# Robinatp/YOLO_Tensorflow

Measured on AMD Instinct MI355X. Metric: images_per_sec, higher is better.
Workload: dtype bf16; 1 GPU; YOLOv3 416x416 batch=32 per GPU, bf16: conv stack + head decode + threshold + TF-NMS; global_batch=32, input=uint8 NHWC resident in HBM, weights=seeded synthetic darknet stream (seed 0), parallelism=dp1

## Files before the change

### include/yolo_hip.h

```cpp
#ifndef YOLO_HIP_H
#define YOLO_HIP_H

#include <stddef.h>
#include <stdint.h>

#ifdef __cplusplus
extern "C" {
#endif

typedef struct yolo_ctx yolo_ctx;

enum yolo_status {
    YOLO_OK = 0,
    YOLO_ERR_INVALID = -1,
    YOLO_ERR_HIP = -2,
    YOLO_ERR_STATE = -3,
    YOLO_ERR_NOMEM = -4,
    YOLO_ERR_IO = -5,
    YOLO_ERR_UNSUPPORTED = -6
};

enum yolo_dtype { YOLO_BF16 = 0, YOLO_FP32 = 1, YOLO_FP8 = 2,
                  YOLO_FP16 = 3,
                  YOLO_FP16X2 = 4 };
// ... 12 lines not shown
    YOLO_NMS_TF_V1 = 4,
    YOLO_NMS_NUMPY_V3 = 3
};
enum yolo_select_mode {
    YOLO_SELECT_GT = 0,
    YOLO_SELECT_GE = 1
};

typedef struct yolo_config {
    uint32_t struct_size;
    const char *cfg_text;
    int32_t max_batch;
    int32_t dtype;
    int32_t semantics;
    int32_t decode;
    int32_t device;
    int32_t keep_layers;
    void *stream;
} yolo_config;

typedef struct yolo_box {
    float x0, y0, x1, y1;
    float score;
    int32_t cls;
} yolo_box;

typedef struct yolo_image_desc {
    uint64_t offset;
    int32_t h, w;
} yolo_image_desc;
enum yolo_fit {
    YOLO_FIT_STRETCH = 0,
    YOLO_FIT_LETTERBOX = 1,
    YOLO_FIT_CV2 = 2,
    YOLO_FIT_CV2_BGR = 3
};
enum yolo_box_units { YOLO_UNITS_NETWORK = 0, YOLO_UNITS_SOURCE_PIXELS = 1 };

yolo_ctx *yolo_create(const yolo_config *cfg, char *err, size_t err_len);
void yolo_destroy(yolo_ctx *ctx);
const char *yolo_last_error(const yolo_ctx *ctx);

int yolo_load_darknet_weights(yolo_ctx *ctx, const char *path, int header_ints);
int yolo_export(yolo_ctx *ctx, const char *path);
yolo_ctx *yolo_create_from_file(const char *path, int max_batch, int device, void *stream, int keep_layers, char *err, size_t err_len);
int yolo_set_weights(yolo_ctx *ctx, const float *flat, size_t n);
size_t yolo_weights_count(const yolo_ctx *ctx);
int yolo_set_act_scales(yolo_ctx *ctx, const float *scales, int n_layers);

int yolo_input_size(const yolo_ctx *ctx, int *height, int *width, int *channels);
int yolo_num_rows(const yolo_ctx *ctx);
int yolo_num_attrs(const yolo_ctx *ctx);
int yolo_num_layers(const yolo_ctx *ctx);
int yolo_head_geometry_hw(const yolo_ctx *ctx, int head, int *kind, int *grid_h, int *grid_w, int *anchors, int *row_offset);
int yolo_head_geometry(const yolo_ctx *ctx, int head, int *kind, int *grid, int *anchors, int *row_offset);
double yolo_conv_flops(const yolo_ctx *ctx);
double yolo_conv_bytes(const yolo_ctx *ctx, int n);

int yolo_forward(yolo_ctx *ctx, const void *images, int n, int fmt, int loc, float scale,
                 float *detections_out, int out_loc);

int yolo_forward_image_u8(yolo_ctx *ctx, const uint8_t *image, int h, int w, int loc,
                          float *detections_out, int out_loc);
int yolo_forward_letterbox_chw(yolo_ctx *ctx, const float *image_chw, int w, int h, int loc,
                               float *detections_out, int out_loc);

int yolo_forward_images_u8(yolo_ctx *ctx, const uint8_t *pixels, size_t bytes, const yolo_image_desc *descs, int n, int fit, int loc,
                           float *detections_out, int out_loc);
int yolo_detect_images_u8(yolo_ctx *ctx, const uint8_t *pixels, size_t bytes, const yolo_image_desc *descs, int n, int fit, int loc,
                          float score_thr, float iou_thr, int max_out, int nms_mode, int select_mode, int units,
                          yolo_box *boxes_out, int32_t *counts_out, int out_loc);
int yolo_detect_images_graph(yolo_ctx *ctx, const uint8_t *pixels, size_t bytes, const yolo_image_desc *descs, int n, int fit,
                             float score_thr, float iou_thr, int max_out, int nms_mode, int select_mode, int units,
                             yolo_box *boxes_out, int32_t *counts_out);
float yolo_fit_unit_value(int fit, int value);

int yolo_darknet_boxes(yolo_ctx *ctx, int w, int h, float thresh, int relative, float *records, int cap, int *count);
int yolo_darknet_boxes_at(yolo_ctx *ctx, int image, int w, int h, float thresh, int relative, float *records, int cap, int *count);
size_t yolo_last_layer_size(const yolo_ctx *ctx);
int yolo_last_layer_output(yolo_ctx *ctx, float *out, size_t out_floats);
int yolo_last_layer_output_batch(yolo_ctx *ctx, int n, float *out, size_t out_floats);

int yolo_head_raw(yolo_ctx *ctx, int head, int n, float *out, size_t out_floats);

int yolo_postprocess(yolo_ctx *ctx, int n, float score_thr, float iou_thr, int max_out,
                     int nms_mode, int select_mode, yolo_box *boxes_out, int32_t *counts_out, int out_loc);

int yolo_postprocess_rows(yolo_ctx *ctx, int n, float score_thr, float iou_thr, int max_out,
                          int nms_mode, int select_mode, yolo_box *boxes_out, int32_t *counts_out, int32_t *rows_out, int out_loc);

int yolo_detect(yolo_ctx *ctx, const void *images, int n, int fmt, int loc, float scale,
                float score_thr, float iou_thr, int max_out, int nms_mode, int select_mode,
                yolo_box *boxes_out, int32_t *counts_out, int out_loc);

int yolo_detect_graph(yolo_ctx *ctx, const void *images, int n, int fmt, float scale, float score_thr, float iou_thr,
                      int max_out, int nms_mode, int select_mode, yolo_box *boxes_out, int32_t *counts_out);

int yolo_synchronize(yolo_ctx *ctx);

int yolo_layer_output(yolo_ctx *ctx, int index, int n, float *out, size_t out_floats, int *dims_out);
int yolo_time_forward(yolo_ctx *ctx, int n, int iters, float *total_ms, float *conv_ms);
int yolo_calibrate(int device, void *stream, int f16, double seconds, float *tflops, float *clock_ghz);
int yolo_calibrate_copy(int device, void *stream, double seconds, float *gbs);
int yolo_time_layers(yolo_ctx *ctx, int n, int iters, float *ms_out);
int yolo_autotune(yolo_ctx *ctx, int n, int iters);
int yolo_get_tile_configs(const yolo_ctx *ctx, int32_t *cfgs);
int yolo_set_tile_configs(yolo_ctx *ctx, const int32_t *cfgs);

int yolo_op_conv2d(const float *x, int n, int h, int w, int cin, const float *w_hwio, const float *bias,
                   int k, int stride, int cout, int act, const float *residual, float *out,
                   int dtype, int tile_cfg, int device);
int yolo_op_conv_num_cfgs(void);
int yolo_op_upsample2x(const float *x, int n, int h, int w, int c, int semantics, float *out, int device);
int yolo_op_reorg(const float *x, int n, int h, int w, int c, int stride, int semantics, float *out, int device);
int yolo_op_maxpool(const float *x, int n, int h, int w, int c, int size, int stride, float *out, int device);
int yolo_op_resize_u8_hw(const uint8_t *img, int h, int w, int out_h, int out_w, float post_scale, float *out, int device);
int yolo_op_resize_u8(const uint8_t *img, int h, int w, int s, float post_scale, float *out, int device);
int yolo_op_resize_cv2(const uint8_t *img, int h, int w, int oh, int ow, int swap_rb, float divisor, float *out, int device);
int yolo_op_detections_boxes(const float *det, int n, int rows, int attrs, float *out, int device);
int yolo_op_decode_hw(const float *raw, int n, int gh, int gw, int na, int classes, const float *anchors_wh,
                      int img_h, int img_w, int decode, int region, float *out, int device);
int yolo_op_decode(const float *raw, int n, int g, int na, int classes, const float *anchors_wh,
                   int img_size, int decode, int region, float *out, int device);
int yolo_op_letterbox(const float *image_chw, int iw, int ih, int w, int h, int embed, float *out_chw, int device);
int yolo_op_nms_detections(const float *boxes_xywh, float *prob, float *objectness, int n, int classes, float thresh,
                           int by_objectness, int device);
int yolo_op_postprocess(const float *det, int n, int rows, int attrs, float score_thr, float iou_thr,
                        int max_out, int nms_mode, int select_mode, yolo_box *boxes_out,
                        int32_t *counts_out, int device);
int yolo_op_postprocess_rows(const float *det, int n, int rows, int attrs, float score_thr, float iou_thr,
                             int max_out, int nms_mode, int select_mode, yolo_box *boxes_out,
                             int32_t *counts_out, int32_t *rows_out, int device);

int yolo_num_classes(const yolo_ctx *ctx);
int yolo_classify(yolo_ctx *ctx, const void *images, int n, int fmt, int loc, float scale, int top_k,
                  int32_t *classes_out, float *probs_out, int out_loc);
int yolo_classify_images_u8(yolo_ctx *ctx, const uint8_t *pixels, size_t bytes, const yolo_image_desc *descs, int n, int fit, int loc,
                            int top_k, int32_t *classes_out, float *probs_out, int out_loc);
int yolo_op_avgpool(const float *x, int n, int h, int w, int c, int dtype, float *out, int device);
enum yolo_activation { YOLO_ACT_LINEAR = 0, YOLO_ACT_LEAKY = 1, YOLO_ACT_RELU = 2, YOLO_ACT_RELIE = 3, YOLO_ACT_LOGISTIC = 4, YOLO_ACT_LOGGY = 5,
                       YOLO_ACT_ELU = 6, YOLO_ACT_RAMP = 7, YOLO_ACT_TANH = 8, YOLO_ACT_PLSE = 9, YOLO_ACT_STAIR = 10, YOLO_ACT_HARDTAN = 11, YOLO_ACT_LHTAN = 12 };
int yolo_activation_code(const char *name);
int yolo_op_activate(const float *x, int n, int h, int w, int c, int act, int dtype, float *out, int device);
int yolo_op_shortcut(const float *x, int n, int h2, int w2, int c2, const float *from, int h1, int w1, int c1, int act, int dtype,
                     float *out, int device);
int yolo_op_softmax(const float *x, int n, int len, int groups, float temperature, int top_k, float *probs_out,
                    int32_t *classes_out, float *topk_probs_out, int device);

enum yolo_hierarchy_mode { YOLO_HIER_CONDITIONAL = 0, YOLO_HIER_ABSOLUTE = 1, YOLO_HIER_LEAVES = 2 };
int yolo_set_hier_thresh(yolo_ctx *ctx, float hier_thresh);
int yolo_set_hierarchy_mode(yolo_ctx *ctx, int mode);
int yolo_darknet_boxes_map(yolo_ctx *ctx, int image, int w, int h, float thresh, int relative, const int32_t *map200, float *records, int cap, int *count);
int yolo_tree_geometry(const yolo_ctx *ctx, int32_t *nodes, int32_t *groups, int32_t *parent, int32_t *child, int32_t *group_offset,
                       int32_t *group_size, int32_t *leaf);
int yolo_tree_read(const char *path, int32_t *nodes, int32_t *groups, int32_t *parent, int32_t *child, int32_t *group_offset, int32_t *group_size,
                   int32_t *leaf, char *err, size_t err_len);
int yolo_plan_check(const char *cfg_text, int dtype, char *err, size_t err_len);
int yolo_plan_table(const char *cfg_text, int dtype, int max_batch, int keep_layers, char *out, size_t out_len, char *err, size_t err_len);
int yolo_op_tree_softmax(const float *x, int n, int len, const char *tree_path, float temperature, int mode, float *out, int device);
int yolo_op_tree_top(const float *x_logits, int n, const char *tree_path, float hier_thresh, int32_t *labels_out, int device);


int yolo_output_map_geometry(yolo_ctx *ctx, int *h, int *w, int *c);
int yolo_output_map(yolo_ctx *ctx, int n, float *out, size_t out_floats);
int yolo_label_map(yolo_ctx *ctx, int n, float thresh, uint8_t *labels_u8);
int yolo_segment_images_u8(yolo_ctx *ctx, const uint8_t *pixels, const yolo_image_desc *descs, int n, int fit, float thresh,
                           uint8_t *labels_u8, const uint64_t *label_offsets);
int yolo_op_deconv2d(const float *x, int n, int h, int w, int cin, const float *w_iohw, const float *bias, int size, int stride, int padding,
                     int cout, int act, int dtype, int out_f32, float *out, int device);
int yolo_op_conv2d_grouped(const float *x, int n, int h, int w, int cin, const float *w_oihw, const float *bias, int size, int stride, int padding,
                           int cout, int groups, int act, int dtype, int out_f32, float *out, int device);
int yolo_op_l2norm(const float *x, int n, int h, int w, int c, int dtype, float *out, int device);
int yolo_op_upsample(const float *x, int n, int h, int w, int c, int stride, float scale, int dtype, float *out, int device);
int yolo_op_label_map(const float *map, int n, int h, int w, int c, float thresh, uint8_t *labels_out, int device);

#ifdef __cplusplus
}
#endif
#endif
```

### yolo_tensorflow_amd/csrc/conv_cfgs.h

```cpp
#pragma once
#include "kernels.h"
#include <type_traits>

struct ConvCfg {
    int id, wp, wc, tp, tc, ns, bk, nl;
    bool halo;
    bool free;
    int bh, bw;
    bool head_tail;
};
#define X(id, wp, wc, tp, tc, ns, bk, nl) {id, wp, wc, tp, tc, ns, bk, nl, false, false, 0, 0, false},
#define HX(id, wp, wc, tp, tc, ns, bk, nl, free, bh, bw, head_tail) {id, wp, wc, tp, tc, ns, bk, nl, true, free, bh, bw, head_tail},
constexpr ConvCfg kCfgs[] = {
    X(0, 2, 2, 4, 4, 2, 64, 0)  X(1, 2, 2, 4, 4, 3, 64, 0)  X(2, 2, 2, 2, 4, 2, 64, 0)  X(3, 2, 2, 2, 4, 3, 64, 0)
    X(4, 4, 1, 4, 2, 2, 64, 0)  X(5, 4, 1, 4, 2, 3, 64, 0)  X(6, 2, 2, 4, 2, 2, 64, 0)  X(7, 2, 2, 4, 2, 3, 64, 0)
    X(8, 4, 1, 4, 4, 2, 64, 0)  X(9, 4, 1, 4, 4, 3, 64, 0)  X(10, 4, 2, 4, 4, 2, 64, 0) X(11, 4, 2, 4, 4, 3, 64, 0)
    X(12, 2, 4, 4, 4, 2, 64, 0) X(13, 2, 4, 4, 4, 3, 64, 0) X(14, 2, 2, 2, 2, 2, 64, 0) X(15, 2, 2, 2, 2, 4, 64, 0)
    X(16, 1, 4, 11, 2, 2, 64, 0) X(17, 1, 4, 11, 4, 2, 64, 0) X(18, 1, 4, 11, 1, 2, 64, 0) X(19, 1, 4, 10, 2, 2, 64, 0)
    X(20, 1, 4, 12, 2, 2, 64, 0) X(21, 1, 4, 9, 2, 2, 64, 0) X(22, 1, 4, 13, 2, 2, 64, 0) X(23, 1, 4, 6, 2, 2, 64, 0)
    X(24, 1, 4, 7, 2, 2, 64, 0)
    X(25, 1, 4, 11, 2, 2, 32, 0) X(26, 2, 2, 4, 2, 2, 32, 0)  X(27, 4, 1, 4, 2, 2, 32, 0)  X(28, 4, 1, 4, 4, 2, 32, 0)
    X(29, 2, 2, 2, 2, 2, 32, 0)  X(30, 2, 2, 2, 4, 2, 32, 0)
    X(31, 1, 8, 11, 2, 2, 64, 4) X(32, 1, 8, 11, 2, 2, 64, 0)
    X(33, 1, 4, 11, 2, 3, 64, 0) X(34, 1, 4, 6, 2, 3, 64, 0)
    X(35, 2, 4, 3, 4, 2, 64, 0)
    HX(36, 1, 8, 11, 2, 2, 64, 0, false, 13, 13, false) HX(37, 1, 8, 11, 2, 2, 64, 4, false, 13, 13, false)
    HX(38, 1, 4, 11, 2, 2, 64, 4, false, 13, 13, false) HX(39, 1, 4, 11, 2, 2, 64, 0, false, 13, 13, false)
    HX(40, 1, 8, 11, 2, 2, 64, 0, true, 13, 13, true)   HX(41, 1, 8, 11, 1, 2, 64, 0, true, 13, 13, false)
    HX(42, 1, 4, 11, 2, 2, 64, 0, true, 13, 13, false)  HX(43, 1, 8, 11, 1, 3, 64, 0, true, 13, 13, false)
    X(44, 1, 8, 6, 2, 2, 64, 0) X(45, 1, 8, 6, 2, 3, 64, 0) X(46, 2, 4, 3, 4, 2, 64, 0) X(47, 2, 4, 2, 4, 2, 64, 0)
    X(48, 2, 4, 3, 2, 2, 64, 0) X(49, 2, 4, 4, 2, 3, 64, 0) X(50, 1, 8, 4, 2, 3, 64, 0) X(51, 2, 4, 2, 2, 3, 64, 0)
    X(52, 2, 4, 3, 2, 3, 64, 0) X(53, 2, 4, 3, 2, 4, 64, 0)
    HX(54, 1, 8, 12, 2, 2, 64, 0, true, 10, 19, true) HX(55, 1, 8, 12, 1, 3, 64, 0, true, 10, 19, false) HX(56, 1, 8, 6, 1, 3, 64, 0, true, 5, 19, false)
    HX(57, 1, 4, 11, 4, 2, 64, 0, true, 13, 13, false) HX(58, 1, 4, 11, 2, 2, 64, 0, true, 13, 13, false)
};
#undef X
#undef HX
constexpr int kNumCfgs = (int)(sizeof(kCfgs) / sizeof(kCfgs[0]));
constexpr bool conv_cfgs_indexed() { for (int i = 0; i < kNumCfgs; ++i) if (kCfgs[i].id != i) return false; return true; }
static_assert(conv_cfgs_indexed(), "a tile configuration's id is its index in kCfgs");

template <int... I> struct CfgList { static constexpr bool has(int cfg) { return ((cfg == I) || ...); } };
template <int... I, class F> hipError_t cfg_dispatch(CfgList<I...>, int cfg, F &&f)
{
    hipError_t e = hipErrorInvalidValue;
    (void)((cfg == I && ((e = f(std::integral_constant<int, I>{})), true)) || ...);
    return e;
}
using Cfgs16 = CfgList<0, 1, 2, 3, 4, 5, 6, 7, 8, 9, 10, 11, 12, 13, 14, 15, 16, 17, 18, 19, 20, 21, 22, 23, 24, 25, 26, 27, 28, 29, 30, 31, 32, 33, 34, 35,
                       44, 45, 46, 47, 48, 49, 50, 51, 52, 53>;
using CfgsHalo16 = CfgList<36, 37, 38, 39, 40, 41, 42, 43, 54, 55, 56>;
using CfgsFp8 = CfgList<0, 2, 4, 6, 8, 12, 14, 16, 17, 19, 20, 23, 31, 32, 33, 34, 45, 48, 49, 51>;
using CfgsHaloFp8 = CfgList<36, 37, 38, 39, 40, 41, 42, 43>;
using CfgsSplit = CfgList<0, 2, 3, 4, 6, 7, 8, 14, 15, 16, 23, 25, 26, 27, 28, 33, 34, 45, 49, 52>;
using CfgsHaloSplit = CfgList<40, 41, 43>;
using CfgsPairK = CfgList<0, 2, 3, 4, 6, 7, 8, 14, 15, 16, 23, 33, 34, 45, 49, 52>;
using CfgsHaloPairK = CfgList<40, 41, 43, 57, 58>;
using CfgsPairKPlain = CfgList<0, 2, 4, 6, 8, 14, 16, 33>;

template <int... I> constexpr bool cfgs_are(CfgList<I...>, bool halo) { return ((I >= 0 && I < kNumCfgs && kCfgs[I].halo == halo) && ...); }
static_assert(cfgs_are(Cfgs16{}, false) && cfgs_are(CfgsFp8{}, false) && cfgs_are(CfgsSplit{}, false) && cfgs_are(CfgsPairK{}, false) && cfgs_are(CfgsPairKPlain{}, false), "tiled lists hold tiled ids");
static_assert(cfgs_are(CfgsHalo16{}, true) && cfgs_are(CfgsHaloFp8{}, true) && cfgs_are(CfgsHaloSplit{}, true) && cfgs_are(CfgsHaloPairK{}, true), "halo lists hold halo ids");

inline bool conv_cfg_instantiated(const ConvArgs &a, int cfg)
{
    if (a.in_dt == DT_FP8) return CfgsFp8::has(cfg) || CfgsHaloFp8::has(cfg);
    if (a.pairk) return a.split ? CfgsPairK::has(cfg) || CfgsHaloPairK::has(cfg) : CfgsPairKPlain::has(cfg);
    if (a.split) return CfgsSplit::has(cfg) || CfgsHaloSplit::has(cfg);
    return Cfgs16::has(cfg) || CfgsHalo16::has(cfg);
}

constexpr bool conv_tail_shape(int wp, int wc, int bc, int nl, int eb) { return wp == 1 && wc == 8 && (eb == 2 ? nl == 0 && (bc == 256 || bc == 128) : bc == 256); }
```

### yolo_tensorflow_amd/csrc/conv_igemm.hip

```cpp
#include "kernels.h"
#include <cstdio>
#include <mutex>
#include <set>
#include <utility>

hipError_t conv_opt_in_lds(const void *kernel, size_t lds_bytes)
{
    static std::mutex mu;
    static std::set<std::pair<int, const void *>> done;
    int dev = 0;
    hipError_t e = hipGetDevice(&dev); if (e != hipSuccess) return e;
    std::lock_guard<std::mutex> g(mu);
    if (done.count({dev, kernel})) return hipSuccess;
    e = hipFuncSetAttribute(kernel, hipFuncAttributeMaxDynamicSharedMemorySize, (int)lds_bytes);
    if (e == hipSuccess) done.insert({dev, kernel});
    return e;
}

#include "conv_igemm_kernel.h"


template <int EB>
static hipError_t launch_conv_diag_t(const ConvArgs &a, hipStream_t s)
{
// ... 94 lines not shown
{
    return (a.in_dt == DT_BF16 || (a.in_dt == DT_F16 && a.out_dt == DT_F16)) && a.ksize == 3 && a.stride == 1 && a.pad == 1 && a.Cin_pad == 8 && a.out_dt != DT_F32 && !a.res && a.Kpad >= 96 &&
           (a.Cout == 16 || a.Cout == 32 || a.Cout == 64);
}

hipError_t launch_conv_c8_direct(const ConvArgs &a, hipStream_t s)
{
    const long M = (long)a.N * a.Ho * a.Wo;
    long waves = (M + 63) / 64;
    long blocks = (waves + 3) / 4; if (blocks > 256 * 8) blocks = 256 * 8;
    dim3 grid((unsigned)blocks), block(256);
    if (a.in_dt == DT_F16) {
        if (a.Cout == 16) hipLaunchKernelGGL((conv_c8_3x3_direct<1, true>), grid, block, 0, s, a);
        else if (a.Cout == 32) hipLaunchKernelGGL((conv_c8_3x3_direct<2, true>), grid, block, 0, s, a);
        else hipLaunchKernelGGL((conv_c8_3x3_direct<4, true>), grid, block, 0, s, a);
    }
    else if (a.Cout == 16) hipLaunchKernelGGL((conv_c8_3x3_direct<1>), grid, block, 0, s, a);
    else if (a.Cout == 32) hipLaunchKernelGGL((conv_c8_3x3_direct<2>), grid, block, 0, s, a);
    else hipLaunchKernelGGL((conv_c8_3x3_direct<4>), grid, block, 0, s, a);
    return hipGetLastError();
}

int conv_num_cfgs() { return kNumCfgs; }
bool conv_cfg_is_halo(int cfg) { return cfg >= 0 && cfg < kNumCfgs && kCfgs[cfg].halo; }
bool conv_cfg_tail_ok(int cfg, int cout, bool fp8, bool head)
{
    if (cfg < 0 || cfg >= kNumCfgs) return false;
    const ConvCfg &c = kCfgs[cfg];
    const int bc = c.wc * c.tc * 16;
    if (head) return !fp8 && c.head_tail && cout == 256;
    return conv_tail_shape(c.wp, c.wc, bc, c.nl, fp8 ? 1 : 2) && bc == cout;
}
const char *conv_cfg_name(int cfg)
{
    struct Names {
        char s[kNumCfgs][32];
        Names()
        {
            for (const ConvCfg &c : kCfgs) {
                const int bp = c.wp * c.tp * 16, bc = c.wc * c.tc * 16;
                if (c.halo && !CfgsHalo16::has(c.id)) snprintf(s[c.id], sizeof s[c.id], "f%dc%d_w%d_pair", bp, bc, c.wp * c.wc);
                else if (c.halo && (c.bh != HALO_B || c.bw != HALO_B)) snprintf(s[c.id], sizeof s[c.id], "f%dx%dc%d_s%d", c.bh, c.bw, bc, c.ns);
                else snprintf(s[c.id], sizeof s[c.id], "%s%dc%d_s%d_k%d%s%d", c.halo ? (c.free ? "f" : "h") : "p", bp, bc, c.ns, c.bk, c.nl ? "_L" : "_w", c.nl ? c.nl : c.wp * c.wc);
            }
        }
    };
    static const Names names;
    if (cfg < 0 || cfg >= kNumCfgs) return cfg == CONV_CFG_DIRECT ? "direct_c8" : "?";
    return names.s[cfg];
}

template <int WP, int WC, int TP, int TC, int NS, int BK, int NL, bool UNI, int EB, bool H16 = false, bool SPLIT = false>
static hipError_t launch_u(const ConvArgs &a, hipStream_t s)
{
    constexpr int BP = WP * TP * 16, BC = WC * TC * 16;
    const long M = (long)a.N * a.Ho * a.Wo;
    const long tiles = ((M + BP - 1) / BP) * ((a.Cout + BC - 1) / BC);
    constexpr size_t lds = conv_lds_bytes<WP, WC, TP, TC, NS, BK, NL>();
    dim3 grid((unsigned)((tiles + 7) / 8 * 8)), block(64 * (WP * WC + NL));
    if (lds > 65536) {
        hipError_t e = conv_opt_in_lds((const void *)conv_igemm<WP, WC, TP, TC, NS, BK, UNI, NL, false, EB, false, false, H16, SPLIT>, lds);
        if (e != hipSuccess) return e;
    }
    hipLaunchKernelGGL((conv_igemm<WP, WC, TP, TC, NS, BK, UNI, NL, false, EB, false, false, H16, SPLIT>), grid, block, lds, s, conv_tile_magic(a, BC, 0));
    return hipGetLastError();
}

template <int WP, int WC, int TP, int TC, int NS, int BK, int NL, int EB, bool H16 = false, bool SPLIT = false>
static hipError_t launch_t(const ConvArgs &a, hipStream_t s)
{
    if (((double)a.N * a.H * a.W * a.in_stride + 2.0 * (a.W + 1) * a.in_stride) * EB >= 2147483648.0) return hipErrorInvalidValue;
    constexpr int BKE = BK * 2 / EB;
    if (a.Kpad % BKE) return hipErrorInvalidValue;
    return (a.Cin_pad % BKE) == 0 ? launch_u<WP, WC, TP, TC, NS, BK, NL, true, EB, H16, SPLIT>(a, s) : launch_u<WP, WC, TP, TC, NS, BK, NL, false, EB, H16, SPLIT>(a, s);
}

template <int ID, int EB, bool H16 = false, bool SPLIT = false>
static hipError_t launch_id(const ConvArgs &a, hipStream_t s)
{
    constexpr ConvCfg c = kCfgs[ID];
    return launch_t<c.wp, c.wc, c.tp, c.tc, c.ns, c.bk, c.nl, EB, H16, SPLIT>(a, s);
}

hipError_t launch_conv_bf16(const ConvArgs &a, int cfg, hipStream_t s)
{
    if (a.in_dt != DT_BF16 && a.in_dt != DT_F16) return hipErrorInvalidValue;
    if (a.in_dt == DT_F16 && a.out_dt != DT_F16 && a.out_dt != DT_F32) return hipErrorInvalidValue;
    if (cfg == CONV_CFG_DIRECT && a.split) return launch_conv_c8_direct_pair(a, s);
    if (a.pairk) return launch_conv_pair(a, cfg, s);
    if (a.split) {
        if (a.in_dt != DT_F16 || (a.out_dt != DT_F16 && a.out_dt != DT_F32) || a.w2 || (a.res && a.out_dt == DT_F32)) return hipErrorInvalidValue;
        if (CfgsHaloSplit::has(cfg)) return launch_conv_halo13(a, cfg, s);
        return cfg_dispatch(CfgsSplit{}, cfg, [&](auto id) { return launch_id<decltype(id)::value, 2, true, true>(a, s); });
    }
    if (cfg == CONV_CFG_DIRECT) return conv_c8_direct_ok(a) ? launch_conv_c8_direct(a, s) : hipErrorInvalidValue;
    if (conv_cfg_is_halo(cfg)) return launch_conv_halo13(a, cfg, s);
    if (a.in_dt == DT_F16) return cfg_dispatch(Cfgs16{}, cfg, [&](auto id) { return launch_id<decltype(id)::value, 2, true>(a, s); });
    return cfg_dispatch(Cfgs16{}, cfg, [&](auto id) { return launch_id<decltype(id)::value, 2>(a, s); });
}

hipError_t launch_conv_fp8(const ConvArgs &a, int cfg, hipStream_t s)
{
    if (a.in_dt != DT_FP8) return hipErrorInvalidValue;
    if (CfgsHaloFp8::has(cfg)) return launch_conv_halo13(a, cfg, s);
    return cfg_dispatch(CfgsFp8{}, cfg, [&](auto id) { return launch_id<decltype(id)::value, 1>(a, s); });
}
```

### yolo_tensorflow_amd/csrc/conv_igemm_kernel.h

```cpp
#pragma once
#include "kernels.h"
#include "conv_cfgs.h"
#include "device_common.h"
#include "halo_perm_tables.h"
#include <type_traits>
#include <utility>

__device__ __forceinline__ uint32_t f32_to_bf16_rn(float f)
{
    __bf16 b = (__bf16)f;
    return (uint32_t)__builtin_bit_cast(uint16_t, b);
}
__device__ __forceinline__ float bf16_bits_to_f32(uint32_t b) { return __builtin_bit_cast(float, b << 16); }
__device__ __forceinline__ void pair_join2(uint32_t H, uint32_t L, float &a, float &b)
{
    asm("v_fma_mix_f32 %0, %1, 1.0, %2 op_sel_hi:[1,0,1]" : "=v"(a) : "v"(H), "v"(L));
    asm("v_fma_mix_f32 %0, %1, 1.0, %2 op_sel:[1,0,1] op_sel_hi:[1,0,1]" : "=v"(b) : "v"(H), "v"(L));
}
__device__ __forceinline__ void pair_split2(float a, float b, uint32_t &H, uint32_t &L)
{
    H = __builtin_bit_cast(uint32_t, __builtin_convertvector(f32x2_t{a, b}, f16x2_t));
    uint32_t l;
    asm("v_fma_mixlo_f16 %0, %1, -1.0, %2 op_sel_hi:[1,0,0]" : "=v"(l) : "v"(H), "v"(a));
    asm("v_fma_mixhi_f16 %0, %1, -1.0, %2 op_sel:[1,0,0] op_sel_hi:[1,0,0]" : "+v"(l) : "v"(H), "v"(b));
    L = l;
}
template <bool HI> __device__ __forceinline__ uint32_t f32x2_to_fp8(float a, float b, uint32_t old)
{
    a = __builtin_amdgcn_fmed3f(a, -FP8_MAX, FP8_MAX); b = __builtin_amdgcn_fmed3f(b, -FP8_MAX, FP8_MAX);
    return (uint32_t)__builtin_amdgcn_cvt_pk_fp8_f32(a, b, (int)old, HI);
}

__device__ __forceinline__ int fast_div(int n, uint32_t mul, uint32_t shift)
{
    return shift == 255 ? n : (int)(__umulhi((uint32_t)n, mul) >> shift);
}

constexpr int PAIR_PD = 4, PAIR_SLEEP = 48;
template <int MAXN> __device__ __forceinline__ void wait_vmcnt_rt(int n)
{
    static_assert(MAXN <= 16, "ladder length");
    switch (n) {
#define W_(k) case k: if (k <= MAXN) { wait_vmcnt<k>(); } break;
        W_(1) W_(2) W_(3) W_(4) W_(5) W_(6) W_(7) W_(8) W_(9) W_(10) W_(11) W_(12) W_(13) W_(14) W_(15) W_(16)
#undef W_
    default: wait_vmcnt<0>(); break;
    }
}

#define OOB_OFFSET 0x80000000u

template <int... I, class F> __device__ __forceinline__ void static_for_impl(std::integer_sequence<int, I...>, F &&f) { (f(std::integral_constant<int, I>{}), ...); }
template <int N, class F> __device__ __forceinline__ void static_for(F &&f) { static_for_impl(std::make_integer_sequence<int, N>{}, f); }

struct HaloPermPk { unsigned w[16][8]; };
template <int N> constexpr HaloPermPk make_halo_perm_pk(const unsigned short (&tab)[N])
{
    HaloPermPk t{};
    for (int l = 0; l < 16; ++l)
        for (int j = 0; j < N / 16; ++j) {
            const unsigned v = tab[j * 16 + l];
            t.w[l][j / 4] |= (v & 0xffu) << (8 * (j % 4));
            t.w[l][4 + j / 4] |= (v >> 8) << (8 * (j % 4));
        }
    return t;
}
__device__ const HaloPermPk kHaloPermPk = make_halo_perm_pk(kHaloPerm13);
__device__ const HaloPermPk kHaloPermPk10x19 = make_halo_perm_pk(kHaloPerm10x19);
__device__ const HaloPermPk kHaloPermPk5x19 = make_halo_perm_pk(kHaloPerm5x19);
constexpr int HALO_B = 13;
constexpr int HALO_APIX = 160;
constexpr int halo_apieces(int bh, int bw) { return ((bh + 2) * (bw + 2) * (HALO_APIX / 16) + 63) / 64; }
constexpr int HALO_APIECES = halo_apieces(HALO_B, HALO_B);
constexpr int HALO_ACT_BYTES = HALO_APIECES * 1024;
constexpr unsigned halo_div_mul(int bw) { return (65536u + bw - 1) / bw; }
constexpr bool halo_div_ok(int bw) { for (unsigned r = 0; r < 256; ++r) if (((r * halo_div_mul(bw)) >> 16) != r / bw) return false; return true; }

template <int WP, int WC, int TP, int TC, int NS, int BK, bool UNI, int NL = 0, bool DIAG = false, int EB = 2, bool HALO = false, bool FREE = false, bool H16 = false, bool SPLIT = false, int BH = HALO_B, int BW = HALO_B, bool HEADT = false, bool PAIRK = false>
__global__ __launch_bounds__(64 * (WP * WC + NL)) void conv_igemm(const ConvArgs a)
{
#if defined(__HIP_DEVICE_COMPILE__)
    constexpr int NC = WP * WC;
    constexpr int NW = NL > 0 ? NL : NC;
    constexpr int NTOT = NC + NL;
    constexpr int BP = WP * TP * 16;
    constexpr int BC = WC * TC * 16;
    static_assert(BK == 64 || BK == 32, "K-step");
    static_assert(BC <= 256, "filters and bias are padded to multiples of 256 output channels (cout_pad): a wider tile would read past them");
    static_assert(EB == 2 || (EB == 1 && BK == 64), "fp8 operands need the 128-B-row form");
    static_assert(!H16 || EB == 2, "fp16 is a 16-bit storage type");
    static_assert(!SPLIT || (H16 && !DIAG), "split pairs are fp16 pairs");
    static_assert(!PAIRK || (H16 && EB == 2 && BK == 64 && UNI && !DIAG && NL == 0), "pair K loop: fp16, 128-byte rows = one 32-channel group hi | lo, uniform taps");
    constexpr int RB = BK * 2;
    constexpr int EPC = 16 / EB;
    constexpr int BKE = RB / EB;
    constexpr int CPRW = RB / 16;
    constexpr int RG = 64 / CPRW;
    constexpr int GP = (BP + RG - 1) / RG, GC = (BC + RG - 1) / RG;
    constexpr int LA = (GP + NW - 1) / NW, LB = (GC + NW - 1) / NW;
    constexpr int L = LA + LB;
    constexpr int BPL = LA * NW * RG, BCL = LB * NW * RG;
    constexpr int STAGE_BYTES = (BPL + BCL) * RB;
    static_assert(!HALO || (WP == 1 && TP == (BH * BW + 15) / 16 && TP <= 16 && BK == 64 && UNI && (NS == 2 || (FREE && NS <= 4))), "halo form: one BH x BW block per workgroup; more than two filter stages in the free-running form only");
    static_assert((BH == 13 && BW == 13) || (BH == 10 && BW == 19) || (BH == 5 && BW == 19), "block shapes with a generated permutation table");
    static_assert(halo_div_ok(BW) && BH * BW <= 256, "row / BW by multiply-high");
    constexpr int HBH = BH, HBW = BW, HPW = BW + 2, HPH = BH + 2, APIX = HALO_APIX, APIECES = halo_apieces(BH, BW), ACT_BYTES = APIECES * 1024;
    constexpr int LAH = HALO ? (APIECES + NW - 1) / NW : 1;
    constexpr int FSTAGE = BCL * RB;
    static_assert(!HALO || LAH <= 9, "a halo tile is fetched during the nine taps of the previous chunk");
    static_assert(!FREE || (HALO && NL == 0 && LB * RG == TC * 16), "free-running form: every wave fetches its own filter rows");

    if constexpr (H16) fp16_saturating_mode();
    extern __shared__ __attribute__((aligned(16))) char smem[];

    unsigned long long t_top = 0;
    if (DIAG) asm volatile("s_memtime %0\n\ts_waitcnt lgkmcnt(0)" : "=s"(t_top)::"memory");
    const int tid = threadIdx.x;
    const int lane = tid & 63;
    u32x4_t perm_rd = {0, 0, 0, 0}, perm_wr = {0, 0, 0, 0};
    if constexpr (HALO) {
        const u32x4_t *pk = (const u32x4_t *)(BH == 10 ? kHaloPermPk10x19.w[lane & 15] : BH == 5 ? kHaloPermPk5x19.w[lane & 15] : kHaloPermPk.w[lane & 15]);
        perm_rd = pk[0]; perm_wr = pk[1];
    }
    asm volatile("" ::"s"(a.in), "s"(a.wt), "s"(a.in_stride), "s"(a.N), "s"(a.H), "s"(a.W), "s"(a.Cout), "s"(a.Kpad), "s"(a.Ho), "s"(a.Wo),
                 "s"(a.tc_mul), "s"(a.tc_shift), "s"(a.bpi_mul), "s"(a.bpi_shift), "s"(a.bpr_mul), "s"(a.bpr_shift));
    const int wave_id = __builtin_amdgcn_readfirstlane(tid >> 6);
    const bool is_loader = NL == 0 || wave_id >= NC;
    const bool is_consumer = wave_id < NC;
    const int wid = NL > 0 ? (wave_id >= NC ? wave_id - NC : 0) : wave_id;
    const int wpi = wave_id % WP, wci = (wave_id / WP) % WC;

    const int M = a.N * a.Ho * a.Wo;
    const int tilesC = (a.Cout + BC - 1) / BC;
    const int hbr = HALO ? (a.H + HBH - 1) / HBH : 0, hbc = HALO ? (a.W + HBW - 1) / HBW : 0;
    const int tilesP = HALO ? a.N * hbr * hbc : (M + BP - 1) / BP;
    const int per_xcd = gridDim.x >> 3;
    const int tile = (blockIdx.x & 7) * per_xcd + (blockIdx.x >> 3);
    if (tile >= tilesP * tilesC) return;
    const int pt = fast_div(tile, a.tc_mul, a.tc_shift);
    const int ct = tile - pt * tilesC;
    int bn = 0, by = 0, bx = 0;
    if constexpr (HALO) {
        const int bpr = hbc, bpi = hbc * hbr;
        bn = fast_div(pt, a.bpi_mul, a.bpi_shift); const int r = pt - bn * bpi; by = fast_div(r, a.bpr_mul, a.bpr_shift); bx = r - by * bpr;
    }

    const int shift = HALO ? 0 : (a.W + 1) * a.in_stride * EB;
    __amdgpu_buffer_rsrc_t rx = buf_rsrc((const char *)a.in - shift);
    __amdgpu_buffer_rsrc_t rw = buf_rsrc(a.wt);

    const int rl = lane / CPRW;
    const int chunk = BK == 64 ? ((lane & 7) ^ (rl & 7)) : ((lane & 3) ^ (3 * ((rl >> 2) & 1)));
    const int KK = a.ksize * a.ksize;
    const int HoWo = a.Ho * a.Wo;
    unsigned woff[LB > 0 ? LB : 1];
#pragma unroll
    for (int i = 0; i < LB; ++i) {
        const int crow = (FREE ? wid * LB + i : wid + i * NW) * RG + rl;
        woff[i] = crow < BC ? (unsigned)((ct * BC + crow) * a.Kpad + chunk * EPC) * (unsigned)EB : OOB_OFFSET;
    }
    if (is_loader && 0 < a.Kpad / BKE) {
// ... 715 lines not shown
                if (is_consumer) {
                    const float slope2 = act_slope(a.act2);
                    f32x4 b2v[T2W];
#pragma unroll
                    for (int t = 0; t < T2W; ++t) b2v[t] = *(const f32x4 *)(a.b2 + (t2g * T2W + t) * 16 + lq * 4);
                    const int hch = (t2g * T2W) * 16 + lq * 4;
                    auto finish = [&](const f32x4 &acc2, int j, int t) {
                        f32x4 v = acc2 + b2v[t];
                        if constexpr (HEAD_TAIL_OK) if (head_tail) {
                            const unsigned r = (unsigned)(j * 16 + l15), y = __umul24(r, halo_div_mul(BW)) >> 16, x = r - __umul24(y, (unsigned)BW);
                            if (y < ylim && x < xlim) {
                                const size_t m = m0 + (size_t)y * a.W + x;
                                const int ch = hch + t * 16;
                                float *o = (float *)a.out2 + m * a.out2_stride + ch;
                                if (a.obj_out) {
#pragma unroll
                                    for (int q = 0; q < 4; ++q) {
                                        const int an = fast_div(ch + q, a.obj_mul, a.obj_shift);
                                        if (ch + q - an * a.obj_attrs == 4 && ch + q < a.C2out) a.obj_out[m * a.obj_na + an] = v[q];
                                    }
                                }
                                if (ch + 3 < a.C2out) *(float4 *)o = float4{v[0], v[1], v[2], v[3]};
                                else
                                    for (int q = 0; q < 4; ++q) if (ch + q < a.C2out) o[q] = v[q];
                            }
                            return;
                        }
                        const f32x4 u = v * slope2;
#pragma unroll
                        for (int q = 0; q < 4; ++q) v[q] = vmax_f32(v[q], u[q]);
                        *(uint2 *)(st2 + (j * 16 + l15) * RS2 + ((t2g * T2W + t) * 16 + lq * 4) * 2) = uint2{pack16x2<H16>(v[0], v[1]), pack16x2<H16>(v[2], v[3])};
                    };
                    const int j0 = head_tail ? 0 : (TP * t2p) / T2P, j1 = head_tail ? TP : (TP * (t2p + 1)) / T2P;
                    {
                        int j = j0;
#pragma unroll 1
                        for (; j + 1 < j1; j += 2) {
                            f32x4 ca[T2W], cb[T2W];
#pragma unroll
                            for (int t = 0; t < T2W; ++t) ca[t] = cb[t] = f32x4{0.f, 0.f, 0.f, 0.f};
#pragma unroll
                            for (int kk = 0; kk < K2S; ++kk) {
                                const bf16x8 xa = *(const bf16x8 *)(smem + (j * 16 + l15) * RS + (kk * 4 + lq) * 16);
                                const bf16x8 xb = *(const bf16x8 *)(smem + ((j + 1) * 16 + l15) * RS + (kk * 4 + lq) * 16);
#pragma unroll
                                for (int t = 0; t < T2W; ++t) {
                                    ca[t] = mma16<H16>(fw2[t][kk], xa, ca[t]);
                                    cb[t] = mma16<H16>(fw2[t][kk], xb, cb[t]);
                                }
                            }
#pragma unroll
                            for (int t = 0; t < T2W; ++t) { finish(ca[t], j, t); finish(cb[t], j + 1, t); }
                        }
                        if (j < j1) {
                            f32x4 cc_[T2W];
#pragma unroll
                            for (int t = 0; t < T2W; ++t) cc_[t] = f32x4{0.f, 0.f, 0.f, 0.f};
#pragma unroll
                            for (int kk = 0; kk < K2S; ++kk) {
                                const bf16x8 x = *(const bf16x8 *)(smem + (j * 16 + l15) * RS + (kk * 4 + lq) * 16);
#pragma unroll
                                for (int t = 0; t < T2W; ++t) cc_[t] = mma16<H16>(fw2[t][kk], x, cc_[t]);
                            }
#pragma unroll
                            for (int t = 0; t < T2W; ++t) finish(cc_[t], j, t);
                        }
                    }
                }
                if (DIAG) te5 = stamp();
                asm volatile("s_waitcnt lgkmcnt(0)" ::: "memory");
                block_barrier();
                if (DIAG) te6 = stamp();
                constexpr int CPR2 = C2 / 8;
                const __amdgpu_buffer_rsrc_t rs_out2 = tile_rsrc((char *)a.out2 + m0 * a.out2_stride * 2);
                if (!head_tail)
#pragma unroll
                for (int it = 0; it < (BP * CPR2 + NT - 1) / NT; ++it) {
                    int row, cc;
                    const unsigned off = piece_off(tid + it * NT, CPR2, 0, (unsigned)a.out2_stride * 2u, row, cc);
                    __builtin_amdgcn_raw_buffer_store_b128(*(const u32x4_t *)(st2 + row * RS2 + cc * 16), rs_out2, off, 0, OUT_STORE_AUX);
                }
            }
        }
    } else if (is_consumer && !HALO) {
#pragma unroll
        for (int i = 0; i < TC; ++i) {
            const int ch = ct * BC + (wci * TC + i) * 16 + lq * 4;
            if (ch >= a.Cout) continue;
            const float4 bv = *(const float4 *)(a.bias + ch);
            float4 sv = float4{1.f, 1.f, 1.f, 1.f};
            if (EB == 1 && a.oscale) sv = *(const float4 *)(a.oscale + ch);
            int oq = -1, oan = 0;
            if (a.obj_out) {
#pragma unroll
                for (int q = 0; q < 4; ++q) {
                    const int an = fast_div(ch + q, a.obj_mul, a.obj_shift);
                    if (ch + q - an * a.obj_attrs == 4 && ch + q < a.Cout) { oq = q; oan = an; }
                }
            }
#pragma unroll
            for (int j = 0; j < TP; ++j) {
                const int m = pt * BP + (wpi * TP + j) * 16 + l15;
                if (m >= M) continue;
                float v[4];
                if (EB == 1) { v[0] = acc[i][j][0] * sv.x + bv.x; v[1] = acc[i][j][1] * sv.y + bv.y; v[2] = acc[i][j][2] * sv.z + bv.z; v[3] = acc[i][j][3] * sv.w + bv.w; }
                else { v[0] = acc[i][j][0] + bv.x; v[1] = acc[i][j][1] + bv.y; v[2] = acc[i][j][2] + bv.z; v[3] = acc[i][j][3] + bv.w; }
                if (a.act != ACT_LINEAR) {
                    const float slope = act_slope(a.act);
#pragma unroll
                    for (int q = 0; q < 4; ++q) v[q] = fmaxf(v[q], slope * v[q]);
                }
                float *o = (float *)a.out + (size_t)m * a.out_stride + ch;
                if (oq >= 0) a.obj_out[(size_t)m * a.obj_na + oan] = oq == 0 ? v[0] : oq == 1 ? v[1] : oq == 2 ? v[2] : v[3];
                if (ch + 3 < a.Cout) *(float4 *)o = float4{v[0], v[1], v[2], v[3]};
                else
                    for (int q = 0; q < 4; ++q) if (ch + q < a.Cout) o[q] = v[q];
            }
        }
    }
    if (DIAG && a.dbg && lane == 0) {
        asm volatile("s_waitcnt vmcnt(0)" ::: "memory");
        const unsigned long long t_end = stamp_loop();
        unsigned long long *d = a.dbg + ((size_t)tile * NTOT + wave_id) * 16;
        const unsigned long long rt1 = __builtin_amdgcn_s_memrealtime();
        d[0] = t_wait; d[1] = t_issue; d[2] = t_mma; d[3] = t_loop_end - t_all0; d[4] = t_end - t_loop_end;
        d[6] = t_all0 - t_top; d[7] = t_first - t_all0; d[8] = te1 - t_loop_end; d[9] = te2 - te1; d[10] = te3 - te2; d[11] = t_end - (te6 ? te6 : te3);
        d[12] = te4 ? te4 - te3 : 0; d[13] = te4 ? te5 - te4 : 0; d[14] = te4 ? te6 - te5 : 0;
        d[15] = (t_loop_end - t_all0) * 100ull / (rt_loop - rt0 ? rt_loop - rt0 : 1);
        d[5] = ((unsigned long long)KT << 40) | ((t_end - t_all0) * 100ull / (rt1 - rt0 ? rt1 - rt0 : 1));
    }
#endif
}

template <int WP, int WC, int TP, int TC, int NS, int BK, int NL = 0, bool HALO = false, int BH = HALO_B, int BW = HALO_B>
constexpr size_t conv_lds_bytes()
{
    constexpr int NW = NL > 0 ? NL : WP * WC, BP = WP * TP * 16, BC = WC * TC * 16;
    constexpr int RG = 64 / (BK * 2 / 16);
    constexpr int LA = ((BP + RG - 1) / RG + NW - 1) / NW, LB = ((BC + RG - 1) / RG + NW - 1) / NW;
    constexpr size_t stage = (size_t)(LA + LB) * NW * RG * (BK * 2);
    constexpr bool tail = conv_tail_shape(WP, WC, BC, 0, 2);
    constexpr size_t lds0 = HALO ? (size_t)2 * halo_apieces(BH, BW) * 1024 + (size_t)NS * LB * NW * RG * (BK * 2) : (size_t)NS * stage, ldso = (size_t)BP * (BC * 2 + 16) + (tail ? (size_t)BP * (BC + 16) : 0);
    return lds0 > ldso ? lds0 : ldso;
}
```

### yolo_tensorflow_amd/csrc/kernels.h

```cpp
#pragma once
#ifndef OUT_STORE_AUX
#define OUT_STORE_AUX 16
#endif
#ifndef HALO_LOAD_AUX
#define HALO_LOAD_AUX 0
#endif
#ifndef RES_LOAD_AUX
#define RES_LOAD_AUX 0
#endif
#include <hip/hip_runtime.h>
#include <stdint.h>
typedef unsigned out_u32x4 __attribute__((ext_vector_type(4)));
__device__ __forceinline__ void out_store16_at(const void *base, unsigned byte_off, unsigned x, unsigned y, unsigned z, unsigned w)
{
#if defined(__HIP_DEVICE_COMPILE__)
    __amdgpu_buffer_rsrc_t r = __builtin_amdgcn_make_buffer_rsrc((void *)base, 0, 0x80000000u, 0x00020000);
    __builtin_amdgcn_raw_buffer_store_b128(out_u32x4{x, y, z, w}, r, byte_off, 0, OUT_STORE_AUX);
#endif
}

typedef uint16_t bf16_t;
struct fp8_t { uint8_t b; };
struct f16_t { uint16_t b; };
enum { DT_BF16 = 0, DT_F32 = 1, DT_FP8 = 2, DT_F16 = 3 };
inline size_t dt_size(int dt) { return dt == DT_F32 ? 4 : dt == DT_FP8 ? 1 : 2; }
#define FP8_MAX 448.0f

struct TView {
    void *ptr = nullptr;
    int n = 0, h = 0, w = 0, c = 0;
    int stride = 0;
    int dt = DT_BF16;
};

enum { ACT_LINEAR = 0, ACT_LEAKY = 1, ACT_RELU = 2, ACT_RELIE = 3, ACT_LOGISTIC = 4, ACT_LOGGY = 5, ACT_ELU = 6, ACT_RAMP = 7, ACT_TANH = 8,
       ACT_PLSE = 9, ACT_STAIR = 10, ACT_HARDTAN = 11, ACT_LHTAN = 12, ACT_COUNT = 13 };
inline bool act_is_slope(int act) { return act == ACT_LINEAR || act == ACT_LEAKY || act == ACT_RELU || act == ACT_RELIE; }
int act_from_name(const char *name);

struct ConvArgs {
    const void *in; int in_stride;
    const void *wt;
    const float *bias;
    void *out; int out_stride; int out_dt;
    const void *res; int res_stride;
    int in_dt;
    int split;
    int pairk;
    const float *oscale;
    float out_inv_scale, res_scale;
    float mid_scale, mid_inv_scale;
    const void *w2; const float *b2; void *out2; int out2_stride, K2pad, act2;
    const void *w2f;
    const float *oscale2; float out2_inv_scale;
    int N, H, W, Cin_pad;
    int Ho, Wo, Cout;
    int ksize, stride, pad;
    int Kpad;
    int kchunk;
    int act;
    const void *zeros;
    uint32_t howo_mul, howo_shift, wo_mul, wo_shift;
    float *obj_out; int obj_attrs, obj_na; uint32_t obj_mul, obj_shift;
    unsigned long long *dbg;
    int dbg_light;
    int C2out;
    int tail_f32;
    uint32_t tc_mul, tc_shift, bpi_mul, bpi_shift, bpr_mul, bpr_shift;
};
inline int conv_kchunk(int cin_pad, int wdt) { const int row = wdt == DT_FP8 ? 128 : 64; return (wdt != DT_F32 && cin_pad % row == 0) ? row : cin_pad; }
inline void conv_magic(uint32_t d, uint32_t &mul, uint32_t &shift)
{
    if (d <= 1) { mul = 0; shift = 255; return; }
    uint32_t l = 0; while ((1u << l) < d) ++l;
    const unsigned k = 31 + l;
    mul = (uint32_t)(((unsigned long long)1 << k) / d + 1);
    shift = k - 32;
}
inline void conv_finalize(ConvArgs &a)
{
    conv_magic((uint32_t)(a.Ho * a.Wo), a.howo_mul, a.howo_shift);
    conv_magic((uint32_t)a.Wo, a.wo_mul, a.wo_shift);
}
inline ConvArgs conv_tile_magic(const ConvArgs &a0, int BC, int bh, int bw = 0)
{
    ConvArgs a = a0;
    if (bw == 0) bw = bh;
    conv_magic((uint32_t)((a.Cout + BC - 1) / BC), a.tc_mul, a.tc_shift);
    if (bh > 0) { const int br = (a.H + bh - 1) / bh, bc = (a.W + bw - 1) / bw; conv_magic((uint32_t)(br * bc), a.bpi_mul, a.bpi_shift); conv_magic((uint32_t)bc, a.bpr_mul, a.bpr_shift); }
    return a;
}

hipError_t conv_opt_in_lds(const void *kernel, size_t lds_bytes);
#define CONV_CFG_DIRECT 1000
bool conv_c8_direct_ok(const ConvArgs &a);
int conv_num_cfgs();
const char *conv_cfg_name(int cfg);
int conv_default_cfg(const ConvArgs &a);
bool conv_cfg_runs(const ConvArgs &a, int cfg);
int conv_resolve_cfg(const ConvArgs &a, int planned);
hipError_t launch_conv_bf16(const ConvArgs &a, int cfg, hipStream_t s);
bool conv_halo13_ok(const ConvArgs &a);
bool conv_halo_cfg_ok(const ConvArgs &a, int cfg);
bool conv_cfg_is_halo(int cfg);
hipError_t launch_conv_halo13(const ConvArgs &a, int cfg, hipStream_t s);
hipError_t launch_conv_halo13_diag(const ConvArgs &a, hipStream_t s, int variant = 0);
bool conv_cfg_tail_ok(int cfg, int cout, bool fp8, bool head = false);
hipError_t launch_conv_pair(const ConvArgs &a, int cfg, hipStream_t s);
struct StemPairArgs {
    const void *in;
    const uint8_t *in_u8; float in_scale, in_mul, in_add;
    const void *w0; const float *b0; int Kpad0, C0, act0;
    const void *w1; const float *b1; int Kpad1, act1;
    void *out; int out_stride;
    int N, H, W, Ho, Wo;
};
bool conv_stem_pair_ok(const StemPairArgs &a);
hipError_t launch_conv_stem_pair(const StemPairArgs &a, hipStream_t s);
bool conv_c8_direct_pair_ok(const ConvArgs &a);
hipError_t launch_conv_c8_direct_pair(const ConvArgs &a, hipStream_t s);
hipError_t launch_conv_fp8(const ConvArgs &a, int cfg, hipStream_t s);
hipError_t launch_conv_diag(const ConvArgs &a, hipStream_t s);
struct StemArgs {
    const void *in; int in_stride;
    const uint8_t *in_u8; float in_scale, in_mul, in_add;
    const void *w0; const float *b0; int Kpad0, C0, act0;
    const void *w1; const float *b1; int Kpad1, C1, act1;
    void *out; int out_stride;
    int dt;
    const void *w2; const float *b2; int Kpad2, C2, act2;
    void *out2; int out2_stride;
    int N, H, W, Ho, Wo;
    const void *zeros;
};
bool conv_stem_ok(const StemArgs &a);
hipError_t launch_conv_stem(const StemArgs &a, hipStream_t s);
struct HaloArgs {
    const void *in; int in_stride;
    const void *w; const float *b; int Kpad, Cin, Cout, act;
    const void *res; int res_stride;
    void *out; int out_stride;
    int N, H, W;
    int dt;
};
bool conv_halo_ok(const HaloArgs &a);
hipError_t launch_conv_halo(const HaloArgs &a, hipStream_t s);
bool conv_s2_ok(const HaloArgs &a);
hipError_t launch_conv_s2(const HaloArgs &a, hipStream_t s);
struct C3S2Args {
    const void *in; int in_stride;
    const void *w3; const float *b3; int Kpad3, act3;
    const void *res; int res_stride;
    const void *w5; const float *b5; int Kpad5, act5;
    void *out; int out_stride;
    int N, H, W;
    int dt;
};
bool conv_c3s2_ok(const C3S2Args &a);
hipError_t launch_conv_c3s2(const C3S2Args &a, hipStream_t s);
struct BlockArgs {
    const void *x; int x_stride;
    const void *w1; const float *b1; int Kpad1, act1;
    const void *w2; const float *b2; int Kpad2, act2;
    void *out; int out_stride;
    int N, H, W, C, Cmid;
    int dt;
};
bool conv_resblock_ok(const BlockArgs &a);
hipError_t launch_conv_resblock(const BlockArgs &a, hipStream_t s);
hipError_t launch_conv_f32(const ConvArgs &a, hipStream_t s);

#define DECONV_MAX_SIZE 7
#define DECONV_MAX_STRIDE 4
#define DECONV_CO_TILE 32
struct DeconvArgs {
    const void *in; int in_stride;
    const void *wt;
    const float *bias;
    void *out; int out_stride; int out_dt, in_dt;
    int N, H, W, Cin_pad, Ho, Wo, Cout;
    int Cstore;
    int size, stride, pad, act;
    int cout_pad;
    int woff[DECONV_MAX_STRIDE * DECONV_MAX_STRIDE], kp[DECONV_MAX_STRIDE * DECONV_MAX_STRIDE];
// ... 205 lines not shown
```

### yolo_tensorflow_amd/csrc/post_ops.hip

```cpp
#include "kernels.h"
#include "wave_ops.h"
#include <math.h>

struct BoxOut { float x0, y0, x1, y1, score; int cls; };

__device__ __forceinline__ float sigmoidf_(float x) { return 1.0f / (1.0f + expf(-x)); }
__device__ __forceinline__ float sigmoid_fast(float x)
{
    const float e = __builtin_amdgcn_exp2f(-x * 1.44269504088896340736f);
    return __builtin_amdgcn_rcpf(1.0f + e);
}

__device__ __forceinline__ float yolo_box_attr(int k, float x, int cx, int cy, const float *anchor, float GW, float GH, float SX, float SY, int mode)
{
    const float t = k < 2 ? sigmoidf_(x) + (float)(k == 0 ? cx : cy) : expf(x) * anchor[k - 2];
    const float G = (k & 1) ? GH : GW, S = (k & 1) ? SY : SX;
    return mode == 0 ? t / G : t * S;
}

__global__ __launch_bounds__(256) void k_decode_yolo(const DecodeArgs a, float *scores, int *labels)
{
    const int attrs = 5 + a.classes;
    const int lane = threadIdx.x & 63;
    const long wave = ((long)blockIdx.x * blockDim.x + threadIdx.x) >> 6;
    const long nwaves = ((long)gridDim.x * blockDim.x) >> 6;
    const int gg = a.gh * a.gw;
    const long total = (long)a.n * gg * a.na;
    const float GW = (float)a.gw, GH = (float)a.gh, SX = (float)(a.img_w / a.gw), SY = (float)(a.img_h / a.gh);
    constexpr int U = 4;
    const bool two = attrs > 64;
    for (long b0 = wave * U; b0 < total; b0 += nwaves * U) {
        float v0[U], v1[U];
        const float *src[U]; float *dst[U]; size_t rowi[U]; int an_[U], cell_[U];
        const unsigned ub = (unsigned)__builtin_amdgcn_readfirstlane((int)b0);
        unsigned t0 = ub / (unsigned)a.na; int an = (int)(ub - t0 * a.na);
        int b = (int)(t0 / (unsigned)gg); int cell = (int)(t0 - (unsigned)b * gg);
#pragma unroll
        for (int u = 0; u < U; ++u) {
            if (u > 0 && b0 + u < total) { if (++an == a.na) { an = 0; if (++cell == gg) { cell = 0; ++b; } } }
            an_[u] = an; cell_[u] = cell;
            src[u] = a.raw + ((size_t)b * gg + cell) * a.raw_stride + an * attrs;
            rowi[u] = (size_t)b * a.rows_total + a.row_off + (size_t)cell * a.na + an;
            dst[u] = a.det + rowi[u] * attrs;
            v0[u] = lane < attrs ? src[u][lane] : 0.f;
            v1[u] = (two && lane + 64 < attrs) ? src[u][lane + 64] : 0.f;
        }
#pragma unroll
        for (int u = 0; u < U; ++u) {
            if (b0 + u >= total) break;
            const int an = an_[u], cell = cell_[u];
            const float r0 = lane < 4 ? yolo_box_attr(lane, v0[u], cell % a.gw, cell / a.gw, a.anchors + 2 * an, GW, GH, SX, SY, a.mode) : sigmoid_fast(v0[u]);
            const float r1 = sigmoid_fast(v1[u]);
            if (lane < attrs) dst[u][lane] = r0;
            if (two && lane + 64 < attrs) dst[u][lane + 64] = r1;
            const float obj = __shfl(r0, 4);
            float best = -INFINITY; int bi = 0x7fffffff;
            if (lane >= 5 && lane < attrs) { best = obj * r0; bi = lane - 5; }
            if (two && lane + 64 < attrs) first_max(best, bi, obj * r1, lane + 59);
            wave_argmax(best, bi);
            if (lane == 0 && scores) { scores[rowi[u]] = best; labels[rowi[u]] = bi; }
        }
    }
}

template <int CTRL, int ROWS = 0xF, typename T>
__device__ __forceinline__ T dpp(T v)
{
    const int i = __builtin_bit_cast(int, v);
    return __builtin_bit_cast(T, __builtin_amdgcn_update_dpp(i, i, CTRL, ROWS, 0xF, false));
}
template <typename T, typename Op>
__device__ __forceinline__ T row_reduce_dpp(T v, Op op)
{
    v = op(v, dpp<0xB1>(v));
    v = op(v, dpp<0x4E>(v));
    v = op(v, dpp<0x124>(v));
    v = op(v, dpp<0x128>(v));
    return v;
}
__device__ __forceinline__ float row_max_dpp(float v) { return row_reduce_dpp(v, [](float x, float y) { return fmaxf(x, y); }); }
__device__ __forceinline__ int row_min_dpp(int v) { return row_reduce_dpp(v, [](int x, int y) { return min(x, y); }); }
__device__ __forceinline__ float wave_max_dpp(float v)
{
    v = row_max_dpp(v);
    v = fmaxf(v, dpp<0x142, 0xA>(v));
    v = fmaxf(v, dpp<0x143, 0xC>(v));
    return __builtin_bit_cast(float, __builtin_amdgcn_readlane(__builtin_bit_cast(int, v), 63));
}

__device__ __forceinline__ int block_rank(bool flag, int *wcnt, int &total)
{
    const int lane = threadIdx.x & 63, wv = threadIdx.x >> 6;
    const unsigned long long m = __ballot(flag);
    if (lane == 0) wcnt[wv] = __popcll(m);
// ... 36 lines not shown
    }
    for (long p = wave; p < total; p += nwaves) {
        const unsigned up = (unsigned)__builtin_amdgcn_readfirstlane((int)p);
        const int b = (int)(up / (unsigned)gg), cell = (int)(up - (unsigned)b * gg);
        const int cy = cell / a.gw, cx = cell - cy * a.gw;
        const size_t row0 = (size_t)b * a.rows_total + a.row_off + (size_t)cell * a.na;
        float *dst = a.det ? a.det + row0 * attrs : nullptr;
        float *dst4 = a.box4 ? a.box4 + row0 * 4 : nullptr;
        float x[R], v[R];
#pragma unroll
        for (int r = 0; r < R; ++r) x[r] = xn[r];
        if (p + nwaves < total) {
            const float *src = a.raw + (size_t)(p + nwaves) * a.raw_stride;
#pragma unroll
            for (int r = 0; r < R; ++r) xn[r] = ok_[r] ? src[lane + 64 * r] : 0.f;
        }
        float xs = 0.f; int ks = 4, ans = 0;
        if (merged) {
#pragma unroll
            for (int r = 0; r < R; ++r) if (spec_[r]) { xs = x[r]; ks = k_[r]; ans = an_[r]; }
            const float vs = ks < 4 ? yolo_box_attr(ks, xs, cx, cy, a.anchors + 2 * ans, GW, GH, SX, SY, a.mode) : 0.f;
#pragma unroll
            for (int r = 0; r < R; ++r) {
                v[r] = spec_[r] ? vs : sigmoid_fast(x[r]);
                if (dst) { if (ok_[r]) dst[lane + 64 * r] = v[r]; }
                else if (spec_[r]) dst4[an_[r] * 4 + k_[r]] = v[r];
            }
        } else {
#pragma unroll
            for (int r = 0; r < R; ++r) {
                v[r] = k_[r] < 4 ? yolo_box_attr(k_[r], x[r], cx, cy, a.anchors + 2 * an_[r], GW, GH, SX, SY, a.mode) : sigmoid_fast(x[r]);
                if (dst) { if (ok_[r]) dst[lane + 64 * r] = v[r]; }
                else if (spec_[r]) dst4[an_[r] * 4 + k_[r]] = v[r];
            }
        }
        if (!scores) continue;
        for (int an = 0; an < a.na; ++an) {
            const int oc = an * attrs + 4, ol = oc & 63, orr = oc >> 6;
            float ov = v[0];
#pragma unroll
            for (int r = 1; r < R; ++r) ov = orr == r ? v[r] : ov;
            const float obj = __shfl(ov, ol);
            if (obj < a.reject_below) {
                if (lane == 0) { scores[row0 + an] = obj; labels[row0 + an] = 0; }
                continue;
            }
            float sc[R]; float best = -INFINITY;
#pragma unroll
            for (int r = 0; r < R; ++r) {
                sc[r] = (ok_[r] && an_[r] == an && k_[r] >= 5) ? obj * v[r] : -INFINITY;
                best = fmaxf(best, sc[r]);
            }
            best = wave_max_dpp(best);
            int label = 0x7fffffff;
#pragma unroll
            for (int r = R - 1; r >= 0; --r) {
                const unsigned long long m = __ballot(sc[r] == best);
                if (m) label = (int)__builtin_ctzll(m) + 64 * r - an * attrs - 5;
            }
            if (lane == 0) { scores[row0 + an] = best; labels[row0 + an] = label; }
        }
    }
}

__global__ __launch_bounds__(1024) void k_decode_yolo_lean_p1(const LeanArgs a, float *scores, int *labels)
{
    __shared__ int wcnt[16]; __shared__ unsigned s_base;
    const int attrs = 5 + a.classes;
    for (long base = (long)blockIdx.x * 1024; base < a.total; base += (long)gridDim.x * 1024) {
        const long box = base + threadIdx.x;
        const bool valid = box < a.total;
        int hd = 0;
#pragma unroll
        for (int k = 1; k < 4; ++k) if (k < a.nheads && box >= a.h[k].box_begin) hd = k;
        const float *raw = a.h[0].raw, *objp = a.h[0].obj; int raw_stride = a.h[0].raw_stride, gg = a.h[0].gh * a.h[0].gw, na = a.h[0].na, row_off = a.h[0].row_off; long bb = a.h[0].box_begin;
#pragma unroll
        for (int k = 1; k < 4; ++k) if (hd == k) { raw = a.h[k].raw; objp = a.h[k].obj; raw_stride = a.h[k].raw_stride; gg = a.h[k].gh * a.h[k].gw; na = a.h[k].na; row_off = a.h[k].row_off; bb = a.h[k].box_begin; }
        const unsigned ubox = valid ? (unsigned)(box - bb) : 0u;
        const unsigned cidx = ubox / (unsigned)na; const int an = (int)(ubox - cidx * (unsigned)na);
        const unsigned b = cidx / (unsigned)gg; const int cell = (int)(cidx - b * (unsigned)gg);
        const unsigned row = b * (unsigned)a.rows_total + (unsigned)row_off + (unsigned)cell * (unsigned)na + (unsigned)an;
        const unsigned eoff = cidx * (unsigned)raw_stride + (unsigned)(an * attrs);
        const float obj = sigmoid_fast(objp ? objp[ubox] : raw[eoff + 4]);
        const bool pass = valid && !(obj < a.reject_below);
        if (valid && !pass) { scores[row] = obj; labels[row] = 0; }
        int tot;
        const int rank = block_rank(pass, wcnt, tot);
        if (threadIdx.x == 0 && tot) s_base = atomicAdd(a.list_count, (unsigned)tot);
        __syncthreads();
        const unsigned slot = s_base + (unsigned)rank;
        if (pass && slot < a.list_cap) a.list[slot] = uint4{eoff, row, (unsigned)cell | ((unsigned)an << 24) | ((unsigned)hd << 28), __float_as_uint(obj)};
    }
}
__global__ __launch_bounds__(256) void k_decode_yolo_lean_p2(const LeanArgs a, float *scores, int *labels)
{
    const int attrs = 5 + a.classes;
    const int l15 = threadIdx.x & 15;
    const unsigned rowid = (blockIdx.x * blockDim.x + threadIdx.x) >> 4, nrows = (gridDim.x * blockDim.x) >> 4;
    unsigned count = __hip_atomic_load(a.list_count, __ATOMIC_RELAXED, __HIP_MEMORY_SCOPE_AGENT);
    if (count > a.list_cap) count = a.list_cap;
    for (unsigned base = 0; base < count; base += nrows) {
        const unsigned idx = base + rowid;
        const bool act = idx < count;
        const uint4 d = act ? a.list[idx] : uint4{0, 0, 0, 0};
        const unsigned r_eoff = d.x, r_row = d.y; const int r_cell = (int)(d.z & 0xffffffu), r_an = (int)((d.z >> 24) & 15u), r_hd = (int)(d.z >> 28);
        const float r_obj = __uint_as_float(d.w);
        const float *r_raw = a.h[0].raw; int r_gw = a.h[0].gw, r_gh = a.h[0].gh; float r_sx = a.h[0].sx, r_sy = a.h[0].sy;
#pragma unroll
        for (int k = 1; k < 4; ++k) if (r_hd == k) { r_raw = a.h[k].raw; r_gw = a.h[k].gw; r_gh = a.h[k].gh; r_sx = a.h[k].sx; r_sy = a.h[k].sy; }
        const float *src = r_raw + r_eoff;
        float vv[8];
#pragma unroll
        for (int t = 0; t < 8; ++t) { const int k = l15 + 16 * t; vv[t] = (act && k < attrs) ? src[k] : 0.f; }
        const float g_raw = vv[0];
        float best = -INFINITY; int label = 0x7fffffff;
#pragma unroll
        for (int t = 0; t < 8; ++t) {
            const int k = l15 + 16 * t;
            if (act && k >= 5 && k < attrs) first_max(best, label, r_obj * sigmoid_fast(vv[t]), k - 5);
        }
        const float rbest = row_max_dpp(best);
        const int rlabel = row_min_dpp(best == rbest ? label : 0x7fffffff);
        if (act && l15 < 4) {
            a.box4[(size_t)r_row * 4 + l15] = yolo_box_attr(l15, g_raw, r_cell % r_gw, r_cell / r_gw, a.h[r_hd].anchors + 2 * r_an, (float)r_gw, (float)r_gh, r_sx, r_sy, a.mode);
            if (l15 == 0) { scores[r_row] = rbest; labels[r_row] = rlabel; }
        }
    }
}
hipError_t launch_decode_lean(const LeanArgs &a, float *scores, int *labels, hipStream_t s)
{
    if (a.nheads < 1 || a.nheads > 4 || !a.box4 || !scores || !labels || 5 + a.classes > 128 || !a.list || !a.list_count) return hipErrorInvalidValue;
    size_t blocks = ((size_t)a.total + 1023) / 1024; if (blocks > 256 * 2) blocks = 256 * 2;
    hipLaunchKernelGGL(k_decode_yolo_lean_p1, dim3((unsigned)blocks), dim3(1024), 0, s, a, scores, labels);
    hipLaunchKernelGGL(k_decode_yolo_lean_p2, dim3(1024), dim3(256), 0, s, a, scores, labels);
    return hipGetLastError();
}

__global__ void k_decode_region(const DecodeArgs a)
{
    const int attrs = 5 + a.classes;
    size_t box = (size_t)blockIdx.x * blockDim.x + threadIdx.x;
    const int gg = a.gh * a.gw;
    const size_t total = (size_t)a.n * gg * a.na;
    if (box >= total) return;
    int an = (int)(box % a.na); size_t t = box / a.na;
    int cell = (int)(t % gg); int b = (int)(t / gg);
    const float *p = a.raw + ((size_t)b * gg + cell) * a.raw_stride + an * attrs;
    float *o = a.det + ((size_t)b * a.rows_total + a.row_off + (size_t)cell * a.na + an) * attrs;
#pragma unroll
    for (int k = 0; k < 5; ++k) o[k] = region_box_attr(k, p, cell, a.gw, a.gh, a.anchors + 2 * an);
    float mx = -INFINITY;
    for (int k = 0; k < a.classes; ++k) mx = fmaxf(mx, p[5 + k]);
    float sum = 0.f;
    for (int k = 0; k < a.classes; ++k) sum += expf(p[5 + k] - mx);
    for (int k = 0; k < a.classes; ++k) o[5 + k] = expf(p[5 + k] - mx) / sum;
}

__global__ void k_decode_v1(const float *raw, int raw_stride, int n, int S, int B, int C, int sqr, float *det, int rows_total, int row_off,
                            float *scores, int *labels)
{
    const int i = blockIdx.x * blockDim.x + threadIdx.x;
    const int per = S * S * B;
    if (i >= n * per) return;
    const int img = i / per, r = i - img * per, cell = r / B, b = r - cell * B;
    const float *p = raw + (size_t)img * raw_stride;
    const float *cls = p + cell * C, *box = p + S * S * (C + B) + (cell * B + b) * 4;
    const float conf = p[S * S * C + cell * B + b];
// ... 674 lines not shown
```

### yolo_tensorflow_amd/csrc/yolo_api.cpp

```cpp
#include "yolo_ctx.h"

namespace yolo_impl {

int need_map(yolo_ctx *c, const char *what)
{
    if (c->map_layer < 0) return fail(c, YOLO_ERR_INVALID, "%s: the network is not a map network (a %s; [net] yolo_output=map declares one)", what, c->cls_layer >= 0 ? "classifier" : "detector");
    return YOLO_OK;
}

int map_to_f32(yolo_ctx *c, int n)
{
    const Layer &M = c->layers[c->map_layer];
    const size_t cap = 2 * (size_t)c->max_batch * M.H * M.W * M.C;
    if (c->map_f32_cap < cap) { HIPCK(c, hipMalloc((void **)&c->d_map_f32, cap * 4)); c->map_f32_cap = cap; }
    TView v = M.out; v.n = n;
    HIPCK(c, launch_to_f32(v, c->d_map_f32, c->stream));
    return YOLO_OK;
}

int map_f32_view(yolo_ctx *c, int n, const float **map, int *stride)
{
    const Layer &M = c->layers[c->map_layer];
    if (M.out.dt == DT_F32) { *map = (const float *)M.out.ptr; *stride = M.out.stride; return YOLO_OK; }
    if (int r = map_to_f32(c, n)) return r;
// ... 87 lines not shown
    if (int r = yolo_head_geometry_hw(c, head, kind, &gh, &gw, anchors, row_offset)) return r;
    if (gh != gw) return fail(const_cast<yolo_ctx *>(c), YOLO_ERR_UNSUPPORTED, "yolo_head_geometry: head %d has a %d x %d grid; use yolo_head_geometry_hw", head, gh, gw);
    if (grid) *grid = gh;
    return YOLO_OK;
}
double yolo_conv_flops(const yolo_ctx *c) { return c ? c->conv_flops : 0; }
double yolo_conv_bytes(const yolo_ctx *c, int n)
{
    if (!c) return 0;
    double b = 0;
    for (int i = 0; i < (int)c->layers.size(); ++i) if (c->layers[i].type == L_CONV) {
        const Layer &L = c->layers[i];
        const TView in = view_of(c, L.in[0]); const double ie = (double)dt_size(L.in_dt), oe = (double)dt_size(L.out.dt);
        if (!input_never_loaded(L, i)) b += (double)n * in.h * in.w * L.cin * ie;
        if (!never_stored(L, i)) b += (double)n * L.H * L.W * L.filters * oe;
        b += (double)L.filters * L.cin * L.size * L.size * ie;
    }
    return b;
}

int yolo_darknet_boxes(yolo_ctx *c, int w, int h, float thresh, int relative, float *records, int cap, int *count)
{
    return yolo_darknet_boxes_at(c, 0, w, h, thresh, relative, records, cap, count);
}

int yolo_darknet_boxes_at(yolo_ctx *c, int image, int w, int h, float thresh, int relative, float *records, int cap, int *count)
{
    return yolo_darknet_boxes_map(c, image, w, h, thresh, relative, nullptr, records, cap, count);
}

int yolo_darknet_boxes_map(yolo_ctx *c, int image, int w, int h, float thresh, int relative, const int32_t *map200, float *records, int cap, int *count)
{
    if (!c || !count) return YOLO_ERR_INVALID;
    if (map200) {
        if (c->tree_head < 0) return fail(c, YOLO_ERR_INVALID, "yolo_darknet_boxes_map: the network has no [region] head with a tree");
        if (c->attrs - 5 < 200) return fail(c, YOLO_ERR_INVALID, "yolo_darknet_boxes_map: a map has 200 entries and the head only %d classes", c->attrs - 5);
        for (int j = 0; j < 200; ++j) if (map200[j] < 0 || map200[j] >= c->attrs - 5) return fail(c, YOLO_ERR_INVALID, "yolo_darknet_boxes_map: map[%d] = %d is not a class", j, (int)map200[j]);
    }
    if (int r = need_detector(c, "yolo_darknet_boxes")) return r;
    if (c->last_n < 1 || !c->det_valid) return fail(c, YOLO_ERR_STATE, "yolo_darknet_boxes needs a yolo_forward* pass first");
    if (image < 0 || image >= c->last_n) return fail(c, YOLO_ERR_INVALID, "image %d outside the last forward's batch of %d", image, c->last_n);
    if (w < 1 || h < 1 || cap < 0 || (cap > 0 && !records)) return fail(c, YOLO_ERR_INVALID, "bad image size / capacity");
    HIPCK(c, hipSetDevice(c->device));
    if (!c->d_dn_rec) {
        HIPCK(c, hipMalloc((void **)&c->d_dn_rec, (size_t)c->rows * c->attrs * 4));
        HIPCK(c, hipMalloc((void **)&c->d_dn_src, (size_t)c->rows * 4));
        HIPCK(c, hipMalloc((void **)&c->d_dn_count, 4));
    }
    DnBoxesArgs a; memset(&a, 0, sizeof a);
    a.det = c->d_det + (size_t)image * c->rows * c->attrs; a.attrs = c->attrs;
    for (size_t li = 0; li < c->layers.size(); ++li) {
        const Layer &L = c->layers[li];
        if (L.type != L_YOLO && L.type != L_REGION && L.type != L_DETECT) continue;
        if (a.nheads == 8) return fail(c, YOLO_ERR_UNSUPPORTED, "more than 8 heads");
        if (L.type == L_DETECT) {
            if (a.nheads) return fail(c, YOLO_ERR_UNSUPPORTED, "a [detection] head next to other heads");
            a.raw = (const float *)c->layers[li - 1].out.ptr + (size_t)image * c->layers[li - 1].out.stride; a.side = L.side; a.classes = L.classes; a.sqr = L.sqr;
            a.kind[0] = 2; a.cells[0] = L.side * L.side; a.na[0] = L.na; a.off[0] = L.row_off; a.nheads = 1;
            continue;
        }
        if (a.raw) return fail(c, YOLO_ERR_UNSUPPORTED, "a [detection] head next to other heads");
        a.kind[a.nheads] = L.type == L_REGION; a.cells[a.nheads] = L.H * L.W; a.na[a.nheads] = L.na; a.off[a.nheads] = L.row_off; ++a.nheads;
    }
    a.thresh = thresh; a.w = w; a.h = h; a.netw = c->in_w; a.neth = c->in_h; a.relative = relative;
    a.cap = cap < c->rows ? cap : c->rows;
    a.rec = a.cap > 0 ? c->d_dn_rec : nullptr; a.src = c->d_dn_src; a.count = c->d_dn_count;
    HIPCK(c, launch_darknet_boxes(a, c->stream));
    if (c->tree_head >= 0 && a.rec) {
        if (map200) {
            if (!c->d_map200) HIPCK(c, hipMalloc((void **)&c->d_map200, 200 * 4));
            HIPCK(c, hipMemcpyAsync(c->d_map200, map200, 200 * 4, hipMemcpyHostToDevice, c->stream));
        }
        HIPCK(c, launch_darknet_tree_probs(a.det, c->attrs, c->trees[c->layers[c->tree_head].tree].dev, thresh, c->hier_thresh, map200 ? c->d_map200 : nullptr,
                                           a.rec, a.src, a.count, a.cap, c->stream));
    }
    int n = 0;
    HIPCK(c, hipMemcpyAsync(&n, c->d_dn_count, 4, hipMemcpyDeviceToHost, c->stream)); HIPCK(c, hipStreamSynchronize(c->stream));
    *count = n;
    const int got = n < a.cap ? n : a.cap;
    if (got > 0) { HIPCK(c, hipMemcpyAsync(records, c->d_dn_rec, (size_t)got * c->attrs * 4, hipMemcpyDeviceToHost, c->stream)); HIPCK(c, hipStreamSynchronize(c->stream)); }
    return YOLO_OK;
}

size_t yolo_last_layer_size(const yolo_ctx *c)
{
    if (!c) return 0;
    if (c->cls_layer >= 0) return (size_t)c->layers[c->cls_layer].C;
    if (c->map_layer >= 0) { const Layer &M = c->layers[c->map_layer]; return (size_t)M.H * M.W * M.C; }
    for (int i = (int)c->layers.size() - 1; i >= 0; --i) {
        const Layer &L = c->layers[i];
        if (L.type == L_DETECT) return (size_t)L.side * L.side * (L.classes + 5 * L.na);
        if (L.type == L_YOLO || L.type == L_REGION) return (size_t)L.H * L.W * L.na * (5 + L.classes);
    }
    return 0;
}

int yolo_last_layer_output_batch(yolo_ctx *c, int n, float *out, size_t out_floats)
{
    if (!c || !out) return YOLO_ERR_INVALID;
    if (c->last_n < 1) return fail(c, YOLO_ERR_STATE, "yolo_last_layer_output before a forward pass");
    if (n < 1 || n > c->last_n) return fail(c, YOLO_ERR_INVALID, "yolo_last_layer_output of %d images but the last forward ran %d", n, c->last_n);
    if (c->cls_layer >= 0) {
        const Layer &S = c->layers[c->cls_layer];
        if (out_floats < (size_t)n * S.C) return fail(c, YOLO_ERR_INVALID, "output buffer too small (%zu < %zu floats)", out_floats, (size_t)n * S.C);
        HIPCK(c, hipSetDevice(c->device));
        return copy_out(c, out, S.out.ptr, (size_t)n * S.C * 4, YOLO_HOST);
    }
    if (c->map_layer >= 0) {
        const Layer &M = c->layers[c->map_layer];
        const size_t per = (size_t)M.H * M.W * M.C;
        if (out_floats < per * n) return fail(c, YOLO_ERR_INVALID, "output buffer too small (%zu < %zu floats)", out_floats, per * n);
        HIPCK(c, hipSetDevice(c->device));
        if (int r = map_to_f32(c, n)) return r;
        HIPCK(c, launch_nhwc_to_chw(c->d_map_f32, c->d_map_f32 + (size_t)c->max_batch * per, n, M.H * M.W, M.C, c->stream));
        return copy_out(c, out, c->d_map_f32 + (size_t)c->max_batch * per, per * n * 4, YOLO_HOST);
    }
    const int li = output_layer(c);
    if (li < 1 || (c->layers[li].type != L_YOLO && c->layers[li].type != L_REGION && c->layers[li].type != L_DETECT))
        return fail(c, YOLO_ERR_UNSUPPORTED, "the last layer is not a detection head");
    const Layer &L = c->layers[li]; const Layer &P = c->layers[li - 1];
    const size_t per = yolo_last_layer_size(c), need = per * (size_t)n;
    if (out_floats < need) return fail(c, YOLO_ERR_INVALID, "output buffer too small (%zu < %zu floats)", out_floats, need);
    HIPCK(c, hipSetDevice(c->device));
    if (L.type == L_DETECT) {
        HIPCK(c, hipMemcpy2DAsync(out, per * 4, P.out.ptr, (size_t)P.out.stride * 4, per * 4, (size_t)n, hipMemcpyDeviceToHost, c->stream)); HIPCK(c, hipStreamSynchronize(c->stream));
        return YOLO_OK;
    }
    if (!c->d_dn_last || c->dn_last_cap < need) {
        if (c->d_dn_last) { HIPCK(c, hipStreamSynchronize(c->stream)); HIPCK(c, hipFree(c->d_dn_last)); c->d_dn_last = nullptr; c->dn_last_cap = 0; }
        HIPCK(c, hipMalloc((void **)&c->d_dn_last, need * 4)); c->dn_last_cap = need;
    }
    const size_t cells = (size_t)L.H * L.W;
    for (int b = 0; b < n; ++b)
        if (L.tree >= 0) HIPCK(c, launch_head_darknet_layout_tree((const float *)P.out.ptr + (size_t)b * cells * P.out.stride, P.out.stride, (int)cells, L.na, L.classes, c->trees[L.tree].dev, c->d_dn_last + (size_t)b * per, c->stream));
        else HIPCK(c, launch_head_darknet_layout((const float *)P.out.ptr + (size_t)b * cells * P.out.stride, P.out.stride, (int)cells, L.na, L.classes, L.type == L_REGION, c->d_dn_last + (size_t)b * per, c->stream));
    HIPCK(c, hipMemcpyAsync(out, c->d_dn_last, need * 4, hipMemcpyDeviceToHost, c->stream)); HIPCK(c, hipStreamSynchronize(c->stream));
    return YOLO_OK;
}

int yolo_last_layer_output(yolo_ctx *c, float *out, size_t out_floats) { return yolo_last_layer_output_batch(c, 1, out, out_floats); }

int yolo_head_raw(yolo_ctx *c, int head, int n, float *out, size_t out_floats)
{
    if (!c || !out || head < 0) return YOLO_ERR_INVALID;
    if (int r = need_detector(c, "yolo_head_raw")) return r;
    if (c->last_n < 1 || n < 1 || n > c->last_n) return fail(c, YOLO_ERR_STATE, "yolo_head_raw of %d images but the last forward ran %d", n, c->last_n);
    int k = 0;
    for (size_t li = 1; li < c->layers.size(); ++li) {
        const Layer &L = c->layers[li];
        if (L.type != L_YOLO && L.type != L_REGION && L.type != L_DETECT) continue;
        if (k++ != head) continue;
        const Layer &P = c->layers[li - 1];
        const size_t px = (size_t)n * P.H * P.W, need = px * P.C;
        if (out_floats < need) return fail(c, YOLO_ERR_INVALID, "output buffer too small (%zu < %zu floats)", out_floats, need);
        if (P.out.dt != DT_F32 || !P.out.ptr) return fail(c, YOLO_ERR_STATE, "internal: head conv output is not fp32");
        HIPCK(c, hipSetDevice(c->device));
        HIPCK(c, hipMemcpy2DAsync(out, (size_t)P.C * 4, P.out.ptr, (size_t)P.out.stride * 4, (size_t)P.C * 4, px, hipMemcpyDeviceToHost, c->stream));
        HIPCK(c, hipStreamSynchronize(c->stream));
        return YOLO_OK;
    }
    return fail(c, YOLO_ERR_INVALID, "no detection head %d", head);
}

int yolo_output_map_geometry(yolo_ctx *c, int *h, int *w, int *ch)
{
    if (!c) return YOLO_ERR_INVALID;
    if (int r = need_map(c, "yolo_output_map_geometry")) return r;
    const Layer &M = c->layers[c->map_layer];
    if (h) *h = M.H; if (w) *w = M.W; if (ch) *ch = M.C;
    return YOLO_OK;
}

int yolo_output_map(yolo_ctx *c, int n, float *out, size_t out_floats)
{
    if (!c || !out) return YOLO_ERR_INVALID;
    if (int r = need_map(c, "yolo_output_map")) return r;
    if (c->last_n < 1 || n < 1 || n > c->last_n) return fail(c, YOLO_ERR_STATE, "yolo_output_map of %d images but the last forward ran %d", n, c->last_n);
    const Layer &M = c->layers[c->map_layer];
    const size_t need = (size_t)n * M.H * M.W * M.C;
    if (out_floats < need) return fail(c, YOLO_ERR_INVALID, "output buffer too small (%zu < %zu floats)", out_floats, need);
    HIPCK(c, hipSetDevice(c->device));
    if (int r = map_to_f32(c, n)) return r;
    return copy_out(c, out, c->d_map_f32, need * 4, YOLO_HOST);
}

int yolo_label_map(yolo_ctx *c, int n, float thresh, uint8_t *labels_u8)
{
    if (!c || !labels_u8) return YOLO_ERR_INVALID;
    if (int r = need_map(c, "yolo_label_map")) return r;
    if (c->last_n < 1 || n < 1 || n > c->last_n) return fail(c, YOLO_ERR_STATE, "yolo_label_map of %d images but the last forward ran %d", n, c->last_n);
    const Layer &M = c->layers[c->map_layer];
    if (M.C > 255) return fail(c, YOLO_ERR_UNSUPPORTED, "yolo_label_map: a map of %d channels (uint8 labels hold at most 255 classes; 255 itself means `below thresh`)", M.C);
    HIPCK(c, hipSetDevice(c->device));
    const size_t npix = (size_t)n * M.H * M.W;
    const float *map = nullptr; int map_stride = 0;
    if (int r = map_f32_view(c, n, &map, &map_stride)) return r;
    if (int r = map_labels_room(c, npix)) return r;
    HIPCK(c, launch_label_map(map, map_stride, npix, M.C, thresh, c->d_map_labels, c->stream));
    return copy_out(c, labels_u8, c->d_map_labels, npix, YOLO_HOST);
}

int yolo_synchronize(yolo_ctx *c) { if (!c) return YOLO_ERR_INVALID; HIPCK(c, hipStreamSynchronize(c->stream)); return YOLO_OK; }

int yolo_layer_output(yolo_ctx *c, int index, int n, float *out, size_t out_floats, int *dims_out)
{
    if (!c) return YOLO_ERR_INVALID;
    if (index < 0 || index >= (int)c->layers.size() || n < 1 || n > c->last_n) return fail(c, YOLO_ERR_INVALID, "bad layer index / n");
    const Layer &L = c->layers[index];
    if (!c->keep_layers) {
        bool kept = L.type == L_CONV && L.storage >= 0 && L.residual_from < -1 && !never_stored(L, index);
        if (kept) for (const Storage &o : c->storages) if (&o != &c->storages[L.storage] && o.phys == c->storages[L.storage].phys && o.def > c->storages[L.storage].def) kept = false;
        if (!kept) return fail(c, YOLO_ERR_STATE, "yolo_layer_output needs keep_layers=1 (without it: only a conv layer's own tensor whose buffer no later layer reuses)");
    }
    if (dims_out) { dims_out[0] = L.H; dims_out[1] = L.W; dims_out[2] = L.C; }
    size_t need = (size_t)n * L.H * L.W * L.C;
    if (!out) return YOLO_OK;
    if (out_floats < need) return fail(c, YOLO_ERR_INVALID, "output buffer too small");
    HIPCK(c, hipSetDevice(c->device));
    float *tmp = nullptr; HIPCK(c, hipMalloc((void **)&tmp, need * 4));
    TView v = L.out; v.n = n;
    float vs = 1.f;
    if (v.dt == DT_FP8) {
        vs = c->eff_scale[index];
        if (vs != vs) { hipFree(tmp); return fail(c, YOLO_ERR_UNSUPPORTED, "layer %d concatenates tensors with different fp8 scales; read its sources", index); }
    }
    hipError_t e = hipSuccess;
    float *wide = nullptr;
    if (L.pair && v.dt == DT_F16) {
        const int cp = roundup(L.C, 32);
        e = hipMalloc((void **)&wide, (size_t)n * L.H * L.W * cp * 4);
        if (e == hipSuccess) e = launch_split_to_f32(v.ptr, v.stride, cp, wide, cp, (size_t)n * L.H * L.W, c->stream);
        v.ptr = wide; v.stride = cp; v.dt = DT_F32;
    }
    if (e == hipSuccess) e = launch_to_f32(v, tmp, c->stream, vs);
    if (e == hipSuccess) e = hipMemcpyAsync(out, tmp, need * 4, hipMemcpyDeviceToHost, c->stream);
    if (e == hipSuccess) e = hipStreamSynchronize(c->stream);
    hipFree(tmp); if (wide) hipFree(wide);
    if (e != hipSuccess) return fail(c, YOLO_ERR_HIP, "layer_output: %s", hipGetErrorString(e));
    return YOLO_OK;
}

}
```

### yolo_tensorflow_amd/csrc/yolo_ctx.h

```cpp
#pragma once
#include "../../include/yolo_hip.h"
#include "kernels.h"

#include <algorithm>
#include <cmath>
#include <cstdarg>
#include <cstdio>
#include <cstdlib>
#include <cstring>
#include <map>
#include <string>
#include <vector>

namespace yolo_impl {

enum LType { L_CONV, L_SHORTCUT, L_ROUTE, L_UPSAMPLE, L_MAXPOOL, L_REORG, L_YOLO, L_REGION, L_DETECT, L_LOCAL, L_AVGPOOL, L_SOFTMAX,
             L_DECONV, L_ACTIVATE, L_L2NORM,
             L_GCONV };
enum ConvKernel { K_TILED, K_HALO, K_S2 };
enum FuseKind { F_NONE, F_STEM, F_PSTEM, F_RESBLOCK, F_C3S2 };

struct Section { std::string type; std::map<std::string, std::string> kv; };

struct Layer {
    LType type;
    int H = 0, W = 0, C = 0;
    std::vector<int> in;
    int filters = 0, size = 0, stride = 1, pad = 0, bn = 0, act = ACT_LINEAR;
    int post_act = ACT_LINEAR;
    bool general = false;
    int cin = 0, cin_pad = 0, kpad = 0, cout_pad = 0;
    void *d_w = nullptr; float *d_b = nullptr; float *d_sc = nullptr;
    void *d_wf = nullptr;
    int in_dt = DT_BF16;
    int store_dt = DT_BF16;
    bool pair = false;
    int tile_cfg = -1;
    int residual_from = -2;
    bool head = false;
    float *d_obj = nullptr;
    int kernel = K_TILED;
    int fused = F_NONE, launcher = -1;
    int fuse_n = 0; bool fuse_ok = false;
    bool fc = false; int fc_h = 0, fc_w = 0, fc_c = 0;
    bool s2d7 = false;
    int side = 0, sqr = 0;
    int tail_layer = -1, fused_into = -1; bool tail_on = false;
    bool noop = false;
    std::vector<int> copy_inputs;
    std::vector<int> copy_offsets;
    int psize = 0, pstride = 0, ppad = 0;
    float up_scale = 1.f;
    bool inplace = false;
    int na = 0, classes = 0, row_off = 0;
    std::vector<float> anchors;
    int groups = 1; float temperature = 1.f; bool pool_fused = false; bool cost = false;
    int tree = -1;
    int storage = -1; int ch_off = 0;
    TView out;
};

struct Tree {
    std::string path, text;
    int n = 0, groups = 0, levels = 0;
    std::vector<int> parent, child, goff, gsize, leaf, order, lvl;
    int *d_all = nullptr; TreeDev dev{};
};

struct Storage { int def = 1 << 30, last = -1; size_t bytes = 0; int phys = -1; int stride = 0; int dt = DT_BF16; bool persistent = false; };


}
using namespace yolo_impl;

struct yolo_ctx {
    std::string err, cfg_text;
    int device = 0;
    hipStream_t stream = nullptr; bool own_stream = false;
    int max_batch = 1, dtype = YOLO_BF16, semantics = YOLO_SEM_TF, decode = YOLO_DECODE_RATIO, keep_layers = 0;
    int in_h = 0, in_w = 0, in_c = 0;
    std::vector<Layer> layers;
    std::vector<Storage> storages;
    std::vector<void *> phys; std::vector<size_t> phys_bytes;
    TView input;
    void *d_zeros = nullptr;
    void *d_stage = nullptr; size_t stage_bytes = 0;
    TView s2d;
    const uint8_t *stem_u8 = nullptr; float stem_scale = 1.f; int stem_u8_n = 0;
    float in_mul = 1.f, in_add = 0.f;
    float *d_det = nullptr; int rows = 0, attrs = 0;
    int cls_layer = -1, cls_topk = 0, cls_mode = 0; int *d_cls_idx = nullptr; float *d_cls_prob = nullptr;
    int map_layer = -1; float *d_map_f32 = nullptr; size_t map_f32_cap = 0; uint8_t *d_map_labels = nullptr; size_t map_labels_cap = 0; unsigned long long *d_label_off = nullptr;
    bool lean_cnt_dirty = false;
    void *d_lean_list = nullptr; unsigned *d_lean_cnt = nullptr;
    float *d_box4 = nullptr; bool lean = false, det_valid = false, lean_ok = false; float lean_thr = 0.f; int lean_heads = 0;
    float *d_scores = nullptr; int *d_labels = nullptr; int *d_cand = nullptr; unsigned long long *d_keys = nullptr;
    float4 *d_sbox = nullptr; int *d_slabel = nullptr; float *d_sscore = nullptr; int rows_pow2 = 0;
    void *d_boxes = nullptr; int *d_counts = nullptr; int boxes_cap = 0;
    int *d_srow = nullptr, *d_rows = nullptr;
    float *d_dn_rec = nullptr; int *d_dn_src = nullptr; int *d_dn_count = nullptr; float *d_dn_last = nullptr; size_t dn_last_cap = 0;
    struct GKey { const void *img; int n, fmt; float scale, st, it; int mo, nm, sm; void *bo, *co; } gkey{};
    hipGraphExec_t gexec = nullptr; int gstate = 0;
    ImgDesc *d_descs = nullptr; void *d_pix = nullptr; size_t pix_cap = 0;
    int geom_fit = -1, geom_n = 0;
    struct GKeyImages { const void *pix; size_t bytes; int n, fit, units; float st, it; int mo, nm, sm; void *bo, *co; } gkey_img;
    hipGraphExec_t gexec_img = nullptr; int gstate_img = 0;
    std::vector<Tree> trees; int tree_head = -1; float hier_thresh = 0.5f, lean_hier = 0.f; int hierarchy_mode = 0; bool tree_full = false;
    int *d_map200 = nullptr;
    bool weights_loaded = false;
    int scores_mode = -1;
    size_t weights_count = 0;
    double conv_flops = 0;
    int last_n = 0;
    std::vector<float> user_scale, eff_scale;
    bool split() const { return dtype == YOLO_FP16X2; }
    bool in_pair = false;
    bool pair_of(int idx) const { return idx < 0 ? in_pair : layers[idx].pair; }
    float *d_f32a = nullptr, *d_f32b = nullptr; size_t f32_cap = 0;
    int act_dt() const { return dtype == YOLO_FP32 ? DT_F32 : dtype == YOLO_FP8 ? DT_FP8 : (dtype == YOLO_FP16 || dtype == YOLO_FP16X2) ? DT_F16 : DT_BF16; }
    bool half_like() const { return dtype == YOLO_BF16 || dtype == YOLO_FP16; }
    int gran() const { return dtype == YOLO_FP8 ? 16 : 8; }
    size_t esize() const { return dt_size(act_dt()); }
};

namespace yolo_impl {

int fail(yolo_ctx *c, int code, const char *fmt, ...);
#define HIPCK(c, expr)                                                                       \
    do { hipError_t e_ = (expr);                                                             \
        if (e_ != hipSuccess) return fail(c, YOLO_ERR_HIP, "%s: %s", #expr, hipGetErrorString(e_)); } while (0)

inline int roundup(int x, int m) { return (x + m - 1) / m * m; }
inline int pair_width(int C) { return 2 * roundup(C, 32); }
inline int gran_of(int dt) { return dt == DT_FP8 ? 16 : 8; }
inline void drop_graph(yolo_ctx *c)
{
    if (c->gexec) { hipGraphExecDestroy(c->gexec); c->gexec = nullptr; } if (c->gstate > 0) c->gstate = 0;
    if (c->gexec_img) { hipGraphExecDestroy(c->gexec_img); c->gexec_img = nullptr; } if (c->gstate_img > 0) c->gstate_img = 0;
}

inline bool fused_may_fall_back(const Layer &L) { return L.fused == F_RESBLOCK || L.fused == F_C3S2; }
inline bool never_stored(const Layer &L, int i) { return L.fused != F_NONE && i < L.launcher; }
inline bool input_never_loaded(const Layer &L, int i) { return L.fused != F_NONE && L.fused != F_PSTEM && i >= L.launcher; }
inline bool fixed_kernel(const Layer &L) { return L.kernel != K_TILED || L.fused != F_NONE; }
inline bool window_check_skipped(const Layer &L, int i) { return L.fused != F_NONE && (!fused_may_fall_back(L) || (L.fused == F_RESBLOCK && i < L.launcher)); }
inline bool rides_as_tail(const yolo_ctx *c, const Layer &L) { return L.fused_into >= 0 && c->layers[L.fused_into].tail_on; }
inline bool issues_launch(const yolo_ctx *c, int i) { const Layer &L = c->layers[i]; return (L.fused == F_NONE || L.launcher == i) && !rides_as_tail(c, L); }

uint16_t f2bf(float f);
uint16_t f2h(float f);
uint8_t f2e4m3(float f);
void pack_conv(const Layer &L, const float *bn_or_bias, const float *w_oihw, int wdt, const float *in_scale,
               std::vector<uint8_t> &wbuf, std::vector<float> &bias, std::vector<float> &osc, int semantics = YOLO_SEM_TF, int split = 0);
void pack_deconv(const Layer &L, const float *bn_or_bias, const float *w_iohw, int wdt, std::vector<uint8_t> &wbuf, std::vector<float> &bias, int semantics = YOLO_SEM_TF);
void pack_gconv(const Layer &L, const float *bn_or_bias, const float *w_oihw, int wdt, std::vector<uint8_t> &wbuf, std::vector<float> &bias, int semantics = YOLO_SEM_TF);
float h2f(uint16_t h);
void resolve_scales(yolo_ctx *c);
void channel_scales(const yolo_ctx *c, int idx, std::vector<float> &out);
int tail_fragments(yolo_ctx *c);
int parse_tree(const std::string &text, Tree &t, std::string &err);
int load_tree(const std::string &path, Tree &t, std::string &err);
std::vector<int> pack_tree(const Tree &t, size_t at[7]);
TreeDev tree_dev(const Tree &t, const int *base, const size_t at[7]);
int upload_tree(yolo_ctx *c, Tree &t);
void free_tree(Tree &t);
int score_tree_rows(yolo_ctx *c, int n);
extern thread_local const std::vector<std::pair<std::string, std::string>> *g_tree_texts;
bool parse_cfg(const char *text, std::vector<Section> &out, std::string &err);
int build_plan(yolo_ctx *c, const std::vector<Section> &secs);
int allocate(yolo_ctx *c);
TView view_of(const yolo_ctx *c, int idx);
ConvArgs conv_args(const yolo_ctx *c, const Layer &L, int n);
DeconvArgs deconv_geometry(int size, int stride, int pad, int h, int w, int cin_pad, int filters, int act, int in_dt);
GConvArgs gconv_geometry(int size, int stride, int pad, int h, int w, int cin, int filters, int groups, int act, int in_dt);
int run_layer(yolo_ctx *c, int i, int n);
int stage_in(yolo_ctx *c, const void *images, int n, int fmt, int loc, float scale);
int run_network(yolo_ctx *c, int n, bool lean = false);
int copy_out(yolo_ctx *c, void *dst, const void *src, size_t bytes, int loc);
int output_layer(const yolo_ctx *c);
int need_detector(yolo_ctx *c, const char *what);
int post_args_ok(yolo_ctx *c, int max_out, int nms_mode, int select_mode);
struct PostGeom { int fit, pixels; };
int post(yolo_ctx *c, const float *det, int n, int rows, int attrs, float score_thr, float iou_thr, int max_out,
         int nms_mode, int select_mode, int img_h, int img_w, int scores_ready, yolo_box *boxes_out, int32_t *counts_out, int out_loc, int32_t *rows_out = nullptr,
         const PostGeom *geom = nullptr);
int need_map(yolo_ctx *c, const char *what);
int map_to_f32(yolo_ctx *c, int n);
int map_f32_view(yolo_ctx *c, int n, const float **map, int *stride);
int map_labels_room(yolo_ctx *c, size_t bytes);
extern thread_local std::string g_op_err;
TView make_view(void *p, int n, int h, int w, int c, int stride, int dt);

}
```

### yolo_tensorflow_amd/csrc/yolo_run.cpp

```cpp
#include "yolo_ctx.h"

namespace yolo_impl {

int fail(yolo_ctx *c, int code, const char *fmt, ...)
{
    char buf[512];
    va_list ap; va_start(ap, fmt); vsnprintf(buf, sizeof buf, fmt, ap); va_end(ap);
    if (c) c->err = buf;
    return code;
}

ConvArgs conv_args(const yolo_ctx *c, const Layer &L, int n)
{
    ConvArgs a; memset(&a, 0, sizeof a);
    TView in = view_of(c, L.in[0]);
    a.in = in.ptr; a.in_stride = in.stride; a.wt = L.d_w; a.bias = L.d_b;
    a.out = L.out.ptr; a.out_stride = L.out.stride; a.out_dt = L.out.dt; a.in_dt = L.in_dt; a.oscale = L.d_sc;
    if (L.pair || (c->split() && L.out.dt == DT_F32)) a.split = 1;
    a.pairk = L.in[0] >= 0 && c->pair_of(L.in[0]) ? 1 : 0;
    a.out_inv_scale = 1.f; a.res_scale = 1.f; a.mid_scale = 1.f; a.mid_inv_scale = 1.f;
    const int li = (int)(&L - c->layers.data());
    if (L.residual_from >= -1) { TView r = view_of(c, L.residual_from); a.res = r.ptr; a.res_stride = r.stride; }
    if (L.tail_on && L.tail_layer >= 0 && c->layers[L.tail_layer].in_dt == L.in_dt && (L.in_dt == DT_FP8 || c->layers[L.tail_layer].d_wf)) {
        const Layer &T = c->layers[L.tail_layer];
// ... 51 lines not shown
{
    const TView in = view_of(c, L.in[0]);
    GConvArgs a = gconv_geometry(L.size, L.stride, L.pad, in.h, in.w, L.cin, L.filters, L.groups, L.act, L.in_dt);
    a.in = in.ptr; a.in_stride = in.stride; a.wt = L.d_w; a.bias = L.d_b; a.out = L.out.ptr; a.out_stride = L.out.stride; a.out_dt = L.out.dt; a.N = n;
    a.Cstore = std::min(L.out.stride, roundup(L.filters, L.out.dt == DT_F32 && L.head ? 4 : 8));
    return a;
}

static int via_f32(yolo_ctx *c, const Layer &L, int n, int kind)
{
    hipStream_t s = c->stream;
    const TView in = view_of(c, L.in[0]);
    const int cpi = roundup(in.c, 32), cpo = roundup(L.C, 32);
    const size_t pin = (size_t)n * in.h * in.w, pout = (size_t)n * L.H * L.W;
    if (pin * cpi > c->f32_cap || pout * cpo > c->f32_cap) return fail(c, YOLO_ERR_STATE, "internal: fp32 staging too small");
    HIPCK(c, launch_split_to_f32(in.ptr, in.stride, cpi, c->d_f32a, cpi, pin, s));
    TView a; a.ptr = c->d_f32a; a.n = n; a.h = in.h; a.w = in.w; a.c = cpi; a.stride = cpi; a.dt = DT_F32;
    TView b; b.ptr = c->d_f32b; b.n = n; b.h = L.H; b.w = L.W; b.c = cpo; b.stride = cpo; b.dt = DT_F32;
    if (kind == 0) HIPCK(c, launch_upsample2x(a, b, c->semantics == YOLO_SEM_TF, s));
    else if (kind == 1) HIPCK(c, launch_maxpool(a, b, L.psize, L.pstride, L.ppad, s));
    else {
        a.c = in.c; b.c = L.C;
        if (in.c % 32 || L.C % 32) return fail(c, YOLO_ERR_UNSUPPORTED, "reorg of a pair tensor of %d channels (whole 32-channel groups only)", in.c);
        HIPCK(c, launch_reorg(a, b, L.pstride, c->semantics == YOLO_SEM_DARKNET, s));
    }
    HIPCK(c, launch_split_from_f32(c->d_f32b, cpo, L.out.ptr, L.out.stride, cpo, pout, s));
    return YOLO_OK;
}

static StemPairArgs stem_pair_args(const yolo_ctx *c, int l, int n)
{
    const Layer &A = c->layers[0], &L = c->layers[l]; StemPairArgs t; memset(&t, 0, sizeof t);
    t.in = c->input.ptr; t.w0 = A.d_w; t.b0 = A.d_b; t.Kpad0 = A.kpad; t.C0 = A.filters; t.act0 = A.act;
    t.in_u8 = c->stem_u8; t.in_scale = c->stem_scale; t.in_mul = c->in_mul; t.in_add = c->in_add;
    t.w1 = L.d_w; t.b1 = L.d_b; t.Kpad1 = L.kpad; t.act1 = L.act;
    t.out = L.out.ptr; t.out_stride = L.out.stride; t.N = n; t.H = A.H; t.W = A.W; t.Ho = L.H; t.Wo = L.W;
    return t;
}
static StemArgs stem_args(const yolo_ctx *c, int l, int n)
{
    const Layer &A = c->layers[0], &L = c->layers[l]; StemArgs t; memset(&t, 0, sizeof t);
    t.in = c->input.ptr; t.in_stride = c->input.stride;
    t.in_u8 = c->stem_u8; t.in_scale = c->stem_scale; t.in_mul = c->in_mul; t.in_add = c->in_add;
    t.w0 = A.d_w; t.b0 = A.d_b; t.Kpad0 = A.kpad; t.C0 = A.filters; t.act0 = A.act;
    t.w1 = L.d_w; t.b1 = L.d_b; t.Kpad1 = L.kpad; t.C1 = L.filters; t.act1 = L.act;
    if (l + 1 < (int)c->layers.size() && c->layers[l + 1].fused == L.fused) { const Layer &T = c->layers[l + 1];
        t.w2 = T.d_w; t.b2 = T.d_b; t.Kpad2 = T.kpad; t.C2 = T.filters; t.act2 = T.act; t.out2 = T.out.ptr; t.out2_stride = T.out.stride;
    }
    t.out = L.out.ptr; t.out_stride = L.out.stride; t.N = n; t.H = A.H; t.W = A.W; t.Ho = L.H; t.Wo = L.W; t.zeros = c->d_zeros; t.dt = L.in_dt;
    return t;
}
static BlockArgs block_args(const yolo_ctx *c, int l, int n)
{
    const Layer &A = c->layers[l - 1], &B = c->layers[l]; const TView x = view_of(c, A.in[0]); BlockArgs b; memset(&b, 0, sizeof b);
    b.x = x.ptr; b.x_stride = x.stride; b.w1 = A.d_w; b.b1 = A.d_b; b.Kpad1 = A.kpad; b.act1 = A.act;
    b.w2 = B.d_w; b.b2 = B.d_b; b.Kpad2 = B.kpad; b.act2 = B.act; b.out = B.out.ptr; b.out_stride = B.out.stride;
    b.N = n; b.H = B.H; b.W = B.W; b.C = B.filters; b.Cmid = A.filters; b.dt = B.in_dt;
    return b;
}
static C3S2Args c3s2_args(const yolo_ctx *c, int l, int n)
{
    const Layer &A = c->layers[l - 2], &B = c->layers[l]; const TView x = view_of(c, A.in[0]), r = view_of(c, A.residual_from); C3S2Args t; memset(&t, 0, sizeof t);
    t.in = x.ptr; t.in_stride = x.stride; t.w3 = A.d_w; t.b3 = A.d_b; t.Kpad3 = A.kpad; t.act3 = A.act; t.res = r.ptr; t.res_stride = r.stride;
    t.w5 = B.d_w; t.b5 = B.d_b; t.Kpad5 = B.kpad; t.act5 = B.act; t.out = B.out.ptr; t.out_stride = B.out.stride;
    t.N = n; t.H = A.H; t.W = A.W; t.dt = B.in_dt;
    return t;
}
static HaloArgs halo_args(const ConvArgs &a, const Layer &L, int n)
{
    HaloArgs h; memset(&h, 0, sizeof h);
    h.in = a.in; h.in_stride = a.in_stride; h.w = a.wt; h.b = a.bias; h.Kpad = a.Kpad; h.Cin = L.cin; h.Cout = L.filters; h.act = L.act;
    h.res = a.res; h.res_stride = a.res_stride; h.out = a.out; h.out_stride = a.out_stride; h.N = n; h.H = a.H; h.W = a.W; h.dt = L.in_dt;
    return h;
}

static bool fused_launch_applies(yolo_ctx *c, const Layer &L, int n)
{
    if (!fused_may_fall_back(L)) return L.fused != F_NONE;
    Layer &G = c->layers[L.launcher]; const int l = L.launcher;
    if (G.fuse_n != n) { G.fuse_ok = L.fused == F_RESBLOCK ? conv_resblock_ok(block_args(c, l, n)) : conv_c3s2_ok(c3s2_args(c, l, n)); G.fuse_n = n; }
    return G.fuse_ok;
}

static int run_conv(yolo_ctx *c, int i, int n)
{
    Layer &L = c->layers[i];
    hipStream_t s = c->stream;
    auto nview = [&](TView v) { v.n = n; return v; };
    if (fused_launch_applies(c, L, n)) {
        if (i == L.launcher) switch (L.fused) {
        case F_STEM: { StemArgs t = stem_args(c, i, n); HIPCK(c, launch_conv_stem(t, s)); break; }
        case F_PSTEM: { StemPairArgs t = stem_pair_args(c, i, n); if (c->input.stride != 24 || !conv_stem_pair_ok(t)) return fail(c, YOLO_ERR_STATE, "layer %d: the fused split-fp16 stem does not apply to this plan", i);
            HIPCK(c, launch_conv_stem_pair(t, s)); break; }
        case F_RESBLOCK: { BlockArgs b = block_args(c, i, n); HIPCK(c, launch_conv_resblock(b, s)); break; }
        case F_C3S2: { C3S2Args t = c3s2_args(c, i, n); HIPCK(c, launch_conv_c3s2(t, s)); break; }
        }
        return YOLO_OK;
    }
    if (rides_as_tail(c, L)) return YOLO_OK;
    ConvArgs a = conv_args(c, L, n);
    if (L.tail_on && !a.w2) return fail(c, YOLO_ERR_STATE, "layer %d: the plan folds the 1x1 conv %d into this layer, but its filters are not available in the producer's operand type", i, L.tail_layer);
    if (L.s2d7) HIPCK(c, launch_reorg(nview(c->input), nview(c->s2d), 2, 0, s));
    if (L.kernel != K_TILED) {
        HaloArgs h = halo_args(a, L, n);
        if (L.kernel == K_HALO && conv_halo_ok(h)) { HIPCK(c, launch_conv_halo(h, s)); return YOLO_OK; }
        if (L.kernel == K_S2 && conv_s2_ok(h)) { HIPCK(c, launch_conv_s2(h, s)); return YOLO_OK; }
    }
    if (c->dtype == YOLO_FP32) { HIPCK(c, launch_conv_f32(a, s)); return YOLO_OK; }
    const int cfg = conv_resolve_cfg(a, L.tile_cfg);
    if (a.w2 && !a.split && !a.pairk && !conv_cfg_tail_ok(cfg, a.Cout, a.in_dt == DT_FP8, a.tail_f32 != 0)) return fail(c, YOLO_ERR_STATE, "layer %d: tile config %d cannot run the fused 1x1 tail", i, cfg);
    HIPCK(c, a.in_dt == DT_FP8 ? launch_conv_fp8(a, cfg, s) : launch_conv_bf16(a, cfg, s));
    return YOLO_OK;
}

static int run_decode(yolo_ctx *c, int i, int n)
{
    const Layer &L = c->layers[i];
    hipStream_t s = c->stream;
    if (L.tree < 0 && c->lean && c->lean_thr > 0.f && c->lean_heads >= 1 && c->lean_heads <= 4) {
        bool later_head = false;
        for (size_t k = i + 1; k < c->layers.size(); ++k) later_head |= c->layers[k].type == L_YOLO;
        if (later_head) return YOLO_OK;
        LeanArgs la; memset(&la, 0, sizeof la);
        long begin = 0;
        for (size_t k = 0; k < c->layers.size(); ++k) {
            const Layer &Y = c->layers[k];
            if (Y.type != L_YOLO) continue;
            const Layer &P = c->layers[k - 1];
            LeanHead &h = la.h[la.nheads++];
            h.raw = (const float *)P.out.ptr; h.obj = P.d_obj; h.raw_stride = P.out.stride; h.gh = Y.H; h.gw = Y.W; h.na = Y.na; h.row_off = Y.row_off; h.box_begin = begin;
            const int stride[2] = {c->in_w / Y.W, c->in_h / Y.H};
            h.sx = (float)stride[0]; h.sy = (float)stride[1];
            for (int q = 0; q < 2 * Y.na; ++q) h.anchors[q] = (float)(1.0 * (double)Y.anchors[q] / (double)stride[q & 1]);
            begin += (long)n * Y.H * Y.W * Y.na;
        }
        la.total = begin; la.n = n; la.classes = L.classes; la.mode = c->decode; la.rows_total = c->rows;
        la.box4 = c->d_box4; la.reject_below = c->lean_thr; la.list = (uint4 *)c->d_lean_list; la.list_count = c->d_lean_cnt; la.list_cap = (unsigned)((size_t)c->max_batch * c->rows);
        if (c->lean_cnt_dirty) HIPCK(c, hipMemsetAsync(c->d_lean_cnt, 0, 4, s));
        c->lean_cnt_dirty = true;
        HIPCK(c, launch_decode_lean(la, c->d_scores, c->d_labels, s));
        return YOLO_OK;
    }
    const Layer &P = c->layers[i - 1];
    DecodeArgs d; memset(&d, 0, sizeof d);
    d.raw = (const float *)P.out.ptr; d.raw_stride = P.out.stride; d.n = n; d.gh = L.H; d.gw = L.W; d.na = L.na; d.classes = L.classes;
    d.img_h = c->in_h; d.img_w = c->in_w; d.mode = c->decode; d.region = L.type == L_REGION;
    const int stride[2] = {c->in_w / L.W, c->in_h / L.H};
    for (int k = 0; k < 2 * L.na; ++k) d.anchors[k] = L.type == L_YOLO ? (float)(1.0 * (double)L.anchors[k] / (double)stride[k & 1]) : L.anchors[k];
    d.det = c->lean ? nullptr : c->d_det; d.box4 = c->lean ? c->d_box4 : nullptr; d.rows_total = c->rows; d.row_off = L.row_off;
    d.reject_below = c->lean ? c->lean_thr : -INFINITY;
    if (L.tree < 0) HIPCK(c, launch_decode(d, c->d_scores, c->d_labels, s));
    else if (c->lean) { HIPCK(c, launch_decode_region_tree_lean(d, c->trees[L.tree].dev, c->hier_thresh, c->d_scores, c->d_labels, s)); c->lean_hier = c->hier_thresh; }
    else HIPCK(c, launch_decode_region_tree(d, c->trees[L.tree].dev, s));
    return YOLO_OK;
}

int run_layer(yolo_ctx *c, int i, int n)
{
    Layer &L = c->layers[i];
    hipStream_t s = c->stream;
    auto nview = [&](TView v) { v.n = n; return v; };
    switch (L.type) {
    case L_CONV:
        if (int r = run_conv(c, i, n)) return r;
        if (L.post_act != ACT_LINEAR) HIPCK(c, launch_activate(nview(L.out), L.pair, L.post_act, s));
        break;
    case L_SHORTCUT:
        if (L.general) {
            HIPCK(c, launch_shortcut(nview(view_of(c, L.in[0])), nview(view_of(c, L.in[1])), nview(L.out), L.pair, L.act, s));
        } else if (!L.noop && L.pair) {
            HIPCK(c, launch_add_split(view_of(c, L.in[0]).ptr, view_of(c, L.in[0]).stride, view_of(c, L.in[1]).ptr, view_of(c, L.in[1]).stride, L.out.ptr, L.out.stride, roundup(L.C, 32), (size_t)n * L.H * L.W, s));
        } else if (!L.noop) {
            float sa = 1.f, sb = 1.f, so = 1.f;
            if (c->dtype == YOLO_FP8) { sa = c->eff_scale[L.in[0]]; sb = c->eff_scale[L.in[1]]; so = 1.f / c->eff_scale[i]; }
            HIPCK(c, launch_add(nview(view_of(c, L.in[0])), nview(view_of(c, L.in[1])), nview(L.out), s, sa, sb, so));
        }
        break;
    case L_ROUTE:
        for (size_t k = 0; k < L.copy_inputs.size(); ++k) {
            TView src = nview(view_of(c, L.copy_inputs[k])); TView dst = nview(L.out);
            dst.ptr = (char *)dst.ptr + (size_t)L.copy_offsets[k] * dt_size(dst.dt); dst.c = src.c;
            if (src.c % 8) return fail(c, YOLO_ERR_UNSUPPORTED, "route copy of %d channels", src.c);
            if (L.pair) {
                if (src.c % 32 || L.copy_offsets[k] % 32) return fail(c, YOLO_ERR_UNSUPPORTED, "route copy of a pair tensor: %d channels at offset %d (whole 32-channel groups only)", src.c, L.copy_offsets[k]);
                TView dv = nview(L.out);
                dv.ptr = (char *)L.out.ptr + (size_t)2 * L.copy_offsets[k] * 2; dv.c = 2 * src.c; src.c = 2 * src.c;
                HIPCK(c, launch_copy(src, dv, s));
                continue;
            }
            HIPCK(c, launch_copy(src, dst, s));
        }
        break;
    case L_LOCAL:
        HIPCK(c, launch_local(nview(view_of(c, L.in[0])), nview(L.out), L.d_w, L.d_b, L.size, L.stride, L.pad, L.act, s));
// ... 215 lines not shown
    if (e == hipSuccess && c->in_pair) e = launch_split_from_f32(c->d_f32a, 8, c->input.ptr, 24, 8, (size_t)c->in_h * c->in_w, c->stream, PAIR_B3);
    int r = e == hipSuccess ? run_network(c, 1) : fail(c, YOLO_ERR_HIP, "resize: %s", hipGetErrorString(e));
    if (tmp) { hipStreamSynchronize(c->stream); hipFree(tmp); }
    if (r) return r;
    if (det_out) return copy_out(c, det_out, c->d_det, (size_t)c->rows * c->attrs * 4, out_loc);
    return YOLO_OK;
}

int yolo_forward_letterbox_chw(yolo_ctx *c, const float *image_chw, int w, int h, int loc, float *det_out, int out_loc)
{
    if (!c) return YOLO_ERR_INVALID;
    if (!c->weights_loaded) return fail(c, YOLO_ERR_STATE, "yolo_forward_letterbox_chw before weights were loaded");
    if (!image_chw || h < 1 || w < 1) return fail(c, YOLO_ERR_INVALID, "bad image");
    HIPCK(c, hipSetDevice(c->device));
    const float *src = image_chw; void *tmp = nullptr;
    if (loc == YOLO_HOST) {
        HIPCK(c, hipMalloc(&tmp, (size_t)h * w * 3 * 4));
        HIPCK(c, hipMemcpyAsync(tmp, image_chw, (size_t)h * w * 3 * 4, hipMemcpyHostToDevice, c->stream)); src = (const float *)tmp;
    }
    c->stem_u8 = nullptr;
    hipError_t e = c->in_pair ? launch_letterbox_chw(src, w, h, c->in_h, c->in_w, c->d_f32a, DT_F32, 8, c->stream) : launch_letterbox_chw(src, w, h, c->in_h, c->in_w, c->input.ptr, c->input.dt, 8, c->stream);
    if (e == hipSuccess && c->in_pair) e = launch_split_from_f32(c->d_f32a, 8, c->input.ptr, 24, 8, (size_t)c->in_h * c->in_w, c->stream, PAIR_B3);
    int r = e == hipSuccess ? run_network(c, 1) : fail(c, YOLO_ERR_HIP, "letterbox: %s", hipGetErrorString(e));
    if (tmp) { hipStreamSynchronize(c->stream); hipFree(tmp); }
    if (r) return r;
    if (det_out) return copy_out(c, det_out, c->d_det, (size_t)c->rows * c->attrs * 4, out_loc);
    return YOLO_OK;
}

static int postprocess_impl(yolo_ctx *c, int n, float score_thr, float iou_thr, int max_out, int nms_mode, int select_mode,
                            yolo_box *boxes_out, int32_t *counts_out, int32_t *rows_out, int out_loc, const PostGeom *geom)
{
    if (int r = need_detector(c, "yolo_postprocess")) return r;
    if (n < 1 || n > c->last_n) return fail(c, YOLO_ERR_STATE, "postprocess of %d images but the last forward ran %d", n, c->last_n);
    HIPCK(c, hipSetDevice(c->device));
    if (c->tree_head >= 0) {
        if (nms_mode == YOLO_NMS_NUMPY_V3) return fail(c, YOLO_ERR_UNSUPPORTED, "YOLO_NMS_NUMPY_V3 over a softmax-tree head");
        if (!c->det_valid && (score_thr < c->lean_thr || c->hier_thresh != c->lean_hier))
            return fail(c, YOLO_ERR_STATE, "the last forward ran through yolo_detect* with score threshold %g and hier_thresh %g; other values need yolo_forward", c->lean_thr, c->lean_hier);
        if (c->det_valid) if (int r = score_tree_rows(c, n)) return r;
        c->scores_mode = 2;
        return post(c, c->d_det, n, c->rows, c->attrs, score_thr, iou_thr, max_out, nms_mode, select_mode,
                    nms_mode == YOLO_NMS_PER_CLASS ? c->in_h : 0, nms_mode == YOLO_NMS_PER_CLASS ? c->in_w : 0, 1, boxes_out, counts_out, out_loc, rows_out, geom);
    }
    const int want = nms_mode == YOLO_NMS_NUMPY_V3 ? 1 : 0;
    if (!c->det_valid && score_thr < c->lean_thr)
        return fail(c, YOLO_ERR_STATE, "the last forward ran through yolo_detect* with score threshold %g and pruned the scores below it; a lower threshold needs yolo_forward", c->lean_thr);
    if (!c->det_valid && want != c->scores_mode)
        return fail(c, YOLO_ERR_STATE, "the last forward ran through yolo_detect* without materialising the decoded tensor; this NMS flavour needs it (call yolo_forward)");
    const int ready = c->scores_mode == want;
    c->scores_mode = want;
    return post(c, c->d_det, n, c->rows, c->attrs, score_thr, iou_thr, max_out, nms_mode, select_mode,
                nms_mode == YOLO_NMS_PER_CLASS ? c->in_h : 0, nms_mode == YOLO_NMS_PER_CLASS ? c->in_w : 0, ready, boxes_out, counts_out, out_loc, rows_out, geom);
}

int yolo_postprocess_rows(yolo_ctx *c, int n, float score_thr, float iou_thr, int max_out, int nms_mode, int select_mode,
                          yolo_box *boxes_out, int32_t *counts_out, int32_t *rows_out, int out_loc)
{
    if (!c) return YOLO_ERR_INVALID;
    return postprocess_impl(c, n, score_thr, iou_thr, max_out, nms_mode, select_mode, boxes_out, counts_out, rows_out, out_loc, nullptr);
}

int yolo_postprocess(yolo_ctx *c, int n, float score_thr, float iou_thr, int max_out, int nms_mode, int select_mode,
                     yolo_box *boxes_out, int32_t *counts_out, int out_loc)
{
    return yolo_postprocess_rows(c, n, score_thr, iou_thr, max_out, nms_mode, select_mode, boxes_out, counts_out, nullptr, out_loc);
}

int yolo_detect(yolo_ctx *c, const void *images, int n, int fmt, int loc, float scale, float score_thr, float iou_thr,
                int max_out, int nms_mode, int select_mode, yolo_box *boxes_out, int32_t *counts_out, int out_loc)
{
    if (!c) return YOLO_ERR_INVALID;
    if (int r = post_args_ok(c, max_out, nms_mode, select_mode)) return r;
    int r = forward_impl(c, images, n, fmt, loc, scale, nullptr, YOLO_DEVICE, nms_mode != YOLO_NMS_NUMPY_V3, score_thr); if (r) return r;
    return yolo_postprocess(c, n, score_thr, iou_thr, max_out, nms_mode, select_mode, boxes_out, counts_out, out_loc);
}

int yolo_detect_graph(yolo_ctx *c, const void *images, int n, int fmt, float scale, float score_thr, float iou_thr, int max_out,
                      int nms_mode, int select_mode, yolo_box *boxes_out, int32_t *counts_out)
{
    if (!c) return YOLO_ERR_INVALID;
    if (!images || !boxes_out || !counts_out) return fail(c, YOLO_ERR_INVALID, "yolo_detect_graph needs device pointers for images, boxes_out and counts_out");
    yolo_ctx::GKey k{images, n, fmt, scale, score_thr, iou_thr, max_out, nms_mode, select_mode, (void *)boxes_out, (void *)counts_out};
    if (memcmp(&k, &c->gkey, sizeof k) != 0) {
        if (c->gexec) { hipGraphExecDestroy(c->gexec); c->gexec = nullptr; }
        c->gkey = k; if (c->gstate >= 0) c->gstate = 0;
    }
    if (int r = post_args_ok(c, max_out, nms_mode, select_mode)) return r;
    auto eager = [&]() -> int {
        int r = forward_impl(c, images, n, fmt, YOLO_DEVICE, scale, nullptr, YOLO_DEVICE, nms_mode != YOLO_NMS_NUMPY_V3, score_thr); if (r) return r;
        return yolo_postprocess(c, n, score_thr, iou_thr, max_out, nms_mode, select_mode, boxes_out, counts_out, YOLO_DEVICE);
    };
    if (c->gstate <= 0) { int r = eager(); if (r == YOLO_OK && c->gstate == 0) c->gstate = 1; return r; }
    HIPCK(c, hipSetDevice(c->device));
    if (c->gstate == 1) {
        hipGraph_t g = nullptr;
        if (hipStreamBeginCapture(c->stream, hipStreamCaptureModeThreadLocal) != hipSuccess) { (void)hipGetLastError(); c->gstate = -1; return eager(); }
        int r = eager();
        hipError_t e = hipStreamEndCapture(c->stream, &g);
        if (r != YOLO_OK || e != hipSuccess || !g) { (void)hipGetLastError(); if (g) hipGraphDestroy(g); c->gstate = -1; return r ? r : eager(); }
        e = hipGraphInstantiate(&c->gexec, g, nullptr, nullptr, 0);
        hipGraphDestroy(g);
        if (e != hipSuccess) { (void)hipGetLastError(); c->gexec = nullptr; c->gstate = -1; return eager(); }
        c->gstate = 2;
    }
    if (c->lean_cnt_dirty) { HIPCK(c, hipMemsetAsync(c->d_lean_cnt, 0, 4, c->stream)); c->lean_cnt_dirty = false; }
    HIPCK(c, hipGraphLaunch(c->gexec, c->stream));
    c->lean = nms_mode != YOLO_NMS_NUMPY_V3 && c->lean_ok; c->det_valid = !c->lean; c->lean_thr = score_thr;
    c->last_n = n; c->scores_mode = nms_mode == YOLO_NMS_NUMPY_V3 ? 1 : 0;
    return YOLO_OK;
}

static_assert(sizeof(ImgDesc) == sizeof(yolo_image_desc) && sizeof(yolo_image_desc) == 16, "yolo_image_desc is the device table's row");

static int images_check(yolo_ctx *c, const void *pixels, size_t bytes, const yolo_image_desc *descs, int n, int fit)
{
    if (!c->weights_loaded) return fail(c, YOLO_ERR_STATE, "forward of images before weights were loaded");
    if (n < 1 || n > c->max_batch) return fail(c, YOLO_ERR_INVALID, "batch %d outside 1..%d", n, c->max_batch);
    if (!pixels || !descs) return fail(c, YOLO_ERR_INVALID, "pixels / descs == NULL");
    if (fit < YOLO_FIT_STRETCH || fit > YOLO_FIT_CV2_BGR) return fail(c, YOLO_ERR_INVALID, "bad fit %d", fit);
    if (bytes < 3 || bytes > 0xffffffffull) return fail(c, YOLO_ERR_INVALID, "packed buffer of %zu bytes (3 .. 2^32 - 1)", bytes);
    for (int i = 0; i < n; ++i) {
        const yolo_image_desc &d = descs[i];
        if (d.h < 1 || d.w < 1) return fail(c, YOLO_ERR_INVALID, "image %d: %d x %d", i, (int)d.h, (int)d.w);
        const uint64_t need = (uint64_t)d.h * (uint64_t)d.w * 3u;
        if (d.offset > bytes || need > bytes - d.offset)
            return fail(c, YOLO_ERR_INVALID, "image %d: %d x %d x 3 bytes at offset %llu end past the %zu-byte buffer", i, (int)d.h, (int)d.w, (unsigned long long)d.offset, bytes);
        if (fit == YOLO_FIT_LETTERBOX) {
            int nw, nh; letterbox_dims(c->in_w, c->in_h, d.w, d.h, &nw, &nh);
            if (nw < 1 || nh < 1) return fail(c, YOLO_ERR_INVALID, "image %d: %d x %d letterboxes to less than one pixel", i, (int)d.h, (int)d.w);
        }
    }
    return YOLO_OK;
}

static int detect_images_check(yolo_ctx *c, int fit, int max_out, int nms_mode, int select_mode, int units)
{
    if (int r = post_args_ok(c, max_out, nms_mode, select_mode)) return r;
    if (units != YOLO_UNITS_NETWORK && units != YOLO_UNITS_SOURCE_PIXELS) return fail(c, YOLO_ERR_INVALID, "bad units %d", units);
    if (fit == YOLO_FIT_LETTERBOX)
        for (auto &L : c->layers) if (L.type == L_DETECT) return fail(c, YOLO_ERR_UNSUPPORTED, "letterbox box mapping of a [detection] head (darknet v1 does not letterbox)");
    return YOLO_OK;
}

static int images_step(yolo_ctx *c, const uint8_t *pixels, size_t bytes, const yolo_image_desc *descs, int n, int fit, bool upload, bool lean, float score_thr)
{
    c->lean_thr = score_thr;
    if (upload) HIPCK(c, hipMemcpyAsync(c->d_descs, descs, (size_t)n * sizeof(ImgDesc), hipMemcpyHostToDevice, c->stream));
    c->stem_u8 = nullptr;
    if (c->in_pair) {
        HIPCK(c, launch_fit_images(pixels, bytes, c->d_descs, n, fit, c->in_h, c->in_w, c->d_f32a, DT_F32, 8, c->in_mul, c->in_add, c->stream));
        HIPCK(c, launch_split_from_f32(c->d_f32a, 8, c->input.ptr, 24, 8, (size_t)n * c->in_h * c->in_w, c->stream, PAIR_B3));
    } else HIPCK(c, launch_fit_images(pixels, bytes, c->d_descs, n, fit, c->in_h, c->in_w, c->input.ptr, c->input.dt, 8, c->in_mul, c->in_add, c->stream));
    if (int r = run_network(c, n, lean)) return r;
    c->geom_fit = fit; c->geom_n = n;
    return YOLO_OK;
}

static int forward_images_impl(yolo_ctx *c, const uint8_t *pixels, size_t bytes, const yolo_image_desc *descs, int n, int fit, int loc,
                               float *det_out, int out_loc, bool lean, float score_thr)
{
    if (int r = images_check(c, pixels, bytes, descs, n, fit)) return r;
    HIPCK(c, hipSetDevice(c->device));
    const uint8_t *src = pixels;
    if (loc == YOLO_HOST) {
        if (bytes > c->pix_cap) {
            HIPCK(c, hipStreamSynchronize(c->stream));
            if (c->d_pix) HIPCK(c, hipFree(c->d_pix));
            c->d_pix = nullptr; c->pix_cap = 0;
            HIPCK(c, hipMalloc(&c->d_pix, bytes)); c->pix_cap = bytes;
        }
        HIPCK(c, hipMemcpyAsync(c->d_pix, pixels, bytes, hipMemcpyHostToDevice, c->stream));
        src = (const uint8_t *)c->d_pix;
    }
    if (int r = images_step(c, src, bytes, descs, n, fit, true, lean && !det_out, score_thr)) return r;
    if (det_out) return copy_out(c, det_out, c->d_det, (size_t)n * c->rows * c->attrs * 4, out_loc);
    return YOLO_OK;
}

int yolo_forward_images_u8(yolo_ctx *c, const uint8_t *pixels, size_t bytes, const yolo_image_desc *descs, int n, int fit, int loc,
                           float *det_out, int out_loc)
{
    if (!c) return YOLO_ERR_INVALID;
    return forward_images_impl(c, pixels, bytes, descs, n, fit, loc, det_out, out_loc, false, 0.f);
}

int yolo_detect_images_u8(yolo_ctx *c, const uint8_t *pixels, size_t bytes, const yolo_image_desc *descs, int n, int fit, int loc,
                          float score_thr, float iou_thr, int max_out, int nms_mode, int select_mode, int units,
                          yolo_box *boxes_out, int32_t *counts_out, int out_loc)
{
    if (!c) return YOLO_ERR_INVALID;
    if (int r = detect_images_check(c, fit, max_out, nms_mode, select_mode, units)) return r;
    if (int r = forward_images_impl(c, pixels, bytes, descs, n, fit, loc, nullptr, YOLO_DEVICE, nms_mode != YOLO_NMS_NUMPY_V3, score_thr)) return r;
    const PostGeom g{fit, units == YOLO_UNITS_SOURCE_PIXELS};
    return postprocess_impl(c, n, score_thr, iou_thr, max_out, nms_mode, select_mode, boxes_out, counts_out, nullptr, out_loc, &g);
}

int yolo_detect_images_graph(yolo_ctx *c, const uint8_t *pixels, size_t bytes, const yolo_image_desc *descs, int n, int fit,
                             float score_thr, float iou_thr, int max_out, int nms_mode, int select_mode, int units,
                             yolo_box *boxes_out, int32_t *counts_out)
{
    if (!c) return YOLO_ERR_INVALID;
    if (!pixels || !boxes_out || !counts_out) return fail(c, YOLO_ERR_INVALID, "yolo_detect_images_graph needs device pointers for pixels, boxes_out and counts_out");
    if (int r = detect_images_check(c, fit, max_out, nms_mode, select_mode, units)) return r;
    if (int r = images_check(c, pixels, bytes, descs, n, fit)) return r;
    yolo_ctx::GKeyImages k; memset(&k, 0, sizeof k);
    k.pix = pixels; k.bytes = bytes; k.n = n; k.fit = fit; k.units = units; k.st = score_thr; k.it = iou_thr; k.mo = max_out; k.nm = nms_mode; k.sm = select_mode;
    k.bo = (void *)boxes_out; k.co = (void *)counts_out;
    if (memcmp(&k, &c->gkey_img, sizeof k) != 0) {
        if (c->gexec_img) { hipGraphExecDestroy(c->gexec_img); c->gexec_img = nullptr; }
        c->gkey_img = k; if (c->gstate_img >= 0) c->gstate_img = 0;
    }
    HIPCK(c, hipSetDevice(c->device));
    HIPCK(c, hipMemcpyAsync(c->d_descs, descs, (size_t)n * sizeof(ImgDesc), hipMemcpyHostToDevice, c->stream));
    const PostGeom g{fit, units == YOLO_UNITS_SOURCE_PIXELS};
    const bool lean = nms_mode != YOLO_NMS_NUMPY_V3;
    auto eager = [&]() -> int {
        if (int r = images_step(c, pixels, bytes, descs, n, fit, false, lean, score_thr)) return r;
        return postprocess_impl(c, n, score_thr, iou_thr, max_out, nms_mode, select_mode, boxes_out, counts_out, nullptr, YOLO_DEVICE, &g);
    };
    if (c->gstate_img <= 0) { int r = eager(); if (r == YOLO_OK && c->gstate_img == 0) c->gstate_img = 1; return r; }
    if (c->gstate_img == 1) {
        hipGraph_t gr = nullptr;
        if (hipStreamBeginCapture(c->stream, hipStreamCaptureModeThreadLocal) != hipSuccess) { (void)hipGetLastError(); c->gstate_img = -1; return eager(); }
        int r = eager();
        hipError_t e = hipStreamEndCapture(c->stream, &gr);
        if (r != YOLO_OK || e != hipSuccess || !gr) { (void)hipGetLastError(); if (gr) hipGraphDestroy(gr); c->gstate_img = -1; return r ? r : eager(); }
        e = hipGraphInstantiate(&c->gexec_img, gr, nullptr, nullptr, 0);
        hipGraphDestroy(gr);
        if (e != hipSuccess) { (void)hipGetLastError(); c->gexec_img = nullptr; c->gstate_img = -1; return eager(); }
        c->gstate_img = 2;
    }
    if (c->lean_cnt_dirty) { HIPCK(c, hipMemsetAsync(c->d_lean_cnt, 0, 4, c->stream)); c->lean_cnt_dirty = false; }
    HIPCK(c, hipGraphLaunch(c->gexec_img, c->stream));
    c->lean = lean && c->lean_ok; c->det_valid = !c->lean; c->lean_thr = score_thr;
    c->last_n = n; c->scores_mode = nms_mode == YOLO_NMS_NUMPY_V3 ? 1 : 0; c->stem_u8 = nullptr; c->geom_fit = fit; c->geom_n = n;
    return YOLO_OK;
}

static int classify_check(yolo_ctx *c, int top_k, const int32_t *classes_out, const float *probs_out)
{
    if (c->map_layer >= 0) return fail(c, YOLO_ERR_INVALID, "yolo_classify: the network is a map network ([net] yolo_output=map); use yolo_output_map / yolo_label_map");
    if (c->cls_layer < 0) return fail(c, YOLO_ERR_INVALID, "yolo_classify: the network is a detector (its output layer is not a [softmax])");
    const Layer &L = c->layers[c->cls_layer];
    if (top_k < 0 || top_k > CLS_TOPK_MAX || top_k > L.C) return fail(c, YOLO_ERR_INVALID, "top_k %d outside 0..%d", top_k, L.C < CLS_TOPK_MAX ? L.C : CLS_TOPK_MAX);
    if (top_k > 0 && L.groups != 1) return fail(c, YOLO_ERR_INVALID, "top_k needs a [softmax] with groups=1 (this one has groups=%d)", L.groups);
    if (!probs_out || (top_k > 0 && !classes_out)) return fail(c, YOLO_ERR_INVALID, "classes_out / probs_out == NULL");
    return YOLO_OK;
}

static int classify_out(yolo_ctx *c, int n, int top_k, int32_t *classes_out, float *probs_out, int out_loc)
{
    const Layer &L = c->layers[c->cls_layer];
    if (top_k == 0) return copy_out(c, probs_out, L.out.ptr, (size_t)n * L.C * 4, out_loc);
    if (int r = copy_out(c, classes_out, c->d_cls_idx, (size_t)n * top_k * 4, out_loc)) return r;
    return copy_out(c, probs_out, c->d_cls_prob, (size_t)n * top_k * 4, out_loc);
}

int yolo_classify(yolo_ctx *c, const void *images, int n, int fmt, int loc, float scale, int top_k, int32_t *classes_out, float *probs_out, int out_loc)
{
    if (!c) return YOLO_ERR_INVALID;
    if (int r = classify_check(c, top_k, classes_out, probs_out)) return r;
    c->cls_topk = top_k; c->cls_mode = c->hierarchy_mode;
    const int r = forward_impl(c, images, n, fmt, loc, scale, nullptr, YOLO_DEVICE, false);
    c->cls_topk = 0; c->cls_mode = 0;
    if (r) return r;
    return classify_out(c, n, top_k, classes_out, probs_out, out_loc);
}

int yolo_classify_images_u8(yolo_ctx *c, const uint8_t *pixels, size_t bytes, const yolo_image_desc *descs, int n, int fit, int loc, int top_k,
                            int32_t *classes_out, float *probs_out, int out_loc)
{
    if (!c) return YOLO_ERR_INVALID;
    if (int r = classify_check(c, top_k, classes_out, probs_out)) return r;
    c->cls_topk = top_k; c->cls_mode = c->hierarchy_mode;
    const int r = forward_images_impl(c, pixels, bytes, descs, n, fit, loc, nullptr, YOLO_DEVICE, false, 0.f);
    c->cls_topk = 0; c->cls_mode = 0;
    if (r) return r;
    return classify_out(c, n, top_k, classes_out, probs_out, out_loc);
}

int yolo_segment_images_u8(yolo_ctx *c, const uint8_t *pixels, const yolo_image_desc *descs, int n, int fit, float thresh, uint8_t *labels_u8,
                           const uint64_t *label_offsets)
{
    if (!c) return YOLO_ERR_INVALID;
    if (int r = need_map(c, "yolo_segment_images_u8")) return r;
    if (!labels_u8) return fail(c, YOLO_ERR_INVALID, "labels_u8 == NULL");
    const Layer &M = c->layers[c->map_layer];
    if (M.C > 255) return fail(c, YOLO_ERR_UNSUPPORTED, "yolo_segment_images_u8: a map of %d channels (uint8 labels hold at most 255 classes)", M.C);
    if (!descs || n < 1 || n > c->max_batch) return fail(c, YOLO_ERR_INVALID, "batch %d outside 1..%d", n, c->max_batch);
    size_t bytes = 0, total = 0;
    std::vector<unsigned long long> off(n);
    for (int i = 0; i < n; ++i) {
        if (descs[i].h < 1 || descs[i].w < 1) return fail(c, YOLO_ERR_INVALID, "image %d: %d x %d", i, (int)descs[i].h, (int)descs[i].w);
        const size_t px = (size_t)descs[i].h * (size_t)descs[i].w;
        bytes = std::max(bytes, (size_t)descs[i].offset + px * 3);
        off[i] = label_offsets ? label_offsets[i] : total;
        total = std::max(total, (size_t)off[i] + px);
    }
    if (int r = forward_images_impl(c, pixels, bytes, descs, n, fit, YOLO_HOST, nullptr, YOLO_DEVICE, false, 0.f)) return r;
    if (!c->d_label_off) HIPCK(c, hipMalloc((void **)&c->d_label_off, (size_t)c->max_batch * 8));
    HIPCK(c, hipMemcpyAsync(c->d_label_off, off.data(), (size_t)n * 8, hipMemcpyHostToDevice, c->stream));
    const float *map = nullptr; int map_stride = 0;
    if (int r = map_f32_view(c, n, &map, &map_stride)) return r;
    if (int r = map_labels_room(c, total)) return r;
    if (label_offsets) HIPCK(c, hipMemsetAsync(c->d_map_labels, 0, total, c->stream));
    HIPCK(c, launch_segment_labels(map, map_stride, M.H, M.W, M.C, thresh, c->d_descs, c->d_label_off, n, fit, c->in_h, c->in_w, c->d_map_labels, c->stream));
    return copy_out(c, labels_u8, c->d_map_labels, total, YOLO_HOST);
}

float yolo_fit_unit_value(int fit, int value)
{
    if (fit < YOLO_FIT_STRETCH || fit > YOLO_FIT_CV2_BGR || value < 0 || value > 255) return NAN;
    return fit_unit_value(fit, (unsigned)value);
}

namespace { struct EventSet {
    std::vector<hipEvent_t> e; bool ok = true;
    explicit EventSet(int n) { e.reserve(n); for (int i = 0; i < n; ++i) { hipEvent_t x; if (hipEventCreate(&x) != hipSuccess) { ok = false; break; } e.push_back(x); } }
    ~EventSet() { for (auto x : e) hipEventDestroy(x); }
    EventSet(const EventSet &) = delete; EventSet &operator=(const EventSet &) = delete;
}; }

int yolo_time_forward(yolo_ctx *c, int n, int iters, float *total_ms, float *conv_ms)
{
    if (!c) return YOLO_ERR_INVALID;
    if (!c->weights_loaded) return fail(c, YOLO_ERR_STATE, "weights not loaded");
    if (n < 1 || n > c->max_batch || iters < 1) return fail(c, YOLO_ERR_INVALID, "bad n/iters");
    HIPCK(c, hipSetDevice(c->device));
    EventSet evs(2); if (!evs.ok) return fail(c, YOLO_ERR_HIP, "hipEventCreate failed");
    hipEvent_t e0 = evs.e[0], e1 = evs.e[1];
    c->lean = false;
    if (c->stem_u8 && n > c->stem_u8_n) c->stem_u8 = nullptr;
    if (total_ms) {
        HIPCK(c, hipEventRecord(e0, c->stream));
        for (int it = 0; it < iters; ++it) { int r = run_network(c, n); if (r) return r; }
        HIPCK(c, hipEventRecord(e1, c->stream)); HIPCK(c, hipEventSynchronize(e1));
        float ms = 0; HIPCK(c, hipEventElapsedTime(&ms, e0, e1)); *total_ms = ms / iters;
    }
    if (conv_ms) {
        float all_ms = 0, rest_ms = 0;
        for (int pass = 0; pass < 2; ++pass) {
            HIPCK(c, hipEventRecord(e0, c->stream));
            for (int it = 0; it < iters; ++it) { int r = run_layers(c, n, pass == 1); if (r) return r; }
            HIPCK(c, hipEventRecord(e1, c->stream)); HIPCK(c, hipEventSynchronize(e1));
            float ms = 0; HIPCK(c, hipEventElapsedTime(&ms, e0, e1)); (pass == 0 ? all_ms : rest_ms) = ms / iters;
        }
        *conv_ms = all_ms - rest_ms;
        c->last_n = n; c->scores_mode = 0; c->det_valid = true;
    }
    return YOLO_OK;
}

int yolo_time_layers(yolo_ctx *c, int n, int iters, float *ms_out)
{
    if (!c || !ms_out) return YOLO_ERR_INVALID;
    if (!c->weights_loaded) return fail(c, YOLO_ERR_STATE, "weights not loaded");
    if (n < 1 || n > c->max_batch || iters < 1) return fail(c, YOLO_ERR_INVALID, "bad n/iters");
    HIPCK(c, hipSetDevice(c->device));
    const int NL = (int)c->layers.size();
    c->lean = false; c->det_valid = true;
    if (c->stem_u8 && n > c->stem_u8_n) c->stem_u8 = nullptr;
    EventSet evs(NL + 1); if (!evs.ok) return fail(c, YOLO_ERR_HIP, "hipEventCreate failed");
    std::vector<hipEvent_t> &ev = evs.e;
    std::vector<double> acc(NL, 0.0);
    for (int it = 0; it < iters; ++it) {
        HIPCK(c, hipEventRecord(ev[0], c->stream));
        for (int i = 0; i < NL; ++i) { int r = run_layer(c, i, n); if (r) return r; HIPCK(c, hipEventRecord(ev[i + 1], c->stream)); }
        HIPCK(c, hipStreamSynchronize(c->stream));
        for (int i = 0; i < NL; ++i) { float ms = 0; HIPCK(c, hipEventElapsedTime(&ms, ev[i], ev[i + 1])); acc[i] += ms; }
    }
    for (int i = 0; i < NL; ++i) ms_out[i] = (float)(acc[i] / iters);
    c->last_n = n;
    return YOLO_OK;
}

}
```

### yolo_tensorflow_amd/hip.py

```python
import ctypes as C
import os
import numpy as np

_HERE = os.path.dirname(os.path.abspath(__file__))
LIB_OVERRIDE = os.environ.get("YOLO_HIP_LIB") or None
LIB_PATH = LIB_OVERRIDE or os.path.join(_HERE, "libyolo_hip.so")

BF16, FP32, FP8, FP16, FP16X2 = 0, 1, 2, 3, 4
SEM_TF, SEM_DARKNET = 0, 1
DECODE_RATIO, DECODE_PIXEL = 0, 1
HOST, DEVICE = 0, 1
IMG_U8, IMG_F32, IMG_F32_CHW = 0, 1, 2
NMS_TF, NMS_PER_CLASS, NMS_DARKNET, NMS_NUMPY_V3, NMS_TF_V1 = 0, 1, 2, 3, 4
SELECT_GT, SELECT_GE = 0, 1
FIT_STRETCH, FIT_LETTERBOX, FIT_CV2, FIT_CV2_BGR = 0, 1, 2, 3
UNITS_NETWORK, UNITS_SOURCE_PIXELS = 0, 1

BOX_DTYPE = np.dtype([("x0", "<f4"), ("y0", "<f4"), ("x1", "<f4"), ("y1", "<f4"), ("score", "<f4"), ("cls", "<i4")])
DESC_DTYPE = np.dtype([("offset", "<u8"), ("h", "<i4"), ("w", "<i4")])


class ImageDesc(C.Structure):
    _fields_ = [("offset", C.c_uint64), ("h", C.c_int32), ("w", C.c_int32)]

EXPORTS = [
    "yolo_create", "yolo_destroy", "yolo_last_error", "yolo_load_darknet_weights", "yolo_set_weights",
    "yolo_weights_count", "yolo_set_act_scales", "yolo_export", "yolo_create_from_file", "yolo_input_size", "yolo_num_rows", "yolo_num_attrs", "yolo_num_layers", "yolo_head_geometry", "yolo_head_geometry_hw", "yolo_op_decode_hw", "yolo_op_resize_u8_hw",
    "yolo_conv_flops", "yolo_conv_bytes", "yolo_forward", "yolo_forward_image_u8", "yolo_postprocess",
    "yolo_detect", "yolo_detect_graph", "yolo_synchronize", "yolo_layer_output", "yolo_time_forward", "yolo_time_layers",
    "yolo_autotune", "yolo_get_tile_configs", "yolo_set_tile_configs", "yolo_op_conv2d", "yolo_op_conv_num_cfgs", "yolo_op_upsample2x", "yolo_op_reorg",
    "yolo_darknet_boxes", "yolo_last_layer_size", "yolo_last_layer_output", "yolo_op_letterbox",
    "yolo_op_maxpool", "yolo_op_resize_u8", "yolo_op_detections_boxes", "yolo_op_nms_detections", "yolo_forward_letterbox_chw", "yolo_op_decode", "yolo_op_postprocess",
    "yolo_postprocess_rows", "yolo_op_postprocess_rows", "yolo_last_layer_output_batch", "yolo_head_raw", "yolo_calibrate", "yolo_calibrate_copy", "yolo_op_resize_cv2",
    "yolo_forward_images_u8", "yolo_detect_images_u8", "yolo_detect_images_graph", "yolo_fit_unit_value", "yolo_darknet_boxes_at",
    "yolo_num_classes", "yolo_classify", "yolo_classify_images_u8", "yolo_op_avgpool", "yolo_op_softmax",
    "yolo_set_hier_thresh", "yolo_set_hierarchy_mode", "yolo_darknet_boxes_map", "yolo_tree_geometry", "yolo_tree_read", "yolo_plan_check", "yolo_plan_table",
    "yolo_op_tree_softmax", "yolo_op_tree_top", "yolo_activation_code", "yolo_op_activate", "yolo_op_shortcut",
    "yolo_output_map_geometry", "yolo_output_map", "yolo_label_map", "yolo_segment_images_u8", "yolo_op_deconv2d", "yolo_op_l2norm", "yolo_op_upsample", "yolo_op_label_map",
    "yolo_op_conv2d_grouped",
]
HIER_CONDITIONAL, HIER_ABSOLUTE, HIER_LEAVES = 0, 1, 2
_HIER_MODES = {None: HIER_CONDITIONAL, "conditional": HIER_CONDITIONAL, "absolute": HIER_ABSOLUTE, "leaves": HIER_LEAVES}
DIST_EXPORTS = ["yolo_shard_bounds", "yolo_dist_flat_words", "yolo_dist_split_records", "yolo_dist_unique_id", "yolo_dist_create",
                "yolo_dist_detect", "yolo_dist_detect_async", "yolo_dist_destroy"]


class YoloError(RuntimeError):
    pass


class _Config(C.Structure):
    _fields_ = [("struct_size", C.c_uint32), ("cfg_text", C.c_char_p), ("max_batch", C.c_int32),
                ("dtype", C.c_int32), ("semantics", C.c_int32), ("decode", C.c_int32), ("device", C.c_int32),
                ("keep_layers", C.c_int32), ("stream", C.c_void_p)]


_lib = None


def load_library():
    global _lib
    if _lib is not None:
        return _lib
    if not os.path.exists(LIB_PATH):
        raise YoloError("%s is missing -- build it with `python -c 'import __graft_entry__ as g; g.build()'` "
                        "(or `make -C yolo_tensorflow_amd/csrc`); there is no CPU fallback" % LIB_PATH)
    l = C.CDLL(LIB_PATH)
    P, I, F, D = C.c_void_p, C.c_int, C.c_float, C.c_double
    FP = C.POINTER(C.c_float)
    l.yolo_create.argtypes = [C.POINTER(_Config), C.c_char_p, C.c_size_t]; l.yolo_create.restype = P
    l.yolo_destroy.argtypes = [P]; l.yolo_destroy.restype = None
    l.yolo_last_error.argtypes = [P]; l.yolo_last_error.restype = C.c_char_p
    l.yolo_load_darknet_weights.argtypes = [P, C.c_char_p, I]
    l.yolo_set_weights.argtypes = [P, FP, C.c_size_t]
    l.yolo_weights_count.argtypes = [P]; l.yolo_weights_count.restype = C.c_size_t
    l.yolo_set_act_scales.argtypes = [P, P, I]
    l.yolo_head_geometry.argtypes = [P, I, P, P, P, P]
    l.yolo_head_geometry_hw.argtypes = [P, I, P, P, P, P, P]
    l.yolo_export.argtypes = [P, C.c_char_p]
    l.yolo_create_from_file.argtypes = [C.c_char_p, I, I, P, I, C.c_char_p, C.c_size_t]; l.yolo_create_from_file.restype = P
    l.yolo_input_size.argtypes = [P, C.POINTER(I), C.POINTER(I), C.POINTER(I)]
    for n in ("yolo_num_rows", "yolo_num_attrs", "yolo_num_layers", "yolo_synchronize", "yolo_num_classes"):
        getattr(l, n).argtypes = [P]
    l.yolo_conv_flops.argtypes = [P]; l.yolo_conv_flops.restype = D
    l.yolo_conv_bytes.argtypes = [P, I]; l.yolo_conv_bytes.restype = D
    l.yolo_forward.argtypes = [P, P, I, I, I, F, P, I]
    l.yolo_forward_image_u8.argtypes = [P, P, I, I, I, P, I]
    l.yolo_postprocess.argtypes = [P, I, F, F, I, I, I, P, P, I]
    l.yolo_detect.argtypes = [P, P, I, I, I, F, F, F, I, I, I, P, P, I]
    l.yolo_detect_graph.argtypes = [P, P, I, I, F, F, F, I, I, I, P, P]
    l.yolo_layer_output.argtypes = [P, I, I, P, C.c_size_t, C.POINTER(I)]
    l.yolo_time_forward.argtypes = [P, I, I, FP, FP]
    l.yolo_time_layers.argtypes = [P, I, I, FP]
    l.yolo_autotune.argtypes = [P, I, I]
    l.yolo_get_tile_configs.argtypes = [P, P]
    l.yolo_set_tile_configs.argtypes = [P, P]
    l.yolo_op_conv2d.argtypes = [P, I, I, I, I, P, P, I, I, I, I, P, P, I, I, I]
    l.yolo_op_conv_num_cfgs.argtypes = []
    l.yolo_op_upsample2x.argtypes = [P, I, I, I, I, I, P, I]
    l.yolo_op_reorg.argtypes = [P, I, I, I, I, I, I, P, I]
    l.yolo_op_maxpool.argtypes = [P, I, I, I, I, I, I, P, I]
    l.yolo_op_resize_u8.argtypes = [P, I, I, I, F, P, I]
    l.yolo_op_resize_u8_hw.argtypes = [P, I, I, I, I, F, P, I]
    l.yolo_op_detections_boxes.argtypes = [P, I, I, I, P, I]
    l.yolo_op_nms_detections.argtypes = [P, P, P, I, I, F, I, I]
    l.yolo_forward_letterbox_chw.argtypes = [P, P, I, I, I, P, I]
    l.yolo_op_decode.argtypes = [P, I, I, I, I, P, I, I, I, P, I]
    l.yolo_op_decode_hw.argtypes = [P, I, I, I, I, I, P, I, I, I, I, P, I]
    l.yolo_darknet_boxes.argtypes = [P, I, I, F, I, P, I, P]
    l.yolo_last_layer_size.argtypes = [P]; l.yolo_last_layer_size.restype = C.c_size_t
    l.yolo_last_layer_output.argtypes = [P, P, C.c_size_t]
    l.yolo_op_letterbox.argtypes = [P, I, I, I, I, I, P, I]
    l.yolo_op_postprocess.argtypes = [P, I, I, I, F, F, I, I, I, P, P, I]
    l.yolo_op_postprocess_rows.argtypes = [P, I, I, I, F, F, I, I, I, P, P, P, I]
    l.yolo_postprocess_rows.argtypes = [P, I, F, F, I, I, I, P, P, P, I]
    l.yolo_last_layer_output_batch.argtypes = [P, I, P, C.c_size_t]
    l.yolo_head_raw.argtypes = [P, I, I, P, C.c_size_t]
    l.yolo_calibrate.argtypes = [I, P, I, C.c_double, FP, FP]
    l.yolo_calibrate_copy.argtypes = [I, P, C.c_double, FP]
    l.yolo_op_resize_cv2.argtypes = [P, I, I, I, I, I, F, P, I]
    SZ = C.c_size_t
    l.yolo_forward_images_u8.argtypes = [P, P, SZ, P, I, I, I, P, I]
    l.yolo_detect_images_u8.argtypes = [P, P, SZ, P, I, I, I, F, F, I, I, I, I, P, P, I]
    l.yolo_detect_images_graph.argtypes = [P, P, SZ, P, I, I, F, F, I, I, I, I, P, P]
    l.yolo_fit_unit_value.argtypes = [I, I]; l.yolo_fit_unit_value.restype = F
    l.yolo_darknet_boxes_at.argtypes = [P, I, I, I, F, I, P, I, P]
    l.yolo_classify.argtypes = [P, P, I, I, I, F, I, P, P, I]
    l.yolo_classify_images_u8.argtypes = [P, P, SZ, P, I, I, I, I, P, P, I]
    l.yolo_op_avgpool.argtypes = [P, I, I, I, I, I, P, I]
    l.yolo_op_softmax.argtypes = [P, I, I, I, F, I, P, P, P, I]
    l.yolo_set_hier_thresh.argtypes = [P, F]
    l.yolo_set_hierarchy_mode.argtypes = [P, I]
    l.yolo_darknet_boxes_map.argtypes = [P, I, I, I, F, I, P, P, I, P]
    l.yolo_tree_geometry.argtypes = [P, P, P, P, P, P, P, P]
    l.yolo_tree_read.argtypes = [C.c_char_p, P, P, P, P, P, P, P, C.c_char_p, SZ]
    l.yolo_plan_check.argtypes = [C.c_char_p, I, C.c_char_p, SZ]
    l.yolo_plan_table.argtypes = [C.c_char_p, I, I, I, C.c_char_p, SZ, C.c_char_p, SZ]
    l.yolo_op_tree_softmax.argtypes = [P, I, I, C.c_char_p, F, I, P, I]
    l.yolo_op_tree_top.argtypes = [P, I, C.c_char_p, F, P, I]
    l.yolo_activation_code.argtypes = [C.c_char_p]
    l.yolo_op_activate.argtypes = [P, I, I, I, I, I, I, P, I]
    l.yolo_op_shortcut.argtypes = [P, I, I, I, I, P, I, I, I, I, I, P, I]
    l.yolo_output_map_geometry.argtypes = [P, C.POINTER(I), C.POINTER(I), C.POINTER(I)]
    l.yolo_output_map.argtypes = [P, I, P, SZ]
    l.yolo_label_map.argtypes = [P, I, F, P]
    l.yolo_segment_images_u8.argtypes = [P, P, P, I, I, F, P, P]
    l.yolo_op_deconv2d.argtypes = [P, I, I, I, I, P, P, I, I, I, I, I, I, I, P, I]
    l.yolo_op_conv2d_grouped.argtypes = [P, I, I, I, I, P, P, I, I, I, I, I, I, I, I, P, I]
    l.yolo_op_l2norm.argtypes = [P, I, I, I, I, I, P, I]
    l.yolo_op_upsample.argtypes = [P, I, I, I, I, I, F, I, P, I]
    l.yolo_op_label_map.argtypes = [P, I, I, I, I, F, P, I]
    l.yolo_shard_bounds.argtypes = [I, I, I, C.POINTER(I), C.POINTER(I)]
    l.yolo_dist_flat_words.argtypes = [I, I]; l.yolo_dist_flat_words.restype = C.c_size_t
    l.yolo_dist_split_records.argtypes = [P, I, I, I, P, P]
    l.yolo_dist_unique_id.argtypes = [P]
    l.yolo_dist_create.argtypes = [P, I, I, P, P, I, I, C.c_char_p, C.c_size_t]; l.yolo_dist_create.restype = P
    l.yolo_dist_detect.argtypes = [P, P, I, F, F, F, I, I, P, P]
    l.yolo_dist_detect_async.argtypes = [P, P, I, F, F, F, I, I, C.POINTER(P)]
    l.yolo_dist_destroy.argtypes = [P]; l.yolo_dist_destroy.restype = None
    _lib = l
    return l


def _ptr(a):
    if a is None:
        return None, HOST
    if isinstance(a, int):
        return C.c_void_p(a), DEVICE
    if isinstance(a, np.ndarray):
        if not a.flags["C_CONTIGUOUS"]:
            raise YoloError("array must be C-contiguous")
        return C.c_void_p(a.ctypes.data), HOST
    if hasattr(a, "data_ptr"):
        if not a.is_contiguous():
            raise YoloError("tensor must be contiguous")
        return C.c_void_p(a.data_ptr()), (DEVICE if a.is_cuda else HOST)
    raise YoloError("unsupported buffer type %r" % type(a))


def _op_check(rc, what):
    if rc != 0:
        msg = load_library().yolo_last_error(None)
        raise YoloError("%s failed (%d): %s" % (what, rc, msg.decode() if msg else ""))


_warned_legacy = False
HIP_STREAM_LEGACY = 1


def pack_images(images):
    arrs = []
    for i, im in enumerate(images):
        a = np.ascontiguousarray(im)
        if a.dtype != np.uint8 or a.ndim != 3 or a.shape[2] != 3 or a.shape[0] < 1 or a.shape[1] < 1:
            raise YoloError("image %d: need a uint8 [h, w, 3] array, got %s %s" % (i, a.dtype, a.shape))
        arrs.append(a)
    if not arrs:
        raise YoloError("pack_images: no images")
    descs = np.zeros(len(arrs), dtype=DESC_DTYPE)
    off = 0
# ... 88 lines not shown
        for t in tensors:
            if hasattr(t, "is_cuda") and t.is_cuda:
                import torch
                torch.cuda.current_stream(t.device).synchronize()
                return

    def close(self):
        if getattr(self, "ctx", None):
            self.lib.yolo_destroy(self.ctx)
            self.ctx = None

    def __del__(self):
        try:
            self.close()
        except Exception:
            pass

    def weights_count(self):
        return self.lib.yolo_weights_count(self.ctx)

    def set_act_scales(self, scales):
        sc = np.ascontiguousarray(scales, dtype=np.float32)
        self._check(self.lib.yolo_set_act_scales(self.ctx, sc.ctypes.data, sc.size), "yolo_set_act_scales")

    def load_weights(self, path, header_ints=0):
        self._check(self.lib.yolo_load_darknet_weights(self.ctx, os.fsencode(path), header_ints), "yolo_load_darknet_weights")

    def set_weights(self, flat):
        flat = np.ascontiguousarray(flat, dtype=np.float32)
        self._check(self.lib.yolo_set_weights(self.ctx, flat.ctypes.data_as(C.POINTER(C.c_float)), flat.size), "yolo_set_weights")

    def forward(self, images, scale=1.0 / 255.0, want_detections=True, n=None, fmt=None, out=None):
        p, loc = _ptr(images)
        self._last_image = images if loc == DEVICE else None
        self._order_after_producer(images, out)
        if n is None:
            n = int(images.shape[0])
        if fmt is None:
            fmt = IMG_U8 if str(images.dtype).endswith("uint8") else IMG_F32
        det = None
        dp, dloc = None, HOST
        if out is not None:
            dp, dloc = _ptr(out)
        elif want_detections:
            det = np.empty((n, self.rows, self.attrs), dtype=np.float32)
            dp, dloc = _ptr(det)
        self._check(self.lib.yolo_forward(self.ctx, p, n, fmt, loc, scale, dp, dloc), "yolo_forward")
        return det

    def forward_image(self, image_u8):
        image_u8 = np.ascontiguousarray(image_u8, dtype=np.uint8)
        det = np.empty((1, self.rows, self.attrs), dtype=np.float32)
        self._check(self.lib.yolo_forward_image_u8(self.ctx, image_u8.ctypes.data, image_u8.shape[0], image_u8.shape[1],
                                                   HOST, det.ctypes.data, HOST), "yolo_forward_image_u8")
        return det

    def postprocess(self, n, score_thr=0.5, iou_thr=0.5, max_out=20, nms_mode=NMS_TF, select_mode=SELECT_GT,
                    boxes_out=None, counts_out=None, rows_out=None, return_rows=False):
        if boxes_out is not None:
            bp, bloc = _ptr(boxes_out); cp, _ = _ptr(counts_out); rp, _ = _ptr(rows_out)
            self._order_after_producer(boxes_out, counts_out, rows_out)
            self._check(self.lib.yolo_postprocess_rows(self.ctx, n, score_thr, iou_thr, max_out, nms_mode, select_mode, bp, cp, rp, bloc), "yolo_postprocess")
            return None
        boxes = np.zeros((n, max_out), dtype=BOX_DTYPE); counts = np.zeros(n, dtype=np.int32)
        rows = np.full((n, max_out), -1, dtype=np.int32) if return_rows else None
        self._check(self.lib.yolo_postprocess_rows(self.ctx, n, score_thr, iou_thr, max_out, nms_mode, select_mode,
                                                   boxes.ctypes.data, counts.ctypes.data, rows.ctypes.data if return_rows else None, HOST), "yolo_postprocess")
        recs = [boxes[i, :counts[i]].copy() for i in range(n)]
        if return_rows:
            return recs, [rows[i, :counts[i]].copy() for i in range(n)]
        return recs

    def head_geometry(self, head):
        kind, gh, gw, na, off = C.c_int(), C.c_int(), C.c_int(), C.c_int(), C.c_int()
        self._check(self.lib.yolo_head_geometry_hw(self.ctx, head, C.byref(kind), C.byref(gh), C.byref(gw), C.byref(na), C.byref(off)), "yolo_head_geometry_hw")
        return {"kind": kind.value, "grid_h": gh.value, "grid_w": gw.value, "anchors": na.value, "row_offset": off.value}

    def head_raw(self, head, n):
        g = self.head_geometry(head)
        out = np.empty((n, g["grid_h"], g["grid_w"], g["anchors"] * self.attrs), dtype=np.float32)
        self._check(self.lib.yolo_head_raw(self.ctx, head, n, out.ctypes.data, out.size), "yolo_head_raw")
        return out

    def last_layer_output(self, n=1):
        self.lib.yolo_last_layer_size.restype = C.c_size_t
        per = self.lib.yolo_last_layer_size(self.ctx)
        out = np.empty((n, per), dtype=np.float32)
        self._check(self.lib.yolo_last_layer_output_batch(self.ctx, n, out.ctypes.data, out.size), "yolo_last_layer_output_batch")
        return out

    def set_hier_thresh(self, hier_thresh):
        self._check(self.lib.yolo_set_hier_thresh(self.ctx, float(hier_thresh)), "yolo_set_hier_thresh")

    def set_hierarchy_mode(self, mode):
        self._check(self.lib.yolo_set_hierarchy_mode(self.ctx, _HIER_MODES[mode] if mode in _HIER_MODES else int(mode)), "yolo_set_hierarchy_mode")

    def tree_geometry(self):
        n, g = C.c_int32(0), C.c_int32(0)
        self._check(self.lib.yolo_tree_geometry(self.ctx, C.byref(n), C.byref(g), None, None, None, None, None), "yolo_tree_geometry")
        if n.value == 0:
            return None
        a = {k: np.zeros(n.value if k in ("parent", "child", "leaf") else g.value, dtype=np.int32) for k in ("parent", "child", "group_offset", "group_size", "leaf")}
        self._check(self.lib.yolo_tree_geometry(self.ctx, None, None, a["parent"].ctypes.data, a["child"].ctypes.data, a["group_offset"].ctypes.data,
                                                a["group_size"].ctypes.data, a["leaf"].ctypes.data), "yolo_tree_geometry")
        a.update(n=n.value, groups=g.value)
        return a

    def detect(self, images, scale=1.0 / 255.0, hier_thresh=None, **kw):
        if hier_thresh is not None:
            self.set_hier_thresh(hier_thresh)
        self.forward(images, scale=scale, want_detections=False)
        return self.postprocess(int(images.shape[0]), **kw)

    def detect_fused(self, images, scale=1.0 / 255.0, hier_thresh=None, **kw):
        if hier_thresh is not None:
            self.set_hier_thresh(hier_thresh)
        p, loc = _ptr(images)
        self._last_image = images if loc == DEVICE else None
        self._order_after_producer(images)
        n = int(images.shape[0])
        fmt = IMG_U8 if str(images.dtype).endswith("uint8") else IMG_F32
        a = dict(score_thr=0.5, iou_thr=0.5, max_out=20, nms_mode=NMS_TF, select_mode=SELECT_GT); a.update(kw)
        boxes = np.zeros((n, a["max_out"]), dtype=BOX_DTYPE); counts = np.zeros(n, dtype=np.int32)
        self._check(self.lib.yolo_detect(self.ctx, p, n, fmt, loc, scale, a["score_thr"], a["iou_thr"], a["max_out"], a["nms_mode"], a["select_mode"],
                                         boxes.ctypes.data, counts.ctypes.data, HOST), "yolo_detect")
        return [boxes[i, :counts[i]].copy() for i in range(n)]

    def detect_graph(self, images, boxes_out, counts_out, scale=1.0 / 255.0, score_thr=0.5, iou_thr=0.5, max_out=20,
                     nms_mode=NMS_TF, select_mode=SELECT_GT, hier_thresh=None):
        if hier_thresh is not None:
            self.set_hier_thresh(hier_thresh)
        p, loc = _ptr(images); bp, bl = _ptr(boxes_out); cp, cl = _ptr(counts_out)
        if loc != DEVICE or bl != DEVICE or cl != DEVICE:
            raise YoloError("detect_graph needs device-resident buffers")
        self._last_image = images
        self._order_after_producer(images, boxes_out, counts_out)
        fmt = IMG_U8 if str(images.dtype).endswith("uint8") else IMG_F32
        self._check(self.lib.yolo_detect_graph(self.ctx, p, int(images.shape[0]), fmt, scale, score_thr, iou_thr, max_out,
                                               nms_mode, select_mode, bp, cp), "yolo_detect_graph")

    def _packed(self, images):
        if isinstance(images, tuple):
            buf, descs = images
        else:
            buf, descs = pack_images(images)
        descs = _descs(descs)
        p, loc = _ptr(buf)
        nbytes = int(buf.numel()) if hasattr(buf, "numel") else int(buf.nbytes)
        return buf, descs, p, loc, nbytes

    def forward_images(self, images, fit=FIT_STRETCH, want_detections=True):
        buf, descs, p, loc, nbytes = self._packed(images)
        n = len(descs)
        self._order_after_producer(buf)
        det = np.empty((n, self.rows, self.attrs), dtype=np.float32) if want_detections else None
        self._check(self.lib.yolo_forward_images_u8(self.ctx, p, nbytes, descs.ctypes.data, n, fit, loc,
                                                    det.ctypes.data if det is not None else None, HOST), "yolo_forward_images_u8")
        return det

    def detect_images(self, images, fit=FIT_STRETCH, units=UNITS_NETWORK, score_thr=0.5, iou_thr=0.5, max_out=20, nms_mode=NMS_TF,
                      select_mode=SELECT_GT, hier_thresh=None):
        if hier_thresh is not None:
            self.set_hier_thresh(hier_thresh)
        buf, descs, p, loc, nbytes = self._packed(images)
        n = len(descs)
        self._order_after_producer(buf)
# ... 469 lines not shown
```

Measured before the change: 12570 img/s.

## Store only objectness-passing rows from detection head convs in lean detect mode

```diff
diff --git a/include/yolo_hip.h b/include/yolo_hip.h
--- a/include/yolo_hip.h
+++ b/include/yolo_hip.h
@@ -118,6 +118,7 @@
 int yolo_last_layer_output_batch(yolo_ctx *ctx, int n, float *out, size_t out_floats);
 
 int yolo_head_raw(yolo_ctx *ctx, int head, int n, float *out, size_t out_floats);
+int yolo_head_sparse(const yolo_ctx *ctx, int head);
 
 int yolo_postprocess(yolo_ctx *ctx, int n, float score_thr, float iou_thr, int max_out,
                      int nms_mode, int select_mode, yolo_box *boxes_out, int32_t *counts_out, int out_loc);
@@ -139,6 +140,7 @@
 int yolo_calibrate(int device, void *stream, int f16, double seconds, float *tflops, float *clock_ghz);
 int yolo_calibrate_copy(int device, void *stream, double seconds, float *gbs);
 int yolo_time_layers(yolo_ctx *ctx, int n, int iters, float *ms_out);
+int yolo_set_timing_score_thr(yolo_ctx *ctx, float score_thr);
 int yolo_autotune(yolo_ctx *ctx, int n, int iters);
 int yolo_get_tile_configs(const yolo_ctx *ctx, int32_t *cfgs);
 int yolo_set_tile_configs(yolo_ctx *ctx, const int32_t *cfgs);
diff --git a/yolo_tensorflow_amd/csrc/conv_cfgs.h b/yolo_tensorflow_amd/csrc/conv_cfgs.h
--- a/yolo_tensorflow_amd/csrc/conv_cfgs.h
+++ b/yolo_tensorflow_amd/csrc/conv_cfgs.h
@@ -50,6 +50,7 @@
 using Cfgs16 = CfgList<0, 1, 2, 3, 4, 5, 6, 7, 8, 9, 10, 11, 12, 13, 14, 15, 16, 17, 18, 19, 20, 21, 22, 23, 24, 25, 26, 27, 28, 29, 30, 31, 32, 33, 34, 35,
                        44, 45, 46, 47, 48, 49, 50, 51, 52, 53>;
 using CfgsHalo16 = CfgList<36, 37, 38, 39, 40, 41, 42, 43, 54, 55, 56>;
+using CfgsSparseHead = CfgList<12, 13, 17, 35, 44, 45, 46, 47, 50>;
 using CfgsFp8 = CfgList<0, 2, 4, 6, 8, 12, 14, 16, 17, 19, 20, 23, 31, 32, 33, 34, 45, 48, 49, 51>;
 using CfgsHaloFp8 = CfgList<36, 37, 38, 39, 40, 41, 42, 43>;
 using CfgsSplit = CfgList<0, 2, 3, 4, 6, 7, 8, 14, 15, 16, 23, 25, 26, 27, 28, 33, 34, 45, 49, 52>;
@@ -60,6 +61,8 @@
 
 template <int... I> constexpr bool cfgs_are(CfgList<I...>, bool halo) { return ((I >= 0 && I < kNumCfgs && kCfgs[I].halo == halo) && ...); }
 static_assert(cfgs_are(Cfgs16{}, false) && cfgs_are(CfgsFp8{}, false) && cfgs_are(CfgsSplit{}, false) && cfgs_are(CfgsPairK{}, false) && cfgs_are(CfgsPairKPlain{}, false), "tiled lists hold tiled ids");
+template <int... I> constexpr bool cfgs_sparse_ok(CfgList<I...>) { return ((Cfgs16::has(I) && kCfgs[I].wc * kCfgs[I].tc * 16 == 256 && kCfgs[I].nl == 0 && kCfgs[I].bk == 64) && ...); }
+static_assert(cfgs_sparse_ok(CfgsSparseHead{}), "sparse head stores: symmetric 128-byte-row shapes of the 16-bit family whose channel tile is 256 wide");
 static_assert(cfgs_are(CfgsHalo16{}, true) && cfgs_are(CfgsHaloFp8{}, true) && cfgs_are(CfgsHaloSplit{}, true) && cfgs_are(CfgsHaloPairK{}, true), "halo lists hold halo ids");
 
 inline bool conv_cfg_instantiated(const ConvArgs &a, int cfg)
diff --git a/yolo_tensorflow_amd/csrc/conv_igemm.hip b/yolo_tensorflow_amd/csrc/conv_igemm.hip
--- a/yolo_tensorflow_amd/csrc/conv_igemm.hip
+++ b/yolo_tensorflow_amd/csrc/conv_igemm.hip
@@ -200,8 +200,37 @@
     return launch_t<c.wp, c.wc, c.tp, c.tc, c.ns, c.bk, c.nl, EB, H16, SPLIT>(a, s);
 }
 
+template <int ID, bool H16>
+static hipError_t launch_sparse_head(const ConvArgs &a, hipStream_t s)
+{
+    constexpr ConvCfg c = kCfgs[ID];
+    constexpr int BP = c.wp * c.tp * 16, BC = c.wc * c.tc * 16;
+    if (((double)a.N * a.H * a.W * a.in_stride + 2.0 * (a.W + 1) * a.in_stride) * 2 >= 2147483648.0) return hipErrorInvalidValue;
+    const long M = (long)a.N * a.Ho * a.Wo;
+    const long tiles = (M + BP - 1) / BP;
+    constexpr size_t lds = conv_lds_bytes<c.wp, c.wc, c.tp, c.tc, c.ns, c.bk, 0>();
+    static_assert(lds >= (size_t)BP * 16, "the pass bytes of a tile fit the staging LDS");
+    const auto kernel = conv_igemm<c.wp, c.wc, c.tp, c.tc, c.ns, c.bk, true, 0, false, 2, false, false, H16, false, HALO_B, HALO_B, false, false, true>;
+    if (lds > 65536) { hipError_t e = conv_opt_in_lds((const void *)kernel, lds); if (e != hipSuccess) return e; }
+    hipLaunchKernelGGL(kernel, dim3((unsigned)((tiles + 7) / 8 * 8)), dim3(64 * c.wp * c.wc), lds, s, conv_tile_magic(a, BC, 0));
+    return hipGetLastError();
+}
+
+bool conv_sparse_head_ok(const ConvArgs &a, int cfg)
+{
+    if (!CfgsSparseHead::has(cfg)) return false;
+    if ((a.in_dt != DT_BF16 && a.in_dt != DT_F16) || a.out_dt != DT_F32 || a.split || a.pairk || a.w2 || a.res || a.oscale) return false;
+    if (!a.obj_out || a.obj_na < 1 || a.obj_na > 16 || a.obj_attrs < 6 || a.obj_na * a.obj_attrs != a.Cout || a.Cout > 256) return false;
+    return a.Cin_pad % 64 == 0 && a.Kpad % 64 == 0;
+}
+
 hipError_t launch_conv_bf16(const ConvArgs &a, int cfg, hipStream_t s)
 {
+    if (a.head_reject > 0.f) {
+        if (!conv_sparse_head_ok(a, cfg)) return hipErrorInvalidValue;
+        if (a.in_dt == DT_F16) return cfg_dispatch(CfgsSparseHead{}, cfg, [&](auto id) { return launch_sparse_head<decltype(id)::value, true>(a, s); });
+        return cfg_dispatch(CfgsSparseHead{}, cfg, [&](auto id) { return launch_sparse_head<decltype(id)::value, false>(a, s); });
+    }
     if (a.in_dt != DT_BF16 && a.in_dt != DT_F16) return hipErrorInvalidValue;
     if (a.in_dt == DT_F16 && a.out_dt != DT_F16 && a.out_dt != DT_F32) return hipErrorInvalidValue;
     if (cfg == CONV_CFG_DIRECT && a.split) return launch_conv_c8_direct_pair(a, s);
diff --git a/yolo_tensorflow_amd/csrc/conv_igemm_kernel.h b/yolo_tensorflow_amd/csrc/conv_igemm_kernel.h
--- a/yolo_tensorflow_amd/csrc/conv_igemm_kernel.h
+++ b/yolo_tensorflow_amd/csrc/conv_igemm_kernel.h
@@ -3,6 +3,7 @@
 #include "conv_cfgs.h"
 #include "device_common.h"
 #include "halo_perm_tables.h"
+#include "head_filter.h"
 #include <type_traits>
 #include <utility>
 
@@ -76,7 +77,7 @@
 constexpr unsigned halo_div_mul(int bw) { return (65536u + bw - 1) / bw; }
 constexpr bool halo_div_ok(int bw) { for (unsigned r = 0; r < 256; ++r) if (((r * halo_div_mul(bw)) >> 16) != r / bw) return false; return true; }
 
-template <int WP, int WC, int TP, int TC, int NS, int BK, bool UNI, int NL = 0, bool DIAG = false, int EB = 2, bool HALO = false, bool FREE = false, bool H16 = false, bool SPLIT = false, int BH = HALO_B, int BW = HALO_B, bool HEADT = false, bool PAIRK = false>
+template <int WP, int WC, int TP, int TC, int NS, int BK, bool UNI, int NL = 0, bool DIAG = false, int EB = 2, bool HALO = false, bool FREE = false, bool H16 = false, bool SPLIT = false, int BH = HALO_B, int BW = HALO_B, bool HEADT = false, bool PAIRK = false, bool SPARSE = false>
 __global__ __launch_bounds__(64 * (WP * WC + NL)) void conv_igemm(const ConvArgs a)
 {
 #if defined(__HIP_DEVICE_COMPILE__)
@@ -958,7 +959,36 @@
                 }
             }
         }
-    } else if (is_consumer && !HALO) {
+    } else if ((SPARSE || is_consumer) && !HALO) {
+        constexpr int FLAG_NA = 16;
+        static_assert(!SPARSE || (EB == 2 && !SPLIT && !PAIRK && !DIAG && NL == 0), "sparse head stores: the plain 16-bit symmetric forms");
+        if constexpr (SPARSE) {
+            block_barrier();
+#pragma unroll
+            for (int i = 0; i < TC; ++i) {
+                const int ch = ct * BC + (wci * TC + i) * 16 + lq * 4;
+                int oq = -1, oan = 0;
+#pragma unroll
+                for (int q = 0; q < 4; ++q) {
+                    const int an = fast_div(ch + q, a.obj_mul, a.obj_shift);
+                    if (ch + q - an * a.obj_attrs == 4 && ch + q < a.Cout) { oq = q; oan = an; }
+                }
+                if (oq < 0) continue;
+                const float4 bv = *(const float4 *)(a.bias + ch);
+                const float ob = oq == 0 ? bv.x : oq == 1 ? bv.y : oq == 2 ? bv.z : bv.w;
+#pragma unroll
+                for (int j = 0; j < TP; ++j) {
+                    const int row = (wpi * TP + j) * 16 + l15, m = pt * BP + row;
+                    if (m >= M) continue;
+                    float v = (oq == 0 ? acc[i][j][0] : oq == 1 ? acc[i][j][1] : oq == 2 ? acc[i][j][2] : acc[i][j][3]) + ob;
+                    if (a.act != ACT_LINEAR) v = fmaxf(v, act_slope(a.act) * v);
+                    a.obj_out[(size_t)m * a.obj_na + oan] = v;
+                    smem[row * FLAG_NA + oan] = lean_box_passes(sigmoid_fast(v), a.head_reject) ? 1 : 0;
+                }
+            }
+            asm volatile("s_waitcnt lgkmcnt(0)" ::: "memory");
+            block_barrier();
+        }
 #pragma unroll
         for (int i = 0; i < TC; ++i) {
             const int ch = ct * BC + (wci * TC + i) * 16 + lq * 4;
@@ -967,17 +997,26 @@
             float4 sv = float4{1.f, 1.f, 1.f, 1.f};
             if (EB == 1 && a.oscale) sv = *(const float4 *)(a.oscale + ch);
             int oq = -1, oan = 0;
-            if (a.obj_out) {
+            if (!SPARSE && a.obj_out) {
 #pragma unroll
                 for (int q = 0; q < 4; ++q) {
                     const int an = fast_div(ch + q, a.obj_mul, a.obj_shift);
                     if (ch + q - an * a.obj_attrs == 4 && ch + q < a.Cout) { oq = q; oan = an; }
                 }
             }
+            int an_lo = 0, an_hi = 0;
+            if constexpr (SPARSE) {
+                const int last = ch + 3 < a.Cout ? ch + 3 : a.Cout - 1;
+                an_lo = fast_div(ch, a.obj_mul, a.obj_shift); an_hi = fast_div(last, a.obj_mul, a.obj_shift);
+            }
 #pragma unroll
             for (int j = 0; j < TP; ++j) {
                 const int m = pt * BP + (wpi * TP + j) * 16 + l15;
                 if (m >= M) continue;
+                if constexpr (SPARSE) {
+                    const char *fl = smem + ((wpi * TP + j) * 16 + l15) * FLAG_NA;
+                    if (!(fl[an_lo] | fl[an_hi])) continue;
+                }
                 float v[4];
                 if (EB == 1) { v[0] = acc[i][j][0] * sv.x + bv.x; v[1] = acc[i][j][1] * sv.y + bv.y; v[2] = acc[i][j][2] * sv.z + bv.z; v[3] = acc[i][j][3] * sv.w + bv.w; }
                 else { v[0] = acc[i][j][0] + bv.x; v[1] = acc[i][j][1] + bv.y; v[2] = acc[i][j][2] + bv.z; v[3] = acc[i][j][3] + bv.w; }
diff --git a/yolo_tensorflow_amd/csrc/head_filter.h b/yolo_tensorflow_amd/csrc/head_filter.h
--- /dev/null
+++ b/yolo_tensorflow_amd/csrc/head_filter.h
@@ -0,0 +1,9 @@
+#pragma once
+#include <hip/hip_runtime.h>
+
+__device__ __forceinline__ float sigmoid_fast(float x)
+{
+    const float e = __builtin_amdgcn_exp2f(-x * 1.44269504088896340736f);
+    return __builtin_amdgcn_rcpf(1.0f + e);
+}
+__device__ __forceinline__ bool lean_box_passes(float obj, float reject_below) { return !(obj < reject_below); }
diff --git a/yolo_tensorflow_amd/csrc/kernels.h b/yolo_tensorflow_amd/csrc/kernels.h
--- a/yolo_tensorflow_amd/csrc/kernels.h
+++ b/yolo_tensorflow_amd/csrc/kernels.h
@@ -67,6 +67,7 @@
     int C2out;
     int tail_f32;
     uint32_t tc_mul, tc_shift, bpi_mul, bpi_shift, bpr_mul, bpr_shift;
+    float head_reject;
 };
 inline int conv_kchunk(int cin_pad, int wdt) { const int row = wdt == DT_FP8 ? 128 : 64; return (wdt != DT_F32 && cin_pad % row == 0) ? row : cin_pad; }
 inline void conv_magic(uint32_t d, uint32_t &mul, uint32_t &shift)
@@ -100,6 +101,7 @@
 bool conv_cfg_runs(const ConvArgs &a, int cfg);
 int conv_resolve_cfg(const ConvArgs &a, int planned);
 hipError_t launch_conv_bf16(const ConvArgs &a, int cfg, hipStream_t s);
+bool conv_sparse_head_ok(const ConvArgs &a, int cfg);
 bool conv_halo13_ok(const ConvArgs &a);
 bool conv_halo_cfg_ok(const ConvArgs &a, int cfg);
 bool conv_cfg_is_halo(int cfg);
diff --git a/yolo_tensorflow_amd/csrc/post_ops.hip b/yolo_tensorflow_amd/csrc/post_ops.hip
--- a/yolo_tensorflow_amd/csrc/post_ops.hip
+++ b/yolo_tensorflow_amd/csrc/post_ops.hip
@@ -1,15 +1,11 @@
 #include "kernels.h"
 #include "wave_ops.h"
+#include "head_filter.h"
 #include <math.h>
 
 struct BoxOut { float x0, y0, x1, y1, score; int cls; };
 
 __device__ __forceinline__ float sigmoidf_(float x) { return 1.0f / (1.0f + expf(-x)); }
-__device__ __forceinline__ float sigmoid_fast(float x)
-{
-    const float e = __builtin_amdgcn_exp2f(-x * 1.44269504088896340736f);
-    return __builtin_amdgcn_rcpf(1.0f + e);
-}
 
 __device__ __forceinline__ float yolo_box_attr(int k, float x, int cx, int cy, const float *anchor, float GW, float GH, float SX, float SY, int mode)
 {
@@ -212,7 +208,7 @@
         const unsigned row = b * (unsigned)a.rows_total + (unsigned)row_off + (unsigned)cell * (unsigned)na + (unsigned)an;
         const unsigned eoff = cidx * (unsigned)raw_stride + (unsigned)(an * attrs);
         const float obj = sigmoid_fast(objp ? objp[ubox] : raw[eoff + 4]);
-        const bool pass = valid && !(obj < a.reject_below);
+        const bool pass = valid && lean_box_passes(obj, a.reject_below);
         if (valid && !pass) { scores[row] = obj; labels[row] = 0; }
         int tot;
         const int rank = block_rank(pass, wcnt, tot);
diff --git a/yolo_tensorflow_amd/csrc/yolo_api.cpp b/yolo_tensorflow_amd/csrc/yolo_api.cpp
--- a/yolo_tensorflow_amd/csrc/yolo_api.cpp
+++ b/yolo_tensorflow_amd/csrc/yolo_api.cpp
@@ -193,6 +193,8 @@
     return YOLO_OK;
 }
 
+static int head_whole(yolo_ctx *c, const Layer &P, const char *what);
+
 size_t yolo_last_layer_size(const yolo_ctx *c)
 {
     if (!c) return 0;
@@ -232,6 +234,7 @@
     const Layer &L = c->layers[li]; const Layer &P = c->layers[li - 1];
     const size_t per = yolo_last_layer_size(c), need = per * (size_t)n;
     if (out_floats < need) return fail(c, YOLO_ERR_INVALID, "output buffer too small (%zu < %zu floats)", out_floats, need);
+    if (int r = head_whole(c, P, "yolo_last_layer_output")) return r;
     HIPCK(c, hipSetDevice(c->device));
     if (L.type == L_DETECT) {
         HIPCK(c, hipMemcpy2DAsync(out, per * 4, P.out.ptr, (size_t)P.out.stride * 4, per * 4, (size_t)n, hipMemcpyDeviceToHost, c->stream)); HIPCK(c, hipStreamSynchronize(c->stream));
@@ -250,6 +253,25 @@
 }
 
 int yolo_last_layer_output(yolo_ctx *c, float *out, size_t out_floats) { return yolo_last_layer_output_batch(c, 1, out, out_floats); }
+
+static int head_whole(yolo_ctx *c, const Layer &P, const char *what)
+{
+    if (!P.sparse_last) return YOLO_OK;
+    return fail(c, YOLO_ERR_STATE, "%s: the last pass ran through yolo_detect* with score threshold %g and its head convs stored only the boxes the decode kept "
+                "(sparse head stores); the whole head tensor needs a yolo_forward* pass", what, c->lean_thr);
+}
+
+int yolo_head_sparse(const yolo_ctx *c, int head)
+{
+    if (!c || head < 0) return YOLO_ERR_INVALID;
+    int k = 0;
+    for (size_t li = 1; li < c->layers.size(); ++li) {
+        const Layer &L = c->layers[li];
+        if (L.type != L_YOLO && L.type != L_REGION && L.type != L_DETECT) continue;
+        if (k++ == head) return c->layers[li - 1].sparse_last ? 1 : 0;
+    }
+    return YOLO_ERR_INVALID;
+}
 
 int yolo_head_raw(yolo_ctx *c, int head, int n, float *out, size_t out_floats)
 {
@@ -265,6 +287,7 @@
         const size_t px = (size_t)n * P.H * P.W, need = px * P.C;
         if (out_floats < need) return fail(c, YOLO_ERR_INVALID, "output buffer too small (%zu < %zu floats)", out_floats, need);
         if (P.out.dt != DT_F32 || !P.out.ptr) return fail(c, YOLO_ERR_STATE, "internal: head conv output is not fp32");
+        if (int r = head_whole(c, P, "yolo_head_raw")) return r;
         HIPCK(c, hipSetDevice(c->device));
         HIPCK(c, hipMemcpy2DAsync(out, (size_t)P.C * 4, P.out.ptr, (size_t)P.out.stride * 4, (size_t)P.C * 4, px, hipMemcpyDeviceToHost, c->stream));
         HIPCK(c, hipStreamSynchronize(c->stream));
@@ -326,6 +349,7 @@
     if (dims_out) { dims_out[0] = L.H; dims_out[1] = L.W; dims_out[2] = L.C; }
     size_t need = (size_t)n * L.H * L.W * L.C;
     if (!out) return YOLO_OK;
+    if (int r = head_whole(c, L, "yolo_layer_output")) return r;
     if (out_floats < need) return fail(c, YOLO_ERR_INVALID, "output buffer too small");
     HIPCK(c, hipSetDevice(c->device));
     float *tmp = nullptr; HIPCK(c, hipMalloc((void **)&tmp, need * 4));
diff --git a/yolo_tensorflow_amd/csrc/yolo_ctx.h b/yolo_tensorflow_amd/csrc/yolo_ctx.h
--- a/yolo_tensorflow_amd/csrc/yolo_ctx.h
+++ b/yolo_tensorflow_amd/csrc/yolo_ctx.h
@@ -39,6 +39,7 @@
     int residual_from = -2;
     bool head = false;
     float *d_obj = nullptr;
+    bool sparse_last = false;
     int kernel = K_TILED;
     int fused = F_NONE, launcher = -1;
     int fuse_n = 0; bool fuse_ok = false;
@@ -101,6 +102,8 @@
     float *d_dn_rec = nullptr; int *d_dn_src = nullptr; int *d_dn_count = nullptr; float *d_dn_last = nullptr; size_t dn_last_cap = 0;
     struct GKey { const void *img; int n, fmt; float scale, st, it; int mo, nm, sm; void *bo, *co; } gkey{};
     hipGraphExec_t gexec = nullptr; int gstate = 0;
+    float time_thr = 0.f;
+    bool graph_dense = false;
     ImgDesc *d_descs = nullptr; void *d_pix = nullptr; size_t pix_cap = 0;
     int geom_fit = -1, geom_n = 0;
     struct GKeyImages { const void *pix; size_t bytes; int n, fit, units; float st, it; int mo, nm, sm; void *bo, *co; } gkey_img;
@@ -174,6 +177,7 @@
 DeconvArgs deconv_geometry(int size, int stride, int pad, int h, int w, int cin_pad, int filters, int act, int in_dt);
 GConvArgs gconv_geometry(int size, int stride, int pad, int h, int w, int cin, int filters, int groups, int act, int in_dt);
 int run_layer(yolo_ctx *c, int i, int n);
+bool dense_heads_forced();
 int stage_in(yolo_ctx *c, const void *images, int n, int fmt, int loc, float scale);
 int run_network(yolo_ctx *c, int n, bool lean = false);
 int copy_out(yolo_ctx *c, void *dst, const void *src, size_t bytes, int loc);
diff --git a/yolo_tensorflow_amd/csrc/yolo_run.cpp b/yolo_tensorflow_amd/csrc/yolo_run.cpp
--- a/yolo_tensorflow_amd/csrc/yolo_run.cpp
+++ b/yolo_tensorflow_amd/csrc/yolo_run.cpp
@@ -157,9 +157,32 @@
     return G.fuse_ok;
 }
 
+bool dense_heads_forced() { const char *e = getenv("YOLO_DENSE_HEADS"); return e && *e && strcmp(e, "0") != 0; }
+
+static float head_sparse_thr(const yolo_ctx *c, const Layer &L, const ConvArgs &a, int cfg)
+{
+    const int li = (int)(&L - c->layers.data());
+    if (!L.head || !L.d_obj || li + 1 >= (int)c->layers.size() || c->layers[li + 1].type != L_YOLO) return 0.f;
+    if (!(c->lean && c->lean_thr > 0.f && c->lean_heads >= 1 && c->lean_heads <= 4) || c->tree_head >= 0 || c->keep_layers || !c->half_like()) return 0.f;
+    if (L.kernel != K_TILED || L.fused != F_NONE || rides_as_tail(c, L) || L.post_act != ACT_LINEAR || dense_heads_forced()) return 0.f;
+    return conv_sparse_head_ok(a, cfg) ? c->lean_thr : 0.f;
+}
+
+static void mark_heads(yolo_ctx *c, int n)
+{
+    for (auto &L : c->layers) {
+        if (L.type != L_CONV || !L.head) continue;
+        L.sparse_last = false;
+        if (!L.d_obj || c->dtype == YOLO_FP32) continue;
+        const ConvArgs a = conv_args(c, L, n);
+        L.sparse_last = head_sparse_thr(c, L, a, conv_resolve_cfg(a, L.tile_cfg)) > 0.f;
+    }
+}
+
 static int run_conv(yolo_ctx *c, int i, int n)
 {
     Layer &L = c->layers[i];
+    if (L.head) L.sparse_last = false;
     hipStream_t s = c->stream;
     auto nview = [&](TView v) { v.n = n; return v; };
     if (fused_launch_applies(c, L, n)) {
@@ -184,7 +207,9 @@
     if (c->dtype == YOLO_FP32) { HIPCK(c, launch_conv_f32(a, s)); return YOLO_OK; }
     const int cfg = conv_resolve_cfg(a, L.tile_cfg);
     if (a.w2 && !a.split && !a.pairk && !conv_cfg_tail_ok(cfg, a.Cout, a.in_dt == DT_FP8, a.tail_f32 != 0)) return fail(c, YOLO_ERR_STATE, "layer %d: tile config %d cannot run the fused 1x1 tail", i, cfg);
+    if (L.head) a.head_reject = head_sparse_thr(c, L, a, cfg);
     HIPCK(c, a.in_dt == DT_FP8 ? launch_conv_fp8(a, cfg, s) : launch_conv_bf16(a, cfg, s));
+    L.sparse_last = a.head_reject > 0.f;
     return YOLO_OK;
 }
 
@@ -566,6 +591,7 @@
     if (!c) return YOLO_ERR_INVALID;
     if (!images || !boxes_out || !counts_out) return fail(c, YOLO_ERR_INVALID, "yolo_detect_graph needs device pointers for images, boxes_out and counts_out");
     yolo_ctx::GKey k{images, n, fmt, scale, score_thr, iou_thr, max_out, nms_mode, select_mode, (void *)boxes_out, (void *)counts_out};
+    if (dense_heads_forced() != c->graph_dense) { drop_graph(c); c->graph_dense = !c->graph_dense; }
     if (memcmp(&k, &c->gkey, sizeof k) != 0) {
         if (c->gexec) { hipGraphExecDestroy(c->gexec); c->gexec = nullptr; }
         c->gkey = k; if (c->gstate >= 0) c->gstate = 0;
@@ -592,6 +618,7 @@
     HIPCK(c, hipGraphLaunch(c->gexec, c->stream));
     c->lean = nms_mode != YOLO_NMS_NUMPY_V3 && c->lean_ok; c->det_valid = !c->lean; c->lean_thr = score_thr;
     c->last_n = n; c->scores_mode = nms_mode == YOLO_NMS_NUMPY_V3 ? 1 : 0;
+    mark_heads(c, n);
     return YOLO_OK;
 }
 
@@ -691,6 +718,7 @@
     yolo_ctx::GKeyImages k; memset(&k, 0, sizeof k);
     k.pix = pixels; k.bytes = bytes; k.n = n; k.fit = fit; k.units = units; k.st = score_thr; k.it = iou_thr; k.mo = max_out; k.nm = nms_mode; k.sm = select_mode;
     k.bo = (void *)boxes_out; k.co = (void *)counts_out;
+    if (dense_heads_forced() != c->graph_dense) { drop_graph(c); c->graph_dense = !c->graph_dense; }
     if (memcmp(&k, &c->gkey_img, sizeof k) != 0) {
         if (c->gexec_img) { hipGraphExecDestroy(c->gexec_img); c->gexec_img = nullptr; }
         c->gkey_img = k; if (c->gstate_img >= 0) c->gstate_img = 0;
@@ -719,6 +747,7 @@
     HIPCK(c, hipGraphLaunch(c->gexec_img, c->stream));
     c->lean = lean && c->lean_ok; c->det_valid = !c->lean; c->lean_thr = score_thr;
     c->last_n = n; c->scores_mode = nms_mode == YOLO_NMS_NUMPY_V3 ? 1 : 0; c->stem_u8 = nullptr; c->geom_fit = fit; c->geom_n = n;
+    mark_heads(c, n);
     return YOLO_OK;
 }
 
@@ -806,6 +835,14 @@
     EventSet(const EventSet &) = delete; EventSet &operator=(const EventSet &) = delete;
 }; }
 
+int yolo_set_timing_score_thr(yolo_ctx *c, float score_thr)
+{
+    if (!c) return YOLO_ERR_INVALID;
+    if (!(score_thr >= 0.f)) return fail(c, YOLO_ERR_INVALID, "score_thr %g", score_thr);
+    c->time_thr = score_thr;
+    return YOLO_OK;
+}
+
 int yolo_time_forward(yolo_ctx *c, int n, int iters, float *total_ms, float *conv_ms)
 {
     if (!c) return YOLO_ERR_INVALID;
@@ -814,16 +851,18 @@
     HIPCK(c, hipSetDevice(c->device));
     EventSet evs(2); if (!evs.ok) return fail(c, YOLO_ERR_HIP, "hipEventCreate failed");
     hipEvent_t e0 = evs.e[0], e1 = evs.e[1];
-    c->lean = false;
+    const bool as_detect = c->time_thr > 0.f && c->lean_ok;
+    c->lean = false; c->lean_thr = as_detect ? c->time_thr : 0.f;
     if (c->stem_u8 && n > c->stem_u8_n) c->stem_u8 = nullptr;
     if (total_ms) {
         HIPCK(c, hipEventRecord(e0, c->stream));
-        for (int it = 0; it < iters; ++it) { int r = run_network(c, n); if (r) return r; }
+        for (int it = 0; it < iters; ++it) { int r = run_network(c, n, as_detect); if (r) return r; }
         HIPCK(c, hipEventRecord(e1, c->stream)); HIPCK(c, hipEventSynchronize(e1));
         float ms = 0; HIPCK(c, hipEventElapsedTime(&ms, e0, e1)); *total_ms = ms / iters;
     }
     if (conv_ms) {
         float all_ms = 0, rest_ms = 0;
+        c->lean = as_detect;
         for (int pass = 0; pass < 2; ++pass) {
             HIPCK(c, hipEventRecord(e0, c->stream));
             for (int it = 0; it < iters; ++it) { int r = run_layers(c, n, pass == 1); if (r) return r; }
@@ -831,7 +870,7 @@
             float ms = 0; HIPCK(c, hipEventElapsedTime(&ms, e0, e1)); (pass == 0 ? all_ms : rest_ms) = ms / iters;
         }
         *conv_ms = all_ms - rest_ms;
-        c->last_n = n; c->scores_mode = 0; c->det_valid = true;
+        c->last_n = n; c->scores_mode = 0; c->det_valid = !c->lean;
     }
     return YOLO_OK;
 }
@@ -843,7 +882,7 @@
     if (n < 1 || n > c->max_batch || iters < 1) return fail(c, YOLO_ERR_INVALID, "bad n/iters");
     HIPCK(c, hipSetDevice(c->device));
     const int NL = (int)c->layers.size();
-    c->lean = false; c->det_valid = true;
+    c->lean = c->time_thr > 0.f && c->lean_ok; c->lean_thr = c->lean ? c->time_thr : 0.f; c->det_valid = !c->lean; c->scores_mode = 0;
     if (c->stem_u8 && n > c->stem_u8_n) c->stem_u8 = nullptr;
     EventSet evs(NL + 1); if (!evs.ok) return fail(c, YOLO_ERR_HIP, "hipEventCreate failed");
     std::vector<hipEvent_t> &ev = evs.e;
diff --git a/yolo_tensorflow_amd/hip.py b/yolo_tensorflow_amd/hip.py
--- a/yolo_tensorflow_amd/hip.py
+++ b/yolo_tensorflow_amd/hip.py
@@ -37,7 +37,7 @@
     "yolo_set_hier_thresh", "yolo_set_hierarchy_mode", "yolo_darknet_boxes_map", "yolo_tree_geometry", "yolo_tree_read", "yolo_plan_check", "yolo_plan_table",
     "yolo_op_tree_softmax", "yolo_op_tree_top", "yolo_activation_code", "yolo_op_activate", "yolo_op_shortcut",
     "yolo_output_map_geometry", "yolo_output_map", "yolo_label_map", "yolo_segment_images_u8", "yolo_op_deconv2d", "yolo_op_l2norm", "yolo_op_upsample", "yolo_op_label_map",
-    "yolo_op_conv2d_grouped",
+    "yolo_op_conv2d_grouped", "yolo_head_sparse", "yolo_set_timing_score_thr",
 ]
 HIER_CONDITIONAL, HIER_ABSOLUTE, HIER_LEAVES = 0, 1, 2
 _HIER_MODES = {None: HIER_CONDITIONAL, "conditional": HIER_CONDITIONAL, "absolute": HIER_ABSOLUTE, "leaves": HIER_LEAVES}
@@ -116,6 +116,9 @@
     l.yolo_postprocess_rows.argtypes = [P, I, F, F, I, I, I, P, P, P, I]
     l.yolo_last_layer_output_batch.argtypes = [P, I, P, C.c_size_t]
     l.yolo_head_raw.argtypes = [P, I, I, P, C.c_size_t]
+    if hasattr(l, "yolo_head_sparse"):
+        l.yolo_head_sparse.argtypes = [P, I]
+        l.yolo_set_timing_score_thr.argtypes = [P, F]
     l.yolo_calibrate.argtypes = [I, P, I, C.c_double, FP, FP]
     l.yolo_calibrate_copy.argtypes = [I, P, C.c_double, FP]
     l.yolo_op_resize_cv2.argtypes = [P, I, I, I, I, I, F, P, I]
@@ -370,6 +373,15 @@
         self._check(self.lib.yolo_head_raw(self.ctx, head, n, out.ctypes.data, out.size), "yolo_head_raw")
         return out
 
+    def head_sparse(self, head):
+        rc = self.lib.yolo_head_sparse(self.ctx, head)
+        if rc < 0:
+            raise YoloError("yolo_head_sparse failed (%d): no detection head %d" % (rc, head))
+        return bool(rc)
+
+    def set_timing_score_thr(self, score_thr):
+        self._check(self.lib.yolo_set_timing_score_thr(self.ctx, float(score_thr)), "yolo_set_timing_score_thr")
+
     def last_layer_output(self, n=1):
         self.lib.yolo_last_layer_size.restype = C.c_size_t
         per = self.lib.yolo_last_layer_size(self.ctx)
```

Result: no change. 12580 img/s (median of 3 runs) (+0.0%).
